# hazdzz/STGCN

Measured on AMD Instinct MI355X. Metric: training windows/sec, METR-LA ChebConv K=3 bs=32, higher is better.
Workload: dtype f32; 1 GPU; C2: METR-LA 207 nodes, STGCNChebGraphConv Ks=3 Kt=3, n_his=12, bs=32 per GPU, fp32, dropout 0.5, AdamW lr 1e-3 wd 1e-3; full step zero_grad+fwd+MSE+bwd+opt; graph=real metr_la adj -> sym_norm_lap -> cheb GSO, global_batch=32, parallelism=dp1, output_block=fused HIP path (stgcn_outblock_*), launch=hipGraph replay, chains=1, backward_products=fp32, operator_products=fp32

## Files before the change

### include/stgcn_hip.h

```cpp
#ifndef STGCN_HIP_H
#define STGCN_HIP_H
#include <stddef.h>
#include <stdint.h>
#ifdef __cplusplus
extern "C" {
#endif

#define STGCN_ABI_VERSION 10

#define STGCN_OK 0
#define STGCN_ERR_UNSUPPORTED 1
#define STGCN_ERR_INVALID 2
#define STGCN_ERR_LAUNCH 3

#define STGCN_ACT_GLU 0
#define STGCN_ACT_GTU 1
#define STGCN_GC_CHEB 0
#define STGCN_GC_KIPF 1

#define STGCN_DTYPE_F32 0
#define STGCN_DTYPE_BF16 1

typedef struct stgcn_stblock_desc {
    int32_t B, T, N;
// ... 154 lines not shown

typedef struct stgcn_head_loss {
    const float* pred;
    const float* target;
    const int64_t* target_index_dev;
    int64_t target_index_stride;
    const int64_t* target_window_dev;
    float grad_scale;
    int32_t kind;
    float delta;
} stgcn_head_loss;

typedef struct stgcn_outblock_plan {
    int64_t T1, rows, rows_in;
    int64_t out_floats;
    int64_t saved_floats, ws_floats;
    int64_t sv_U, sv_S;
    int64_t sv_mean, sv_rstd;
    int64_t sv_yln;
    int64_t sv_hd;
    int64_t sv_rowstat;
    int64_t ws_Wp, ws_Wd, ws_b, ws_W1p, ws_W1d;
    int64_t ws_rowstat_b, ws_dh1, ws_dyln, ws_dZ, ws_part, part_floats;
    int64_t ws_chain;
    int64_t chain_words;
} stgcn_outblock_plan;

int stgcn_outblock_plan_query(const stgcn_outblock_desc* desc, stgcn_outblock_plan* plan);
int stgcn_outblock_forward(const stgcn_outblock_desc* desc, const stgcn_outblock_params* params, const float* x, float* out,
                           float* saved, float* ws, uint64_t seed, uint64_t offset, const uint64_t* offset_dev, void* stream);
int stgcn_outblock_chain_status(const stgcn_outblock_desc* desc, const float* ws, uint32_t* sticky, void* stream);
int64_t stgcn_set_chain_spin_ticks(int64_t ticks);
int stgcn_outblock_backward(const stgcn_outblock_desc* desc, const stgcn_outblock_params* params, const float* x,
                            const float* dout, const float* saved, float* ws, const stgcn_outblock_grads* grads, float* dx,
                            void* stream);
int stgcn_outblock_backward_hook(const stgcn_outblock_desc* desc, const stgcn_outblock_params* params, const float* x,
                                 const float* dout, const float* saved, float* ws, const stgcn_outblock_grads* grads, float* dx,
                                 const stgcn_ln_hook* dx_hook, void* stream);
int stgcn_outblock_backward_loss(const stgcn_outblock_desc* desc, const stgcn_outblock_params* params, const float* x,
                                 const stgcn_head_loss* loss, const float* saved, float* ws, const stgcn_outblock_grads* grads, float* dx,
                                 const stgcn_ln_hook* dx_hook, void* stream);

typedef struct stgcn_prepack_block {
    const stgcn_stblock_desc* desc;
    const stgcn_stblock_params* params;
    float* ws;
} stgcn_prepack_block;
typedef struct stgcn_step_counter {
    int64_t* ptr;
    int64_t inc, mod;
} stgcn_step_counter;
int stgcn_prepack(int32_t n_blocks, const stgcn_prepack_block* blocks, const stgcn_outblock_desc* head_desc,
                  const stgcn_outblock_params* head_params, float* head_ws, int32_t n_counters, const stgcn_step_counter* counters,
                  void* stream);
int stgcn_prepack_park(int32_t n_blocks, const stgcn_prepack_block* blocks, const stgcn_outblock_desc* head_desc,
                  const stgcn_outblock_params* head_params, float* head_ws, int32_t n_counters, const stgcn_step_counter* counters,
                  void* stream);
int stgcn_prepack_flush(void);

typedef struct stgcn_adamw_tensor {
    float* param;
    const float* grad;
    float* exp_avg;
    float* exp_avg_sq;
    int64_t numel;
} stgcn_adamw_tensor;
int stgcn_adamw_step(const stgcn_adamw_tensor* tensors, int32_t count, float lr, float beta1, float beta2, float eps,
                     float weight_decay, int64_t step, const int64_t* step_dev, const float* lr_dev, void* stream);

typedef struct stgcn_flush_block {
    const stgcn_stblock_desc* desc;
    const stgcn_stblock_grads* grads;
    float* ws;
} stgcn_flush_block;
typedef struct stgcn_adamw_hyper {
    float lr, beta1, beta2, eps, weight_decay;
    int64_t step;
    const int64_t* step_dev;
    const float* lr_dev;
} stgcn_adamw_hyper;
int stgcn_grad_flush(int32_t n_blocks, const stgcn_flush_block* blocks, const stgcn_outblock_desc* head_desc,
                     const stgcn_outblock_grads* head_grads, float* head_ws, const stgcn_adamw_tensor* opt, int32_t opt_count,
                     const stgcn_adamw_hyper* hyper, void* stream);

#define STGCN_OPT_ADAMW 0
#define STGCN_OPT_NADAMW 1
#define STGCN_OPT_LION 2
typedef struct stgcn_optim_hyper {
    int32_t kind;
    double lr, beta1, beta2, eps, weight_decay, momentum_decay;
    int64_t step;
    const int64_t* step_dev;
    const float* lr_dev;
    float mu_product;
    float* mu_product_dev;
} stgcn_optim_hyper;
int stgcn_optim_step(const stgcn_adamw_tensor* tensors, int32_t count, const stgcn_optim_hyper* hyper, void* stream);
int stgcn_grad_flush_optim(int32_t n_blocks, const stgcn_flush_block* blocks, const stgcn_outblock_desc* head_desc,
                           const stgcn_outblock_grads* head_grads, float* head_ws, const stgcn_adamw_tensor* opt, int32_t opt_count,
                           const stgcn_optim_hyper* hyper, void* stream);

#define STGCN_CLIP_HDR_WORDS 8
typedef struct stgcn_grad_clip {
    double* state;
    int64_t state_words;
    float max_norm;
} stgcn_grad_clip;
int stgcn_grad_clip_words(const stgcn_adamw_tensor* tensors, int32_t count, int64_t* words);
int stgcn_grad_flush_clip_words(int32_t n_blocks, const stgcn_flush_block* blocks, const stgcn_outblock_desc* head_desc,
                                const stgcn_outblock_grads* head_grads, float* head_ws, int64_t* words);
int stgcn_grad_norm(const stgcn_adamw_tensor* tensors, int32_t count, const stgcn_grad_clip* clip, void* stream);
int stgcn_optim_step_clip(const stgcn_adamw_tensor* tensors, int32_t count, const stgcn_optim_hyper* hyper, const stgcn_grad_clip* clip,
                          void* stream);
int stgcn_grad_flush_clip(int32_t n_blocks, const stgcn_flush_block* blocks, const stgcn_outblock_desc* head_desc,
                          const stgcn_outblock_grads* head_grads, float* head_ws, const stgcn_grad_clip* clip, void* stream);

int stgcn_mse_loss_grad(const float* pred, const float* target, int64_t n, float grad_scale, float* loss, float* dpred,
                        const int64_t* target_index_dev, int64_t target_index_stride, void* stream);
int stgcn_mse_loss_grad_windows(const float* pred, const float* target, int64_t n, float grad_scale, float* loss, float* dpred,
                                const int64_t* target_index_dev, int64_t target_index_stride, const int64_t* target_window_dev,
                                int64_t window_floats, void* stream);
int stgcn_loss_grad(int32_t kind, float delta, const float* pred, const float* target, int64_t n, float grad_scale, float* loss,
                    float* dpred, const int64_t* target_index_dev, int64_t target_index_stride, const int64_t* target_window_dev,
                    int64_t window_floats, void* stream);

#define STGCN_EVAL_STATE_WORDS 264
#define STGCN_EVAL_POS_WORDS 4
int stgcn_eval_arm(double* state, int64_t* pos, void* stream);
int stgcn_eval_accumulate(const float* pred, const float* target, int32_t B, int32_t N, const float* scale, const float* mean,
                          int64_t first_valid, int64_t* pos, int64_t target_stride, int64_t num_windows, double* state, void* stream);

int stgcn_profile_enable(int on);
int stgcn_profile_collect(char* json_buf, size_t cap);

#ifdef __cplusplus
}
#endif
#endif
```

### stgcn_amd/_lib.py

```python
from __future__ import annotations

import ctypes as C
import os
from typing import Optional

_HERE = os.path.dirname(os.path.abspath(__file__))
DEFAULT_LIB = os.path.join(_HERE, "libstgcn_hip.so")

STGCN_OK = 0
ABI_VERSION = 10
ACT = {"glu": 0, "gtu": 1}
GRAPH_CONV = {"cheb_graph_conv": 0, "graph_conv": 1}
DTYPE_F32, DTYPE_BF16 = 0, 1
LOSS = {"mse": 0, "mae": 1, "huber": 2}
EVAL_STATE_WORDS, EVAL_POS_WORDS = 264, 4

_fp = C.POINTER(C.c_float)


class StblockDesc(C.Structure):
    _fields_ = [("B", C.c_int32), ("T", C.c_int32), ("N", C.c_int32), ("c_in", C.c_int32),
                ("c0", C.c_int32), ("c1", C.c_int32), ("c2", C.c_int32), ("Kt", C.c_int32), ("Ks", C.c_int32),
                ("act", C.c_int32), ("graph_conv", C.c_int32), ("training", C.c_int32),
                ("droprate", C.c_float), ("ln_eps", C.c_float), ("need_dx", C.c_int32), ("reserved", C.c_int32),
# ... 127 lines not shown
                                       C.POINTER(C.c_int32)]
        d.stgcn_gso_layout.restype = C.c_int
        d.stgcn_set_gc_tiled_min_nodes.argtypes = [C.c_int32]
        d.stgcn_set_gc_tiled_min_nodes.restype = C.c_int
        d.stgcn_outblock_backward_loss.argtypes = [C.POINTER(OutblockDesc), C.POINTER(OutblockParams), C.c_void_p, C.POINTER(HeadLoss), C.c_void_p,
                                                   C.c_void_p, C.POINTER(OutblockGrads), C.c_void_p, C.POINTER(LnHook), C.c_void_p]
        d.stgcn_outblock_backward_loss.restype = C.c_int
        d.stgcn_set_bwd_precision.argtypes = [C.c_int32]
        d.stgcn_set_bwd_precision.restype = C.c_int
        d.stgcn_set_slab_gc_precision.argtypes = [C.c_int32]
        d.stgcn_set_slab_gc_precision.restype = C.c_int
        d.stgcn_set_tc1_bwd_wgs.argtypes = [C.c_int32]
        d.stgcn_set_tc1_bwd_wgs.restype = C.c_int
        d.stgcn_set_tc2ln_peers.argtypes = [C.c_int32]
        d.stgcn_set_tc2ln_peers.restype = C.c_int
        d.stgcn_stblock_chain_status.argtypes = [C.POINTER(StblockDesc), C.c_void_p, C.POINTER(C.c_uint32), C.c_void_p]
        d.stgcn_stblock_chain_status.restype = C.c_int
        d.stgcn_set_debug_stages.argtypes = [C.c_int32]
        d.stgcn_set_debug_stages.restype = C.c_int
        d.stgcn_set_gc_precision.argtypes = [C.c_int32]
        d.stgcn_set_gc_precision.restype = C.c_int
        d.stgcn_set_gc_ld_pad.argtypes = [C.c_int32]
        d.stgcn_set_gc_ld_pad.restype = C.c_int
        d.stgcn_set_gemm_big_nt.argtypes = [C.c_int32]
        d.stgcn_set_gemm_big_nt.restype = C.c_int
        d.stgcn_set_chain_spin_ticks.argtypes = [C.c_int64]
        d.stgcn_set_chain_spin_ticks.restype = C.c_int64
        d.stgcn_outblock_chain_status.argtypes = [C.POINTER(OutblockDesc), C.c_void_p, C.POINTER(C.c_uint32), C.c_void_p]
        d.stgcn_outblock_chain_status.restype = C.c_int
        d.stgcn_stblock_forward.argtypes = [C.POINTER(StblockDesc), C.POINTER(StblockParams), C.c_void_p, C.c_void_p,
                                            C.c_void_p, C.c_void_p, C.c_void_p, C.c_uint64, C.c_uint64, C.c_void_p, C.c_void_p]
        d.stgcn_stblock_backward.argtypes = [C.POINTER(StblockDesc), C.POINTER(StblockParams), C.c_void_p, C.c_void_p,
                                             C.c_void_p, C.c_void_p, C.c_void_p, C.c_void_p, C.POINTER(StblockGrads), C.c_void_p,
                                             C.c_uint64, C.c_uint64, C.c_void_p, C.c_void_p]
        d.stgcn_stblock_backward_hook.argtypes = [C.POINTER(StblockDesc), C.POINTER(StblockParams), C.c_void_p, C.c_void_p,
                                                  C.c_void_p, C.c_void_p, C.c_void_p, C.c_void_p, C.POINTER(StblockGrads), C.c_void_p,
                                                  C.c_uint64, C.c_uint64, C.c_void_p, C.POINTER(LnHook), C.c_void_p]
        d.stgcn_stblock_ln_hook.argtypes = [C.POINTER(StblockDesc), C.POINTER(StblockParams), C.c_void_p, C.c_void_p, C.c_uint64, C.c_uint64,
                                            C.c_void_p, C.POINTER(LnHook)]
        d.stgcn_outblock_backward_hook.argtypes = [C.POINTER(OutblockDesc), C.POINTER(OutblockParams), C.c_void_p, C.c_void_p, C.c_void_p,
                                                   C.c_void_p, C.POINTER(OutblockGrads), C.c_void_p, C.POINTER(LnHook), C.c_void_p]
        for f in ("stgcn_stblock_backward_hook", "stgcn_stblock_ln_hook", "stgcn_outblock_backward_hook"):
            getattr(d, f).restype = C.c_int
        d.stgcn_dropout_mask.argtypes = [C.c_void_p, C.c_int64, C.c_float, C.c_uint64, C.c_uint64, C.c_void_p, C.c_void_p]
        d.stgcn_outblock_plan_query.argtypes = [C.POINTER(OutblockDesc), C.POINTER(OutblockPlan)]
        d.stgcn_outblock_forward.argtypes = [C.POINTER(OutblockDesc), C.POINTER(OutblockParams), C.c_void_p, C.c_void_p, C.c_void_p,
                                             C.c_void_p, C.c_uint64, C.c_uint64, C.c_void_p, C.c_void_p]
        d.stgcn_outblock_backward.argtypes = [C.POINTER(OutblockDesc), C.POINTER(OutblockParams), C.c_void_p, C.c_void_p, C.c_void_p,
                                              C.c_void_p, C.POINTER(OutblockGrads), C.c_void_p, C.c_void_p]
        for f in ("stgcn_outblock_plan_query", "stgcn_outblock_forward", "stgcn_outblock_backward"):
            getattr(d, f).restype = C.c_int
        d.stgcn_adamw_step.argtypes = [C.POINTER(AdamwTensor), C.c_int32, C.c_float, C.c_float, C.c_float, C.c_float, C.c_float, C.c_int64,
                                       C.c_void_p, C.c_void_p, C.c_void_p]
        d.stgcn_adamw_step.restype = C.c_int
        d.stgcn_prepack.argtypes = [C.c_int32, C.POINTER(PrepackBlock), C.POINTER(OutblockDesc), C.POINTER(OutblockParams), C.c_void_p,
                                    C.c_int32, C.POINTER(StepCounter), C.c_void_p]
        d.stgcn_prepack.restype = C.c_int
        d.stgcn_prepack_park.argtypes = [C.c_int32, C.POINTER(PrepackBlock), C.POINTER(OutblockDesc), C.POINTER(OutblockParams), C.c_void_p,
                                    C.c_int32, C.POINTER(StepCounter), C.c_void_p]
        d.stgcn_prepack_park.restype = C.c_int
        d.stgcn_prepack_flush.argtypes = []
        d.stgcn_prepack_flush.restype = C.c_int
        d.stgcn_grad_flush.argtypes = [C.c_int32, C.POINTER(FlushBlock), C.POINTER(OutblockDesc), C.POINTER(OutblockGrads), C.c_void_p,
                                       C.POINTER(AdamwTensor), C.c_int32, C.POINTER(AdamwHyper), C.c_void_p]
        d.stgcn_grad_flush.restype = C.c_int
        d.stgcn_optim_step.argtypes = [C.POINTER(AdamwTensor), C.c_int32, C.POINTER(OptimHyper), C.c_void_p]
        d.stgcn_optim_step.restype = C.c_int
        d.stgcn_grad_flush_optim.argtypes = [C.c_int32, C.POINTER(FlushBlock), C.POINTER(OutblockDesc), C.POINTER(OutblockGrads), C.c_void_p,
                                             C.POINTER(AdamwTensor), C.c_int32, C.POINTER(OptimHyper), C.c_void_p]
        d.stgcn_grad_flush_optim.restype = C.c_int
        for f in ("stgcn_grad_clip_words", "stgcn_grad_flush_clip_words", "stgcn_grad_norm", "stgcn_optim_step_clip", "stgcn_grad_flush_clip"):
            if not hasattr(d, f):
                raise StgcnError(f"{path} does not export {f} (built before gradient clipping was added): rebuild with "
                                 f"`python -m stgcn_amd.build --force`")
        d.stgcn_grad_clip_words.argtypes = [C.POINTER(AdamwTensor), C.c_int32, C.POINTER(C.c_int64)]
        d.stgcn_grad_flush_clip_words.argtypes = [C.c_int32, C.POINTER(FlushBlock), C.POINTER(OutblockDesc), C.POINTER(OutblockGrads), C.c_void_p,
                                                  C.POINTER(C.c_int64)]
        d.stgcn_grad_norm.argtypes = [C.POINTER(AdamwTensor), C.c_int32, C.POINTER(GradClip), C.c_void_p]
        d.stgcn_optim_step_clip.argtypes = [C.POINTER(AdamwTensor), C.c_int32, C.POINTER(OptimHyper), C.POINTER(GradClip), C.c_void_p]
        d.stgcn_grad_flush_clip.argtypes = [C.c_int32, C.POINTER(FlushBlock), C.POINTER(OutblockDesc), C.POINTER(OutblockGrads), C.c_void_p,
                                            C.POINTER(GradClip), C.c_void_p]
        for f in ("stgcn_grad_clip_words", "stgcn_grad_flush_clip_words", "stgcn_grad_norm", "stgcn_optim_step_clip", "stgcn_grad_flush_clip"):
            getattr(d, f).restype = C.c_int
        d.stgcn_mse_loss_grad.argtypes = [C.c_void_p, C.c_void_p, C.c_int64, C.c_float, C.c_void_p, C.c_void_p, C.c_void_p, C.c_int64,
                                          C.c_void_p]
        d.stgcn_mse_loss_grad.restype = C.c_int
        d.stgcn_mse_loss_grad_windows.argtypes = [C.c_void_p, C.c_void_p, C.c_int64, C.c_float, C.c_void_p, C.c_void_p, C.c_void_p, C.c_int64,
                                                  C.c_void_p, C.c_int64, C.c_void_p]
        d.stgcn_mse_loss_grad_windows.restype = C.c_int
        d.stgcn_loss_grad.argtypes = [C.c_int32, C.c_float, C.c_void_p, C.c_void_p, C.c_int64, C.c_float, C.c_void_p, C.c_void_p, C.c_void_p,
                                      C.c_int64, C.c_void_p, C.c_int64, C.c_void_p]
        d.stgcn_loss_grad.restype = C.c_int
        d.stgcn_eval_arm.argtypes = [C.c_void_p, C.c_void_p, C.c_void_p]
        d.stgcn_eval_arm.restype = C.c_int
        d.stgcn_eval_accumulate.argtypes = [C.c_void_p, C.c_void_p, C.c_int32, C.c_int32, C.c_void_p, C.c_void_p, C.c_int64, C.c_void_p,
                                            C.c_int64, C.c_int64, C.c_void_p, C.c_void_p]
        d.stgcn_eval_accumulate.restype = C.c_int
        d.stgcn_profile_enable.argtypes = [C.c_int]
        d.stgcn_profile_enable.restype = C.c_int
        d.stgcn_profile_collect.argtypes = [C.c_char_p, C.c_size_t]
        d.stgcn_profile_collect.restype = C.c_int
        for f in ("stgcn_stblock_plan_query", "stgcn_gso_prepare", "stgcn_stblock_forward", "stgcn_stblock_backward",
                  "stgcn_dropout_mask"):
            getattr(d, f).restype = C.c_int
        self.backend = d.stgcn_backend().decode()
        self.is_emulator = self.backend.startswith("emu")

    def check(self, rc: int, what: str):
        if rc != STGCN_OK:
            msg = self.dll.stgcn_last_error().decode()
            if rc == 1:
                raise NotImplementedError(f"{what}: {msg}")
            if rc == 2:
                raise ValueError(f"{what}: {msg}")
            raise StgcnError(f"{what}: {msg} (code {rc})")


_lib: Optional[_Lib] = None


def use_library(path: str) -> _Lib:
    global _lib
    _lib = _Lib(path)
    return _lib


def lib() -> _Lib:
    global _lib
    if _lib is None:
        _lib = _Lib(os.environ.get("STGCN_AMD_LIB", DEFAULT_LIB))
    return _lib


EXPORTED_SYMBOLS = ["stgcn_version", "stgcn_backend", "stgcn_last_error", "stgcn_stblock_plan_query", "stgcn_gso_prepare",
                    "stgcn_stblock_forward", "stgcn_stblock_backward", "stgcn_dropout_mask", "stgcn_profile_enable",
                    "stgcn_profile_collect", "stgcn_outblock_plan_query", "stgcn_outblock_forward", "stgcn_outblock_backward", "stgcn_adamw_step", "stgcn_prepack",
                    "stgcn_mse_loss_grad", "stgcn_mse_loss_grad_windows", "stgcn_grad_flush", "stgcn_gso_layout", "stgcn_set_gc_tiled_min_nodes",
                    "stgcn_set_gc_precision", "stgcn_set_gc_ld_pad", "stgcn_set_debug_stages",
                    "stgcn_stblock_ln_hook", "stgcn_stblock_backward_hook", "stgcn_outblock_backward_hook", "stgcn_set_tc1_bwd_wgs",
                    "stgcn_set_slab_gc_precision", "stgcn_outblock_backward_loss", "stgcn_set_bwd_precision", "stgcn_set_gemm_big_nt",
                    "stgcn_set_chain_spin_ticks", "stgcn_outblock_chain_status", "stgcn_set_tc2ln_peers", "stgcn_stblock_chain_status", "stgcn_prepack_park", "stgcn_prepack_flush",
                    "stgcn_optim_step", "stgcn_grad_flush_optim", "stgcn_eval_arm", "stgcn_eval_accumulate", "stgcn_loss_grad",
                    "stgcn_grad_clip_words", "stgcn_grad_flush_clip_words", "stgcn_grad_norm", "stgcn_optim_step_clip", "stgcn_grad_flush_clip"]
```

### stgcn_amd/csrc/stgcn_capi.hip

```cpp
#include "../../include/stgcn_hip.h"

#include <atomic>
#include <stdarg.h>
#include <stdio.h>
#include <stdlib.h>
#include <math.h>
#include <string.h>

#include "stgcn_kernels_bwd.hip.h"
#include "stgcn_kernels_fwd.hip.h"
#include "stgcn_kernels_gctile.hip.h"
#include "stgcn_kernels_gcslab16.hip.h"
#include "stgcn_kernels_head.hip.h"
#include "stgcn_route.h"

using namespace stgcn;

namespace {
thread_local char g_err[512] = "";
thread_local bool g_bf16 = false;
std::atomic<long long> g_chain_spin_ticks{kChainSpinTicks};
int g_gemm_big_nt = 0;

int fail(int code, const char* fmt, ...) __attribute__((format(printf, 2, 3)));
// ... 526 lines not shown
    const int HT = a.NP / 16;
    int pf = 0, pb = 1;
    gc_parts_override(pf, pb);
    {
        const int force_parts = force_gcbwd2_parts();
        const bool b16p = g_bf16 && a.Ks > 1;
        const size_t lds2 = gconv_bwd2_lds_bytes(a.NP, a.N, a.Ks, b16p);
        if (lds2 <= 150 * 1024 && HT <= 64) {
            int best = 0;
            for (int parts = (HT + 7) / 8; parts <= HT && !force_parts; ++parts) {
                const int per = (HT + parts - 1) / parts, njw = gcbwd2_job_waves(a.Ks, parts, per > 8 ? 8 : per);
                if (per < 4 && parts > (HT + 7) / 8) break;
                const int cap = b16p ? wg_capacity(gconv_bwd2_kernel<1, bf16, true>, ((per > 8 ? 8 : per) + njw) * 64, lds2)
                                     : STGCN_ETB_VALUE(wg_capacity(gconv_bwd2_kernel<1, ET>, ((per > 8 ? 8 : per) + njw) * 64, lds2));
                if (a.slabs * parts <= cap) best = parts;
            }
            if (force_parts > 0 && force_parts <= HT && (HT + force_parts - 1) / force_parts <= 24) best = force_parts;
            if (!best && !force_parts && HT <= 24) best = 1;
            if (best > 0) {
                const int per = (HT + best - 1) / best, nwa = per > 8 ? 8 : per, maxq = (per + nwa - 1) / nwa, njw = gcbwd2_job_waves(a.Ks, best, nwa);
                a.parts = best;
                const dim3 grid2((unsigned)(a.slabs * best)), blk2((nwa + njw) * 64);
                if (b16p) {
                    if (maxq <= 1) STGCN_LAUNCH("gconv_bwd", st, (gconv_bwd2_kernel<1, bf16, true>), grid2, blk2, lds2, a, nwa);
                    else if (maxq <= 2) STGCN_LAUNCH("gconv_bwd", st, (gconv_bwd2_kernel<2, bf16, true>), grid2, blk2, lds2, a, nwa);
                    else STGCN_LAUNCH("gconv_bwd", st, (gconv_bwd2_kernel<3, bf16, true>), grid2, blk2, lds2, a, nwa);
                    return STGCN_OK;
                }
                if (maxq <= 1) STGCN_LAUNCH_ETB("gconv_bwd", st, (gconv_bwd2_kernel<1, ET>), grid2, blk2, lds2, a, nwa);
                else if (maxq <= 2) STGCN_LAUNCH_ETB("gconv_bwd", st, (gconv_bwd2_kernel<2, ET>), grid2, blk2, lds2, a, nwa);
                else STGCN_LAUNCH_ETB("gconv_bwd", st, (gconv_bwd2_kernel<3, ET>), grid2, blk2, lds2, a, nwa);
                return STGCN_OK;
            }
        }
    }
    const GcGeom g = gc_geom(HT, pb);
    a.parts = g.parts;
    const size_t lds = ((size_t)a.Ks * 16 * (a.NP + 4) + (size_t)a.NP * 20) * sizeof(float);
    if (lds > 160 * 1024) return fail(STGCN_ERR_UNSUPPORTED, "graph-conv backward needs %zu bytes of LDS (N=%d, terms=%d)", lds, a.N, a.Ks);
    const dim3 grid((unsigned)(a.slabs * g.parts)), blk(g.waves * 64);
    if (g.maxq <= 1) STGCN_LAUNCH_ETB("gconv_bwd", st, (gconv_bwd_kernel<1, 16, ET>), grid, blk, lds, a);
    else if (g.maxq <= 2) STGCN_LAUNCH_ETB("gconv_bwd", st, (gconv_bwd_kernel<2, 8, ET>), grid, blk, lds, a);
    else if (g.maxq <= 3) STGCN_LAUNCH_ETB("gconv_bwd", st, (gconv_bwd_kernel<3, 8, ET>), grid, blk, lds, a);
    else if (g.maxq <= 4) STGCN_LAUNCH_ETB("gconv_bwd", st, (gconv_bwd_kernel<4, 8, ET>), grid, blk, lds, a);
    else return fail(STGCN_ERR_UNSUPPORTED, "graph convolution with %d nodes (supported: up to 512)", a.N);
    return STGCN_OK;
}

template <int MTW>
int launch_bwd_weight_n(const char* label, const TconvBwdWeightArgs& a, const WgradGeom& w, hipStream_t st) {
    const dim3 grid(w.chunks, w.mchunks), blk(kThreads * kWgradGroups);
    if (a.NC == 128) STGCN_LAUNCH_ET(label, st, (tconv_bwd_weight_kernel<MTW, 2, true, ET>), grid, blk, wgrad_lds_bytes(MTW, 2), a);
    else STGCN_LAUNCH_ET(label, st, (tconv_bwd_weight_kernel<MTW, 4, true, ET>), grid, blk, wgrad_lds_bytes(MTW, 4), a);
    return STGCN_OK;
}
int launch_bwd_weight(const char* label, const TconvBwdWeightArgs& a, const WgradGeom& w, hipStream_t st) {
    if (a.NC != 128 && a.NC != 256) return fail(STGCN_ERR_UNSUPPORTED, "weight gradient with %d output channels", a.NC);
    if ((a.ts.C & 3) != 0) {
        if (w.MTW != 1) return fail(STGCN_ERR_UNSUPPORTED, "weight gradient: c_in=%d needs Kt*c_in <= 16", a.ts.C);
        if (a.NC == 128) STGCN_LAUNCH_ET(label, st, (tconv_bwd_weight_kernel<1, 2, false, ET>), dim3(w.chunks, w.mchunks), dim3(kThreads * kWgradGroups), wgrad_lds_bytes(1, 2), a);
        else STGCN_LAUNCH_ET(label, st, (tconv_bwd_weight_kernel<1, 4, false, ET>), dim3(w.chunks, w.mchunks), dim3(kThreads * kWgradGroups), wgrad_lds_bytes(1, 4), a);
        return STGCN_OK;
    }
    switch (w.MTW) {
        case 1: return launch_bwd_weight_n<1>(label, a, w, st);
        case 2: return launch_bwd_weight_n<2>(label, a, w, st);
        case 3: return launch_bwd_weight_n<3>(label, a, w, st);
        default: return launch_bwd_weight_n<4>(label, a, w, st);
    }
}

inline bool wgrad_pair_ok(const TconvBwdWeightArgs& a1, const WgradGeom& w1, const TconvBwdWeightArgs& a2, const WgradGeom& w2) {
    return a1.NC == 256 && w1.MTW == 4 && a2.NC == 128 && w2.MTW == 4 && (a1.ts.C & 3) == 0 && (a2.ts.C & 3) == 0;
}
int launch_wgrad_pair(const char* label, const TconvBwdWeightArgs& a1, const WgradGeom& w1, const TconvBwdWeightArgs& a2, const WgradGeom& w2,
                      hipStream_t st) {
    const int n1 = w1.chunks * w1.mchunks, n2 = w2.chunks * w2.mchunks;
    const size_t l1 = wgrad_lds_bytes(4, 4), l2 = wgrad_lds_bytes(4, 2);
    STGCN_LAUNCH_ETB(label, st, (wgrad_pair_kernel<4, 4, 4, 2, ET>), dim3((unsigned)(n1 + n2)), dim3(kThreads * kWgradGroups), l1 > l2 ? l1 : l2, a1, n1,
                    w1.mchunks, a2, n2, w2.mchunks);
    return STGCN_OK;
}

struct ReduceList {
    ReduceArgs ra;
    int nj;
    bool overflow;
    ReduceList() : nj(0), overflow(false) { memset(&ra, 0, sizeof(ra)); }
    void add(float* dst, const float* src, int Pn, long pstride, int n0, int n1, int n2, long s0, long s1, long s2, long t0, long t1,
             long t2) {
        if (!dst) return;
        if (nj >= kMaxReduceJobs) { overflow = true; return; }
        ReduceJob& j = ra.job[nj];
        j.src = src; j.dst = dst; j.P = Pn; j.pstride = pstride; j.n0 = n0; j.n1 = n1; j.n2 = n2;
        j.s0 = (int)s0; j.s1 = (int)s1; j.s2 = (int)s2; j.t0 = (int)t0; j.t1 = (int)t1; j.t2 = (int)t2;
        ra.start[nj + 1] = ra.start[nj] + reduce_job_setup(j);
        ++nj;
    }
    void add_flat(float* dst, const float* src, int Pn, long pstride, int n) { add(dst, src, Pn, pstride, 1, 1, n, 0, 0, 1, 0, 0, 1); }
};
int launch_reduce_list(const char* label, ReduceList& L, hipStream_t st) {
    if (L.overflow) return fail(STGCN_ERR_INVALID, "%s: more than %d reduction jobs in one launch", label, kMaxReduceJobs);
    if (L.nj == 0) return STGCN_OK;
    L.ra.njobs = L.nj;
    if (reduce_log())
        for (int i = 0; i < L.nj; ++i) {
            const ReduceJob& j = L.ra.job[i];
            fprintf(stderr, "[stgcn reduce] %s job %d: %ld elements x %d partials (%.2f MB read), %d workgroups\n", label, i,
                    (long)j.n0 * j.n1 * j.n2, j.P, 4e-6 * (double)j.n0 * j.n1 * j.n2 * j.P, L.ra.start[i + 1] - L.ra.start[i]);
        }
    STGCN_LAUNCH(label, st, reduce_kernel<kOptAdamw>, dim3(L.ra.start[L.nj]), dim3(kThreads), kThreads * 4 * sizeof(float), L.ra);
    return STGCN_OK;
}
int launch_reduce_list_optim(const char* label, ReduceList& L, int kind, const OptimExtra& x, hipStream_t st) {
    if (L.overflow) return fail(STGCN_ERR_INVALID, "%s: more than %d reduction jobs in one launch", label, kMaxReduceJobs);
    if (L.nj == 0) return STGCN_OK;
    L.ra.njobs = L.nj;
    ReduceOptimArgs a = zeroed<ReduceOptimArgs>();
    static_cast<ReduceArgs&>(a) = L.ra;
    a.x = x;
    if (kind == kOptNadamw)
        STGCN_LAUNCH(label, st, reduce_kernel<kOptNadamw>, dim3(L.ra.start[L.nj]), dim3(kThreads), kThreads * 4 * sizeof(float), a);
    else
        STGCN_LAUNCH(label, st, reduce_kernel<kOptLion>, dim3(L.ra.start[L.nj]), dim3(kThreads), kThreads * 4 * sizeof(float), a);
    return STGCN_OK;
}
void reduce_jobs_block(ReduceList& L, const stgcn_stblock_desc* d, const BlockRoute& v, const float* part, const stgcn_stblock_grads* G) {
    const BwdGeom& bg = v.bg;
    auto add_tconv_at = [&](const float* wp, const float* bp, int Pn, long ps, long pb, int NC, long LD, int Cin, int Cout, float* gw, float* gb, float* gaw,
                            float* gab) {
        L.add(gw, wp, Pn, ps, NC, d->Kt, Cin, LD, Cin, 1, (long)Cin * d->Kt, 1, d->Kt);
        L.add_flat(gb, bp, Pn, pb, NC);
        if (Cin > Cout) {
            L.add(gaw, wp + (long)(d->Kt - 1) * Cin, Pn, ps, 1, Cout, Cin, 0, LD, 1, 0, Cin, 1);
            L.add_flat(gab, bp, Pn, pb, Cout);
        }
    };
    auto add_tconv = [&](const WgradGeom& w, int Cin, int Cout, float* gw, float* gb, float* gaw, float* gab) {
        const float* wp = part + w.off;
        add_tconv_at(wp, wp + (long)w.chunks * w.Mpad * w.NC, w.chunks, (long)w.Mpad * w.NC, w.NC, w.NC, w.Mpad, Cin, Cout, gw, gb, gaw, gab);
    };
    if (bg.k3) {
        const float* wp = part + bg.off_k3;
        add_tconv_at(wp, wp + (long)d->Kt * d->c_in * v.NC1, bg.k3_wgs, bg.k3_stride, bg.k3_stride, v.NC1, (long)d->Kt * d->c_in, d->c_in, d->c0, G->tc1_w,
                     G->tc1_b, G->tc1_aw, G->tc1_ab);
    } else if (bg.thin) {
        const float* wp = part + bg.off_al + (long)d->c0 * 16 + 16;
        L.add(G->tc1_w, wp, bg.al_wgs, bg.al_stride, d->Kt, d->c_in, v.NC1, (long)d->c_in * v.NC1, v.NC1, 1, 1, d->Kt, (long)d->c_in * d->Kt);
        L.add_flat(G->tc1_b, wp + 16 * v.NC1, bg.al_wgs, bg.al_stride, v.NC1);
    } else {
        add_tconv(bg.w1, d->c_in, d->c0, G->tc1_w, G->tc1_b, G->tc1_aw, G->tc1_ab);
    }
    if (bg.k1) {
        const float* wp = part + bg.off_k1;
        add_tconv_at(wp, wp + (long)d->Kt * 16 * v.NC2, bg.k1_wgs, bg.k1_stride, bg.k1_stride, v.NC2, (long)d->Kt * 16, d->c1, d->c2, G->tc2_w, G->tc2_b,
                     G->tc2_aw, G->tc2_ab);
    } else {
        add_tconv(bg.w2, d->c1, d->c2, G->tc2_w, G->tc2_b, G->tc2_aw, G->tc2_ab);
    }
    if (d->c0 > d->c1) {
        const float* ap = bg.k3 ? part + bg.off_k3 + (long)d->Kt * d->c_in * v.NC1 + v.NC1 : part + bg.off_al;
        const int Pn = bg.k3 ? bg.k3_wgs : bg.al_wgs, ps = bg.k3 ? bg.k3_stride : bg.al_stride;
        L.add(G->al_w, ap, Pn, ps, 1, d->c0, d->c1, 0, d->c1, 1, 0, 1, d->c0);
        L.add_flat(G->al_b, ap + (long)d->c0 * d->c1, Pn, ps, d->c1);
    }
    if (d->graph_conv == STGCN_GC_KIPF) L.add_flat(G->gc_w, part + bg.off_gc + 256, bg.gc_count, bg.gc_stride, 256);
// ... 315 lines not shown
    hipStream_t st = (hipStream_t)stream;
    const int NP = gc_padded_nodes(N, terms);
    const size_t M = (size_t)NP * NP;
    const dim3 grid(cdiv((int64_t)M, kThreads)), blk(kThreads);
    if (gc_is_tiled(N, terms)) {
        STGCN_LAUNCH("gso_dense", st, gso_dense_kernel, grid, blk, 0, gso, (int)N, NP, gso_pad);
        STGCN_LAUNCH("gso_dense_t", st, gso_dense_t_kernel, grid, blk, 0, gso, (int)N, NP, gso_t_pad);
        unsigned short* hp = reinterpret_cast<unsigned short*>(gso_pad + M);
        unsigned short* ht = reinterpret_cast<unsigned short*>(gso_t_pad + M);
        const int LD = gc_plane_ld(NP);
        STGCN_LAUNCH("gso_bf16", st, gso_bf16_kernel, grid, blk, 0, gso, (int)N, NP, LD, 0, hp, hp + (size_t)NP * LD);
        STGCN_LAUNCH("gso_bf16_t", st, gso_bf16_kernel, grid, blk, 0, gso, (int)N, NP, LD, 1, ht, ht + (size_t)NP * LD);
        return STGCN_OK;
    }
    float* D[3] = {scratch, scratch + M, scratch + 2 * M};
    STGCN_LAUNCH("gso_dense", st, gso_dense_kernel, grid, blk, 0, gso, (int)N, NP, D[0]);
    const float* tm1 = D[0];
    const float* tm2 = nullptr;
    for (int k = 1; k < terms; ++k) {
        const float* tk = tm1;
        if (k >= 2) {
            float* out = (tm1 == D[1]) ? D[2] : D[1];
            STGCN_LAUNCH("cheb_next", st, cheb_next_kernel, grid, blk, 0, (const float*)D[0], tm1, tm2, (int)N, NP, out);
            tm2 = tm1;
            tm1 = out;
            tk = out;
        }
        STGCN_LAUNCH("gso_frag", st, gso_frag_kernel, grid, blk, 0, tk, NP, gso_pad + (size_t)(k - 1) * M, gso_t_pad + (size_t)(k - 1) * M);
        const size_t t16 = gs16_term_floats(NP, N), o16 = (size_t)(terms - 1) * M + (size_t)(k - 1) * t16;
        const int KC32 = gs16_np32(N) / 32;
        STGCN_LAUNCH("gso_frag16", st, gso_frag16_kernel, dim3(cdiv((int64_t)(NP / 16) * KC32 * 512, kThreads)), blk, 0, tk, NP, KC32, gso_pad + o16,
                     gso_t_pad + o16);
    }
    return STGCN_OK;
}

int stgcn_dropout_mask(float* out, int64_t n, float droprate, uint64_t seed, uint64_t offset, const uint64_t* offset_dev, void* stream) {
    if (!out || n < 0 || (n & 3)) return fail(STGCN_ERR_INVALID, "stgcn_dropout_mask: n must be a non-negative multiple of 4");
    if (!(droprate >= 0.f && droprate < 1.f)) return fail(STGCN_ERR_INVALID, "stgcn_dropout_mask: droprate must be in [0, 1)");
    if (n == 0) return STGCN_OK;
    STGCN_LAUNCH("dropout_mask", (hipStream_t)stream, dropout_mask_kernel, dim3(cdiv(n / 4, kThreads)), dim3(kThreads), 0, out,
                 (long)(n / 4), seed, offset, offset_dev, drop_thresh(droprate), 1.0f / (1.0f - droprate));
    return STGCN_OK;
}

int stgcn_stblock_ln_hook(const stgcn_stblock_desc* d, const stgcn_stblock_params* P, const float* y, float* ws, uint64_t seed, uint64_t offset,
                          const uint64_t* offset_dev, stgcn_ln_hook* h) {
    stgcn_stblock_plan pl;
    int rc = stgcn_stblock_plan_query(d, &pl);
    if (rc) return rc;
    if (!P || !P->ln_w || !P->ln_b || !y || !ws || !h) return fail(STGCN_ERR_INVALID, "stgcn_stblock_ln_hook: NULL argument");
    memset(h, 0, sizeof(*h));
    if (!(fuse_mask() & FUSE_ROWSTATS)) return STGCN_OK;
    h->rowstat = ws + pl.ws_rowstat_b; h->y = y; h->gamma = P->ln_w; h->beta = P->ln_b;
    h->N = d->N; h->C = d->c2; h->training = d->training; h->droprate = d->droprate; h->dtype = d->dtype;
    h->seed = seed; h->offset = offset; h->offset_dev = offset_dev;
    return STGCN_OK;
}

int stgcn_stblock_chain_status(const stgcn_stblock_desc* d, const float* ws, uint32_t* sticky, void* stream) {
    STGCN_FLUSH_PENDING_PACK();
    stgcn_stblock_plan pl;
    const int rc = stgcn_stblock_plan_query(d, &pl);
    if (rc) return rc;
    return read_chain_sticky("stgcn_stblock_chain_status", ws, pl.ws_chain, sticky, stream);
}

int stgcn_stblock_forward(const stgcn_stblock_desc* d, const stgcn_stblock_params* P, const float* x, const float* gso_pad, float* y,
                          float* saved, float* ws, uint64_t seed, uint64_t offset, const uint64_t* offset_dev, void* stream) {
    BlockCall c{d, P, {}, {}, x, saved, ws, seed, offset, offset_dev, (hipStream_t)stream};
    int rc = route_and_plan(d, &c.r, &c.pl);
    if (rc) return rc;
    if (!P || !x || !gso_pad || !y || !saved || !ws) return fail(STGCN_ERR_INVALID, "stgcn_stblock_forward: NULL buffer");
    if (!P->tc1_w || !P->tc1_b || !P->gc_w || !P->tc2_w || !P->tc2_b || !P->ln_w || !P->ln_b)
        return fail(STGCN_ERR_INVALID, "stgcn_stblock_forward: missing parameter pointer");
    if (d->c_in > d->c0 && !P->tc1_aw) return fail(STGCN_ERR_INVALID, "tc1_aw required when c_in > c0");
    if (d->c0 > d->c1 && !P->al_w) return fail(STGCN_ERR_INVALID, "al_w required when c0 > c1");
    if (d->c1 > d->c2 && !P->tc2_aw) return fail(STGCN_ERR_INVALID, "tc2_aw required when c1 > c2");
    g_prof_tag = d->reserved;
    g_bf16 = c.r.bf16;

    const bool ride = g_pending_pack.valid && d->prepacked && c.r.tc1_fwd == TC1_FWD_THIN && g_pending_pack.st == c.st;
    if (!ride) STGCN_FLUSH_PENDING_PACK();
    if (!d->prepacked) rc = c.launch_block_pack();
    if (rc) return rc;

    switch (c.r.tc1_fwd) {
        case TC1_FWD_TSTEP: rc = c.launch_tc1_fwd(); break;
        case TC1_FWD_THIN: rc = c.launch_thin_fwd(ride); break;
        case TC1_FWD_ROWTILE: rc = c.launch_rowtile_tc1_fwd(); break;
    }
    if (rc) return rc;
    rc = c.launch_block_gconv_fwd(gso_pad);
    if (rc) return rc;
    return c.r.tc2_ln_fused ? c.launch_tc2_ln_fwd(y) : c.launch_staged_tc2_ln_fwd(y);
}

#include "stgcn_capi_bwd.inc"
#include "stgcn_capi_head.inc"
```

### stgcn_amd/csrc/stgcn_capi_bwd.inc

```

namespace {
int launch_hook_rowstats(const stgcn_ln_hook* hook, const float* dx, long slabs, hipStream_t st) {
    LnBwdArgs hl = zeroed<LnBwdArgs>();
    const LnRowstatOut o = rowstat_out(hook);
    hl.dy = dx; hl.y = o.y; hl.beta = o.beta; hl.gamma = o.gamma; hl.rowstat = o.rowstat;
    hl.n = o.N * o.C; hl.N = o.N; hl.C = o.C; hl.act = o.act; hl.training = o.training; hl.slabs = slabs;
    hl.keep_scale = o.keep_scale; hl.thresh = o.thresh; hl.seed = o.seed; hl.offset = o.offset; hl.offset_dev = o.offset_dev;
    STGCN_LAUNCH_ET("ln_bwd_rowstats", st, (ln_bwd_rowstats_kernel<ET>), dim3(cdiv(hl.slabs * (hl.n / 4), kThreads)), dim3(kThreads), 0, hl);
    return STGCN_OK;
}

struct BlockBwdCall : BlockCall {
    const float* gso_t_pad;
    const float* dy;
    const float* y;
    float* dx;
    const stgcn_ln_hook* dx_hook;
    LnBwdArgs ln;

    int launch_ln_bwd_stats() {
        ln = zeroed<LnBwdArgs>();
        ln.dy = dy; ln.y = y; ln.beta = P->ln_b; ln.U = saved + pl.sv_U2; ln.S = saved + pl.sv_S2; ln.gamma = P->ln_w;
        ln.mean = saved + pl.sv_mean; ln.rstd = saved + pl.sv_rstd; ln.rowstat = reinterpret_cast<float2*>(ws + pl.ws_rowstat_b);
        ln.dZ = ws + pl.ws_dZ2; ln.dgam_part = part() + r.bg.off_ln_g; ln.dbet_part = part() + r.bg.off_ln_b;
// ... 36 lines not shown
            else if (d->act == STGCN_ACT_GLU) STGCN_LAUNCH_ETB("tc2_bwd", st, (tc2_bwd_kernel<C2_, KT_, false, 0, RC_, ET>), grid, blk, lds, a);       \
            else STGCN_LAUNCH_ETB("tc2_bwd", st, (tc2_bwd_kernel<C2_, KT_, false, 1, RC_, ET>), grid, blk, lds, a);                 \
        } while (0)
#define STGCN_TC2_BWD_RC(C2_, KT_) do { if (recomp) { constexpr bool RC_ = true; STGCN_TC2_BWD(C2_, KT_); } else { constexpr bool RC_ = false; STGCN_TC2_BWD(C2_, KT_); } } while (0)
        if (d->Kt == 2) STGCN_TC2_BWD_RC(64, 2); else if (d->Kt == 3) STGCN_TC2_BWD_RC(64, 3); else STGCN_TC2_BWD_RC(64, 4);
#undef STGCN_TC2_BWD_RC
#undef STGCN_TC2_BWD
        return STGCN_OK;
    }
    int launch_staged_tc2_bwd() {
        STGCN_F32_ONLY("ln_gate_bwd + row-tile weight / data gradients of tmp_conv2");
        int rc = launch_ln_gate_bwd();
        if (rc) return rc;
        TconvBwdWeightArgs wa = zeroed<TconvBwdWeightArgs>();
        wa.ts = make_taps(saved + pl.sv_G, d->c1, d->Kt, d->N, r.T1, r.T2, 1, r.rows2);
        wa.dZ = ws + pl.ws_dZ2; wa.part = part() + r.bg.w2.off; wa.NC = r.NC2; wa.Mpad = r.bg.w2.Mpad; wa.rows_per_chunk = r.bg.w2.rows_per_chunk;
        wa.chunks = r.bg.w2.chunks;
        rc = launch_bwd_weight("tconv_bwd_weight.tc2", wa, r.bg.w2, st);
        if (rc) return rc;
        TconvBwdDataArgs a = zeroed<TconvBwdDataArgs>();
        a.ts = make_taps(ws + pl.ws_dZ2, r.NC2, d->Kt, d->N, r.T2, r.T1, -1, r.rows1);
        a.Wp = ws + pl.ws_W2d; a.KCH = d->Kt * r.NC2 / 16; a.Cin = d->c1; a.Gmask = saved + pl.sv_G; a.dX = ws + pl.ws_dYg;
        return launch_bwd_data("tconv_bwd_data.tc2", a, r.CP1 / 16, st);
    }
    int launch_block_gconv_bwd() {
        GconvBwdArgs a = zeroed<GconvBwdArgs>();
        a.dY = ws + pl.ws_dYg; a.X0 = saved + pl.sv_A; a.Xk = saved + pl.sv_Xk; a.LTp = gso_t_pad; a.W = P->gc_w;
        a.dA = ws + pl.ws_dA; a.part = part() + r.bg.off_gc; a.N = d->N; a.NP = r.NP; a.Ks = r.terms;
        a.kipf = d->graph_conv == STGCN_GC_KIPF; a.slabs = r.slabs1;
        a.Gk = r.tiled_gc ? ws + pl.ws_Gk : nullptr; a.tiles_per_wg = r.bg.gc_tiles_per_wg; a.wgs = r.bg.gc_count;
        a.XT = r.tiled_gc && r.terms > 1 ? ws + pl.ws_XT : nullptr;
        return launch_gconv_bwd(a, r.tiled_gc, st);
    }
    int launch_align_gate_bwd() {
        STGCN_F32_ONLY("align_gate_bwd");
        AlignBwdArgs a = zeroed<AlignBwdArgs>();
        a.dA = ws + pl.ws_dA; a.WaT = ws + pl.ws_WaT; a.dZ = ws + pl.ws_dZ1;
        if (r.recompute_tc1) {
            a.Wd = ws + pl.ws_W1dense; a.bias = ws + pl.ws_b1; a.KPd = r.KP1;
            a.ts = input_taps();
        } else {
            a.U = saved + pl.sv_U1; a.S = saved + pl.sv_S1;
        }
        a.part = part() + r.bg.off_al; a.rows = r.rows1; a.c0 = d->c0; a.c1 = d->c1; a.KCH = r.CP1 / 16; a.act = d->act;
        const size_t lds = (size_t)(64 * (d->c1 + 4) + 64 * (d->c0 + 4) + 16 * d->c1) * sizeof(float);
        if (d->c0 == 64) STGCN_LAUNCH("align_gate_bwd", st, (align_gate_bwd_kernel<1>), dim3(r.bg.al_wgs), dim3(kThreads), lds, a);
        else STGCN_LAUNCH("align_gate_bwd", st, (align_gate_bwd_kernel<2>), dim3(r.bg.al_wgs), dim3(kThreads), lds, a);
        return STGCN_OK;
    }
    int launch_tc1_bwd() {
        if (g_debug_stages && !g_bf16) {
            const int rc = launch_align_gate_bwd();
            if (rc) return rc;
        }
        Tc1BwdArgs a = zeroed<Tc1BwdArgs>();
        a.dA = ws + pl.ws_dA; a.U = saved + pl.sv_U1; a.S = saved + pl.sv_S1; a.x = x; a.WaD = ws + pl.ws_WaDense; a.Wd = ws + pl.ws_W1dense;
        a.dx = dx; a.part = part() + r.bg.off_k3; a.B = d->B; a.T = d->T; a.T1 = r.T1; a.N = d->N; a.node_tiles = r.bg.node_tiles;
        const bool hooked = dx_hook && dx_hook->rowstat, epi = hooked && dx_hook->C == d->c_in && dx_hook->N == d->N;
        if (epi) a.rs = rowstat_out(dx_hook);
        const bool x6 = r.tc1_bwd_x6;
        const size_t lds = r.tc1_bwd_lds;
        const dim3 grid((unsigned)r.bg.k3_wgs), blk(768);
#define STGCN_TC1_BWD(CIN_)                                                                                    \
        do {                                                                                                       \
            if (x6 && d->act == STGCN_ACT_GLU) STGCN_LAUNCH("tc1_bwd", st, (tc1_bwd_x6_kernel<64, CIN_, 3, 0>), grid, blk, lds, a);   \
            else if (x6) STGCN_LAUNCH("tc1_bwd", st, (tc1_bwd_x6_kernel<64, CIN_, 3, 1>), grid, blk, lds, a);             \
            else if (d->act == STGCN_ACT_GLU) STGCN_LAUNCH_ETB("tc1_bwd", st, (tc1_bwd_kernel<64, CIN_, 3, 0, ET>), grid, blk, lds, a);   \
            else STGCN_LAUNCH_ETB("tc1_bwd", st, (tc1_bwd_kernel<64, CIN_, 3, 1, ET>), grid, blk, lds, a);             \
        } while (0)
        if (d->c_in == 64) STGCN_TC1_BWD(64); else if (d->c_in == 32) STGCN_TC1_BWD(32); else STGCN_TC1_BWD(16);
#undef STGCN_TC1_BWD
        if (hooked && !epi) return launch_hook_rowstats(dx_hook, dx, (long)d->B * d->T, st);
        return STGCN_OK;
    }
    int launch_thin_bwd() {
        ThinBwdArgs a = zeroed<ThinBwdArgs>();
        a.dA = ws + pl.ws_dA; a.Wd = ws + pl.ws_W1dense; a.bias = ws + pl.ws_b1; a.WaT = ws + pl.ws_WaT;
        a.dZ = d->need_dx ? ws + pl.ws_dZ1 : nullptr; a.part = part() + r.bg.off_al; a.rows = r.rows1; a.c0 = d->c0; a.act = d->act;
        a.ts = input_taps();
        const dim3 grid(r.bg.al_wgs), blk(kThreads);
        if (!r.thin_bwd_waves) {
            const size_t lds = (size_t)(64 * 20 + 64 * (d->c0 + 4) + 64 * (2 * d->c0 + 4) + 64 * 20 + 256) * sizeof(float);
            STGCN_LAUNCH_ETB("align_gate_bwd", st, (thin_tc1_bwd_kernel<ET>), grid, blk, lds, a);
        } else if (d->act == STGCN_ACT_GLU) STGCN_LAUNCH_ETB("align_gate_bwd", st, (thin_tc1_bwd2_kernel<ET, 0>), grid, blk, thin_bwd2_lds_bytes(), a);
        else STGCN_LAUNCH_ETB("align_gate_bwd", st, (thin_tc1_bwd2_kernel<ET, 1>), grid, blk, thin_bwd2_lds_bytes(), a);
        return STGCN_OK;
    }
    int launch_tc1_bwd_weight() {
        TconvBwdWeightArgs wa = zeroed<TconvBwdWeightArgs>();
        wa.ts = input_taps();
        wa.dZ = ws + pl.ws_dZ1; wa.part = part() + r.bg.w1.off; wa.NC = r.NC1; wa.Mpad = r.bg.w1.Mpad; wa.rows_per_chunk = r.bg.w1.rows_per_chunk;
        wa.chunks = r.bg.w1.chunks;
        return launch_bwd_weight("tconv_bwd_weight.tc1", wa, r.bg.w1, st);
    }
    int launch_tc1_bwd_data() {
        TconvBwdDataArgs a = zeroed<TconvBwdDataArgs>();
        a.ts = make_taps(ws + pl.ws_dZ1, r.NC1, d->Kt, d->N, r.T1, d->T, -1, r.rows0);
        a.Wp = ws + pl.ws_W1d; a.KCH = d->Kt * r.NC1 / 16; a.Cin = d->c_in; a.Gmask = nullptr; a.dX = dx;
        const int rc = launch_bwd_data("tconv_bwd_data.tc1", a, r.CP_in / 16, st);
        if (rc || !(dx_hook && dx_hook->rowstat)) return rc;
        return launch_hook_rowstats(dx_hook, dx, (long)d->B * d->T, st);
    }
};
}

int stgcn_stblock_backward(const stgcn_stblock_desc* d, const stgcn_stblock_params* P, const float* x, const float* gso_t_pad,
                           const float* dy, const float* y, const float* saved, float* ws, const stgcn_stblock_grads* G, float* dx, uint64_t seed,
                           uint64_t offset, const uint64_t* offset_dev, void* stream) {
    return stgcn_stblock_backward_hook(d, P, x, gso_t_pad, dy, y, saved, ws, G, dx, seed, offset, offset_dev, nullptr, stream);
}

int stgcn_stblock_backward_hook(const stgcn_stblock_desc* d, const stgcn_stblock_params* P, const float* x, const float* gso_t_pad,
                                const float* dy, const float* y, const float* saved, float* ws, const stgcn_stblock_grads* G, float* dx, uint64_t seed,
                                uint64_t offset, const uint64_t* offset_dev, const stgcn_ln_hook* dx_hook, void* stream) {
    STGCN_FLUSH_PENDING_PACK();
    BlockBwdCall c{{d, P, {}, {}, x, const_cast<float*>(saved), ws, seed, offset, offset_dev, (hipStream_t)stream}, gso_t_pad, dy, y, dx, dx_hook, {}};
    int rc = route_and_plan(d, &c.r, &c.pl);
    if (rc) return rc;
    if (c.r.bf16 && !c.r.bf16_bwd_ok)
        return fail(STGCN_ERR_UNSUPPORTED, "stgcn_stblock_backward: no bf16 backward for c_in=%d channels=(%d, %d, %d) Kt=%d T=%d need_dx=%d "
                    "(bf16 blocks need tc2_bwd_kernel, and tc1_bwd_kernel or the thin first layer without an input gradient)",
                    d->c_in, d->c0, d->c1, d->c2, d->Kt, d->T, d->need_dx);
    if (!P || !x || !gso_t_pad || !dy || !saved || !ws || !G) return fail(STGCN_ERR_INVALID, "stgcn_stblock_backward: NULL buffer");
    if (!d->dy_rowstats_ready && !y) return fail(STGCN_ERR_INVALID, "stgcn_stblock_backward: y (the forward's output) is required unless dy_rowstats_ready is set");
    if (d->need_dx && !dx) return fail(STGCN_ERR_INVALID, "stgcn_stblock_backward: need_dx set but dx is NULL");
    rc = check_dx_hook("stgcn_stblock_backward", dx_hook, d->N, d->c_in, d->need_dx, d->dtype);
    if (rc) return rc;
    g_prof_tag = d->reserved;
    g_bf16 = c.r.bf16;

    rc = c.launch_ln_bwd_stats();
    if (rc) return rc;
    rc = c.r.tc2_bwd == BWD_FUSED ? c.launch_tc2_bwd() : c.launch_staged_tc2_bwd();
    if (rc) return rc;
    rc = c.launch_block_gconv_bwd();
    if (rc) return rc;
    if (c.r.tc1_bwd == BWD_FUSED) {
        rc = c.launch_tc1_bwd();
    } else {
        rc = c.r.tc1_bwd == BWD_THIN ? c.launch_thin_bwd() : c.launch_align_gate_bwd();
        if (!rc && c.r.tc1_bwd == BWD_STAGED) rc = c.launch_tc1_bwd_weight();
        if (!rc && d->need_dx) rc = c.launch_tc1_bwd_data();
    }
    if (rc) return rc;

    if (d->defer_reduce) return STGCN_OK;
    ReduceList RL;
    reduce_jobs_block(RL, d, c.r, c.part(), G);
    return launch_reduce_list("reduce", RL, c.st);
}
```

### stgcn_amd/csrc/stgcn_capi_head.inc

```

namespace {
struct HeadGeom {
    int T1, NC, KP, KCH, CPin, ln_spg, ln_sg, fc_wgs;
    int dense_bwd;
    int fused_ln_bwd;
    int64_t rows, rows_in, slabs;
    WgradGeom wc, wf;
    long off_ln_g, off_ln_b, off_fc, total;
};

int head_check(const stgcn_outblock_desc* d) {
    if (!d) return fail(STGCN_ERR_INVALID, "desc is NULL");
    if (d->B < 1 || d->T < 1 || d->N < 1 || d->c_in < 1 || d->Ko < 1) return fail(STGCN_ERR_INVALID, "B/T/N/c_in/Ko must be positive");
    if (d->T < d->Ko) return fail(STGCN_ERR_INVALID, "T=%d shorter than Ko=%d", d->T, d->Ko);
    if (d->act != STGCN_ACT_GLU && d->act != STGCN_ACT_GTU) return fail(STGCN_ERR_INVALID, "act must be glu or gtu");
    if (!(d->droprate >= 0.f && d->droprate < 1.f)) return fail(STGCN_ERR_INVALID, "droprate must be in [0, 1)");
    if (!(d->c0 == 64 || d->c0 == 128)) return fail(STGCN_ERR_UNSUPPORTED, "output-head conv channels must be 64 or 128 (got %d)", d->c0);
    if (d->c1 != 128) return fail(STGCN_ERR_UNSUPPORTED, "output-head fc1 width must be 128 (got %d)", d->c1);
    if (d->c_end != 1) return fail(STGCN_ERR_UNSUPPORTED, "end_channel must be 1 (got %d)", d->c_end);
    if ((d->c_in & 3) != 0 && d->Ko * d->c_in > 16) return fail(STGCN_ERR_UNSUPPORTED, "c_in=%d must be a multiple of 4", d->c_in);
    if (d->dtype != STGCN_DTYPE_F32 && d->dtype != STGCN_DTYPE_BF16) return fail(STGCN_ERR_INVALID, "dtype must be STGCN_DTYPE_F32 or STGCN_DTYPE_BF16");
    return STGCN_OK;
}

// ... 75 lines not shown
    ok &= L.add(PK_TCONV_FWD, g.NC * g.KP, ws + pl.ws_Wp, P->tc_w, P->tc_b, P->tc_aw, P->tc_ab, d->c_in, d->c0, d->Ko, g.KCH);
    if (d->need_dx || all) {
        if (g.dense_bwd)
            ok &= L.add(PK_TCONV_BWDT, g.NC * d->Ko * d->c_in, ws + pl.ws_Wd, P->tc_w, P->tc_b, P->tc_aw, P->tc_ab, d->c_in, d->c0, d->Ko, g.NC / 16);
        else
            ok &= L.add(PK_TCONV_BWD, d->Ko * g.NC * g.CPin, ws + pl.ws_Wd, P->tc_w, P->tc_b, P->tc_aw, P->tc_ab, d->c_in, d->c0, d->Ko,
                        d->Ko * g.NC / 16);
    }
    ok &= L.add(PK_TCONV_BIAS, g.NC, ws + pl.ws_b, P->tc_w, P->tc_b, P->tc_aw, P->tc_ab, d->c_in, d->c0, d->Ko, 0);
    ok &= L.add(PK_LIN_FWD, d->c0 * d->c1, ws + pl.ws_W1p, P->fc1_w, nullptr, nullptr, nullptr, d->c0, d->c1, 1, d->c0 / 16);
    ok &= L.add(PK_LIN_BWD, d->c1 * d->c0, ws + pl.ws_W1d, P->fc1_w, nullptr, nullptr, nullptr, d->c0, d->c1, 1, d->c1 / 16);
    ok &= L.add(PK_ZERO, (int)pl.chain_words, ws + pl.ws_chain, nullptr, nullptr, nullptr, nullptr, 0, 0, 0, 0);
    return ok;
}

int prepack_impl(int32_t n_blocks, const stgcn_prepack_block* blocks, const stgcn_outblock_desc* hd, const stgcn_outblock_params* hp,
                 float* hws, int32_t n_counters, const stgcn_step_counter* counters, void* stream, bool park) {
    if (n_blocks < 0 || (n_blocks > 0 && !blocks)) return fail(STGCN_ERR_INVALID, "stgcn_prepack: bad block list");
    if (n_counters < 0 || n_counters > kMaxStepCounters || (n_counters > 0 && !counters))
        return fail(STGCN_ERR_INVALID, "stgcn_prepack: at most %d step counters", kMaxStepCounters);
    STGCN_FLUSH_PENDING_PACK();
    g_prof_tag = 0;
    PackList L;
    L.pa.ncounters = n_counters;
    for (int k = 0; k < n_counters; ++k) {
        if (!counters[k].ptr) return fail(STGCN_ERR_INVALID, "stgcn_prepack: NULL step counter %d", k);
        L.pa.cptr[k] = reinterpret_cast<long*>(counters[k].ptr); L.pa.cinc[k] = (long)counters[k].inc; L.pa.cmod[k] = (long)counters[k].mod;
    }
    auto flush_list = [&]() -> int {
        const int rc = launch_pack_list("prepack", L, (hipStream_t)stream);
        L = PackList();
        return rc;
    };
    auto append = [&](auto&& fill) -> int {
        PackList trial = L;
        if (!fill(trial)) {
            if (L.nj == 0) return fail(STGCN_ERR_UNSUPPORTED, "stgcn_prepack: one module needs more than %d pack jobs", kMaxPackJobs);
            const int rc = flush_list();
            if (rc) return rc;
            trial = L;
            if (!fill(trial)) return fail(STGCN_ERR_UNSUPPORTED, "stgcn_prepack: pack job table overflow");
        }
        L = trial;
        return STGCN_OK;
    };
    for (int i = 0; i < n_blocks; ++i) {
        const stgcn_prepack_block& b = blocks[i];
        if (!b.desc || !b.params || !b.ws) return fail(STGCN_ERR_INVALID, "stgcn_prepack: NULL entry in block %d", i);
        BlockRoute r;
        stgcn_stblock_plan pl;
        int rc = route_and_plan(b.desc, &r, &pl);
        if (!rc) rc = append([&](PackList& T) { return pack_fill_block(T, b.desc, r, b.params, pl, b.ws, true); });
        if (rc) return rc;
    }
    if (hd) {
        if (!hp || !hws) return fail(STGCN_ERR_INVALID, "stgcn_prepack: head params / ws are NULL");
        stgcn_outblock_plan pl;
        int rc = stgcn_outblock_plan_query(hd, &pl);
        if (!rc) rc = append([&](PackList& T) { return pack_fill_head(T, hd, hp, pl, hws, true); });
        if (rc) return rc;
    }
    if (L.nj == 0 && L.pa.ncounters == 0) return STGCN_OK;
    if (park && L.nj > 0) {
        g_pending_pack.valid = true;
        g_pending_pack.L = L;
        g_pending_pack.st = (hipStream_t)stream;
        return STGCN_OK;
    }
    return launch_pack_list("prepack", L, (hipStream_t)stream);
}

int check_loss_kind(const char* who, int32_t kind, float delta) {
    if (kind != STGCN_LOSS_MSE && kind != STGCN_LOSS_MAE && kind != STGCN_LOSS_HUBER)
        return fail(STGCN_ERR_INVALID, "%s: unknown loss kind %d (STGCN_LOSS_MSE = 0, _MAE = 1, _HUBER = 2)", who, (int)kind);
    if (kind == STGCN_LOSS_HUBER && !(delta > 0.f && isfinite(delta)))
        return fail(STGCN_ERR_INVALID, "%s: Huber delta = %g must be finite and positive", who, (double)delta);
    return STGCN_OK;
}

int outblock_backward_impl(const stgcn_outblock_desc* d, const stgcn_outblock_params* P, const float* x, const float* dout,
                           const stgcn_head_loss* hl, const float* saved, float* ws, const stgcn_outblock_grads* G, float* dx,
                           const stgcn_ln_hook* dx_hook, void* stream) {
    STGCN_FLUSH_PENDING_PACK();
    stgcn_outblock_plan pl;
    int rc = stgcn_outblock_plan_query(d, &pl);
    if (rc) return rc;
    if (!P || !x || (!dout && !hl) || !saved || !ws || !G) return fail(STGCN_ERR_INVALID, "stgcn_outblock_backward: NULL buffer");
    if (d->need_dx && !dx) return fail(STGCN_ERR_INVALID, "stgcn_outblock_backward: need_dx set but dx is NULL");
    rc = check_dx_hook("stgcn_outblock_backward", dx_hook, d->N, d->c_in, d->need_dx, d->dtype);
    if (rc) return rc;
    const HeadGeom g = head_geom(d);
    hipStream_t st = (hipStream_t)stream;
    g_prof_tag = 0;
    g_bf16 = d->dtype == STGCN_DTYPE_BF16;
    float* part = ws + pl.ws_part;
    const int training = d->training && d->droprate > 0.f;
    const bool own_rowstats = (fuse_mask() & FUSE_ROWSTATS) && d->c0 == d->c1 && d->c0 == 128;

    {
        FcBwdArgs a = zeroed<FcBwdArgs>();
        a.dout = dout; a.hd = saved + pl.sv_hd; a.w2 = P->fc2_w; a.W1d = ws + pl.ws_W1d; a.dh1 = ws + pl.ws_dh1; a.dyln = ws + pl.ws_dyln;
        a.part = part + g.off_fc; a.rows = g.rows; a.c0 = d->c0; a.c1 = d->c1; a.KCH = d->c1 / 16;
        a.grad_scale = training ? 1.0f / (1.0f - d->droprate) : 1.0f;
        if (hl) {
            a.pred = hl->pred; a.target = hl->target; a.target_index = reinterpret_cast<const long*>(hl->target_index_dev);
            a.target_index_stride = (long)hl->target_index_stride; a.loss_scale = hl->grad_scale;
            a.loss_kind = hl->kind; a.loss_delta = hl->delta;
            a.target_window = reinterpret_cast<const long*>(hl->target_window_dev); a.target_window_elems = (unsigned)(g.rows / d->B);
        }
        if (own_rowstats) {
            a.rs.rowstat = reinterpret_cast<float2*>(ws + pl.ws_rowstat_b); a.rs.U = saved + pl.sv_U; a.rs.S = saved + pl.sv_S; a.rs.gamma = P->ln_w;
            a.rs.mean = saved + pl.sv_mean; a.rs.rstd = saved + pl.sv_rstd; a.rs.N = d->N; a.rs.C = d->c0; a.rs.act = d->act; a.rs.training = 0;
            a.rs.keep_scale = 1.f;
        }
        const size_t lds = (size_t)(head_fc_tile_rows() * (d->c1 + 4) + 8 * d->c1 + 16) * sizeof(float);
        if (head_fc_tile_rows() == 16) {
            if (d->c0 == 128) STGCN_LAUNCH_ETB("head.fc_bwd", st, (fc_bwd_kernel<1, 2, ET>), dim3(g.fc_wgs), dim3(kThreads), lds, a);
            else STGCN_LAUNCH_ETB("head.fc_bwd", st, (fc_bwd_kernel<1, 1, ET>), dim3(g.fc_wgs), dim3(kThreads), lds, a);
        } else if (d->c0 == 128) STGCN_LAUNCH_ETB("head.fc_bwd", st, (fc_bwd_kernel<2, 2, ET>), dim3(g.fc_wgs), dim3(kThreads), lds, a);
        else STGCN_LAUNCH_ETB("head.fc_bwd", st, (fc_bwd_kernel<2, 1, ET>), dim3(g.fc_wgs), dim3(kThreads), lds, a);
    }
    TconvBwdWeightArgs wa = zeroed<TconvBwdWeightArgs>();
    wa.ts = make_taps(saved + pl.sv_yln, d->c0, 1, d->N, g.T1, g.T1, 1, g.rows);
    wa.dZ = ws + pl.ws_dh1; wa.part = part + g.wf.off; wa.NC = d->c1; wa.Mpad = g.wf.Mpad; wa.rows_per_chunk = g.wf.rows_per_chunk;
    wa.chunks = g.wf.chunks;
    const TconvBwdWeightArgs wfc = wa;
    TconvBwdWeightArgs wcv = wa;
    wcv.ts.src = x; wcv.ts.C = d->c_in; wcv.ts.taps = d->Ko; wcv.ts.Tsrc = d->T; wcv.ts.Tdst = g.T1;
    wcv.dZ = ws + pl.ws_dZ; wcv.part = part + g.wc.off; wcv.NC = g.NC; wcv.Mpad = g.wc.Mpad; wcv.rows_per_chunk = g.wc.rows_per_chunk;
    wcv.chunks = g.wc.chunks;
    const bool pair = wgrad_pair_ok(wcv, g.wc, wfc, g.wf);
    if (!pair) {
        rc = launch_bwd_weight("head.fc1_bwd_weight", wfc, g.wf, st);
        if (rc) return rc;
    }
    LnBwdArgs ln = zeroed<LnBwdArgs>();
    ln.dy = ws + pl.ws_dyln; ln.U = saved + pl.sv_U; ln.S = saved + pl.sv_S; ln.gamma = P->ln_w;
    ln.mean = saved + pl.sv_mean; ln.rstd = saved + pl.sv_rstd; ln.rowstat = reinterpret_cast<float2*>(ws + pl.ws_rowstat_b);
    ln.dZ = ws + pl.ws_dZ; ln.dgam_part = part + g.off_ln_g; ln.dbet_part = part + g.off_ln_b;
    ln.n = d->N * d->c0; ln.N = d->N; ln.C = d->c0; ln.act = d->act; ln.training = 0; ln.spg = g.ln_spg; ln.slabs = g.slabs;
    ln.keep_scale = 1.f; ln.thresh = 0;
    if (!own_rowstats)
        STGCN_LAUNCH_ET("head.ln_bwd_rowstats", st, (ln_bwd_rowstats_kernel<ET>), dim3(cdiv(g.slabs * (ln.n / 4), kThreads)), dim3(kThreads), 0, ln);
    if (cdiv(ln.n / 4, kThreads) >= kLnBigColgroups) {
        ln.slabconst = reinterpret_cast<float2*>(ws + pl.ws_rowstat_b + 2 * g.rows);
        STGCN_LAUNCH("head.ln_slab_consts", st, ln_slab_consts_kernel, dim3((unsigned)g.slabs), dim3(kThreads), 64, ln);
    }
    const bool fused_ln = g.fused_ln_bwd && own_rowstats;
    if (!fused_ln)
        STGCN_LAUNCH_ET("head.ln_gate_bwd", st, (ln_gate_bwd_kernel<ET>), dim3(cdiv(ln.n / 4, kThreads), g.ln_sg), dim3(kThreads),
                        (8 + 2 * g.ln_spg) * sizeof(float), ln);
    bool hook_pending = false;
    if (d->need_dx && g.dense_bwd) {
        Tconv4Args aa = zeroed<Tconv4Args>();
        aa.f.ts = make_taps(ws + pl.ws_dZ, g.NC, 1, d->N, 1, 1, 1, g.rows);
        aa.f.Wp = ws + pl.ws_Wd; aa.f.KCH = g.NC / 16; aa.f.Cout = 128;
        aa.out = dx; aa.outT = d->T; aa.outC = d->c_in;
        const bool epi = dx_hook && dx_hook->rowstat && dx_hook->C == d->c_in && (d->c_in == 64 || d->c_in == 128) && dx_hook->N == d->N;
        if (epi) aa.rs = rowstat_out(dx_hook);
        if (fused_ln) {
            aa.lnb.dy = ln.dy; aa.lnb.U = ln.U; aa.lnb.S = ln.S; aa.lnb.gamma = ln.gamma; aa.lnb.mean = ln.mean; aa.lnb.rstd = ln.rstd;
            aa.lnb.rowstat = ln.rowstat; aa.lnb.dZ = ln.dZ; aa.lnb.dgam = ln.dgam_part; aa.lnb.N = d->N; aa.lnb.C = d->c0; aa.lnb.act = d->act;
            aa.lnb.dbet = g_bf16 ? ln.dbet_part : nullptr;
        }
        rc = launch_tconv_fwd4<true>("head.tconv_bwd_data", aa, st);
        if (rc) return rc;
        if (dx_hook && dx_hook->rowstat && !epi) hook_pending = true;
    } else if (d->need_dx) {
        TconvBwdDataArgs a = zeroed<TconvBwdDataArgs>();
        a.ts = make_taps(ws + pl.ws_dZ, g.NC, d->Ko, d->N, g.T1, d->T, -1, g.rows_in);
        a.Wp = ws + pl.ws_Wd; a.KCH = d->Ko * g.NC / 16; a.Cin = d->c_in; a.Gmask = nullptr; a.dX = dx;
        rc = launch_bwd_data("head.tconv_bwd_data", a, g.CPin / 16, st);
        if (rc) return rc;
        if (dx_hook && dx_hook->rowstat) hook_pending = true;
    }
    rc = pair ? launch_wgrad_pair("head.wgrad_pair", wcv, g.wc, wfc, g.wf, st) : launch_bwd_weight("head.tconv_bwd_weight", wcv, g.wc, st);
    if (rc) return rc;
    if (hook_pending) {
        rc = launch_hook_rowstats(dx_hook, dx, (long)d->B * d->T, st);
        if (rc) return rc;
    }
    if (d->defer_reduce) return STGCN_OK;
    ReduceList RL;
    reduce_jobs_head(RL, d, g, part, ws + pl.ws_dyln, G);
    return launch_reduce_list("head.reduce", RL, st);
}
int flush_job_list(ReduceList& RL, const char* who, int32_t n_blocks, const stgcn_flush_block* blocks, const stgcn_outblock_desc* head_desc,
                   const stgcn_outblock_grads* head_grads, float* head_ws, const stgcn_adamw_tensor* opt, int32_t opt_count, bool need_v) {
    if (n_blocks < 0 || (n_blocks > 0 && !blocks)) return fail(STGCN_ERR_INVALID, "%s: bad block table", who);
    for (int i = 0; i < n_blocks; ++i) {
        const stgcn_stblock_desc* d = blocks[i].desc;
        BlockRoute r;
        stgcn_stblock_plan pl;
        int rc = route_and_plan(d, &r, &pl);
        if (rc) return rc;
        if (!blocks[i].grads || !blocks[i].ws) return fail(STGCN_ERR_INVALID, "%s: NULL pointer in block %d", who, i);
        reduce_jobs_block(RL, d, r, blocks[i].ws + pl.ws_part, blocks[i].grads);
    }
    if (head_desc) {
        stgcn_outblock_plan pl;
        int rc = stgcn_outblock_plan_query(head_desc, &pl);
        if (rc) return rc;
        if (!head_grads || !head_ws) return fail(STGCN_ERR_INVALID, "%s: NULL head pointer", who);
        const HeadGeom g = head_geom(head_desc);
        reduce_jobs_head(RL, head_desc, g, head_ws + pl.ws_part, head_ws + pl.ws_dyln, head_grads);
    }
    if (opt_count > 0) {
        int matched = 0;
        for (int k = 0; k < RL.nj; ++k)
            for (int i = 0; i < opt_count; ++i)
                if (opt[i].grad == RL.ra.job[k].dst) {
                    if (!opt[i].param || !opt[i].exp_avg || (need_v && !opt[i].exp_avg_sq)) return fail(STGCN_ERR_INVALID, "%s: NULL pointer in optimizer entry %d", who, i);
                    RL.ra.job[k].p = opt[i].param; RL.ra.job[k].m = opt[i].exp_avg; RL.ra.job[k].v = opt[i].exp_avg_sq;
                    if (((reinterpret_cast<uintptr_t>(opt[i].param) | reinterpret_cast<uintptr_t>(opt[i].exp_avg) | reinterpret_cast<uintptr_t>(opt[i].exp_avg_sq)) & 15) != 0)
                        RL.ra.job[k].dvec = 0;
                    ++matched;
                    break;
                }
        if (matched != opt_count) return fail(STGCN_ERR_INVALID, "%s: %d of %d optimizer entries have no gradient in this flush", who, opt_count - matched, opt_count);
    }
    return STGCN_OK;
}

OptimExtra optim_extra(const stgcn_optim_hyper* h) {
    OptimExtra x = zeroed<OptimExtra>();
    x.omb1 = (float)(1.0 - h->beta1);
    x.omb2 = (float)(1.0 - h->beta2);
    x.mu_k = (float)(h->momentum_decay * log(0.96));
    x.mu_prod = h->mu_product;
    x.mu_dev = h->kind == STGCN_OPT_NADAMW ? h->mu_product_dev : nullptr;
    x.mu_job = -1;
    return x;
}
int check_optim_hyper(const stgcn_optim_hyper* h, const char* who) {
    if (!h) return fail(STGCN_ERR_INVALID, "%s: NULL hyper-parameters", who);
    if (h->kind != STGCN_OPT_ADAMW && h->kind != STGCN_OPT_NADAMW && h->kind != STGCN_OPT_LION)
        return fail(STGCN_ERR_INVALID, "%s: unknown optimizer kind %d", who, (int)h->kind);
    return STGCN_OK;
}
}

int stgcn_outblock_plan_query(const stgcn_outblock_desc* d, stgcn_outblock_plan* p) {
    int rc = head_check(d);
    if (rc) return rc;
    if (!p) return fail(STGCN_ERR_INVALID, "plan is NULL");
    const HeadGeom g = head_geom(d);
    memset(p, 0, sizeof(*p));
    p->T1 = g.T1; p->rows = g.rows; p->rows_in = g.rows_in; p->out_floats = g.rows * d->c_end;
    int64_t o = 0;
    auto take = [&](int64_t n) { int64_t at = o; o += rup(n, 64); return at; };
    const bool bf = d->dtype == STGCN_DTYPE_BF16;
    auto act = [&](int64_t n) { return bf ? (n + 1) / 2 : n; };
    p->sv_U = take(act(g.rows * d->c0));
    p->sv_S = take(act(g.rows * d->c0));
    p->sv_mean = take(g.slabs);
    p->sv_rstd = take(g.slabs);
    p->sv_yln = take(act(g.rows * d->c0));
    p->sv_hd = take(act(g.rows * d->c1));
    p->sv_rowstat = take(2 * g.rows);
    p->saved_floats = o;
    o = 0;
    p->chain_words = kChainHdr + g.slabs;
    p->ws_chain = take(p->chain_words);
    p->ws_Wp = take((int64_t)g.NC * g.KP);
    p->ws_Wd = take((int64_t)d->Ko * g.NC * g.CPin);
    p->ws_b = take(g.NC);
    p->ws_W1p = take((int64_t)d->c0 * d->c1);
    p->ws_W1d = take((int64_t)d->c1 * d->c0);
    p->ws_rowstat_b = take(2 * g.rows + 2 * g.slabs);
    p->ws_dh1 = take(act(g.rows * d->c1));
    p->ws_dyln = take(act(g.rows * d->c0));
    p->ws_dZ = take(act(g.rows * g.NC));
    p->part_floats = g.total;
    p->ws_part = take(g.total);
    p->ws_floats = o;
    return STGCN_OK;
}

int stgcn_prepack(int32_t n_blocks, const stgcn_prepack_block* blocks, const stgcn_outblock_desc* hd, const stgcn_outblock_params* hp,
                  float* hws, int32_t n_counters, const stgcn_step_counter* counters, void* stream) {
    return prepack_impl(n_blocks, blocks, hd, hp, hws, n_counters, counters, stream, false);
}
int stgcn_prepack_flush(void) {
    return flush_pending_pack();
}
int stgcn_prepack_park(int32_t n_blocks, const stgcn_prepack_block* blocks, const stgcn_outblock_desc* hd, const stgcn_outblock_params* hp,
                       float* hws, int32_t n_counters, const stgcn_step_counter* counters, void* stream) {
    return prepack_impl(n_blocks, blocks, hd, hp, hws, n_counters, counters, stream, true);
}

int stgcn_outblock_forward(const stgcn_outblock_desc* d, const stgcn_outblock_params* P, const float* x, float* out, float* saved,
                           float* ws, uint64_t seed, uint64_t offset, const uint64_t* offset_dev, void* stream) {
    STGCN_FLUSH_PENDING_PACK();
    stgcn_outblock_plan pl;
    int rc = stgcn_outblock_plan_query(d, &pl);
    if (rc) return rc;
    if (!P || !x || !out || !saved || !ws) return fail(STGCN_ERR_INVALID, "stgcn_outblock_forward: NULL buffer");
    if (!P->tc_w || !P->tc_b || !P->ln_w || !P->ln_b || !P->fc1_w || !P->fc2_w)
        return fail(STGCN_ERR_INVALID, "stgcn_outblock_forward: missing parameter pointer");
    if (d->c_in > d->c0 && !P->tc_aw) return fail(STGCN_ERR_INVALID, "tc_aw required when c_in > c0");
    const HeadGeom g = head_geom(d);
    hipStream_t st = (hipStream_t)stream;
    g_prof_tag = 0;
    g_bf16 = d->dtype == STGCN_DTYPE_BF16;

    if (!d->prepacked) {
        PackList L;
        if (!pack_fill_head(L, d, P, pl, ws, false)) return fail(STGCN_ERR_INVALID, "pack job table overflow");
        rc = launch_pack_list("head.pack", L, st);
        if (rc) return rc;
    }

    TconvFwdArgs t = zeroed<TconvFwdArgs>();
    t.ts = make_taps(x, d->c_in, d->Ko, d->N, d->T, g.T1, 1, g.rows);
    t.Wp = ws + pl.ws_Wp; t.bias = ws + pl.ws_b; t.KCH = g.KCH; t.Cout = d->c0; t.act = d->act;
    t.U = saved + pl.sv_U; t.S = saved + pl.sv_S; t.rowstat = reinterpret_cast<float2*>(saved + pl.sv_rowstat);

    if (head_fuse_mode() && g.T1 == 1 && d->c0 == 128 && d->c1 == 128 && tconv4_ok(t)) {
        constexpr int KC = 4;
        int tm = 0, ticket = 0;
        {
            const int forced = head_fuse_mode() > 1 ? head_fuse_mode() : 0;
            const size_t l2 = (size_t)(tconv2_lds_floats(g.KP, 256, 32) + 48) * sizeof(float), l4 = (size_t)(tconv2_lds_floats(g.KP, 256, 64) + 48) * sizeof(float);
            const int cap2 = STGCN_ET_VALUE(wg_capacity(head_fwd_kernel<2, KC, ET>, 512, l2));
            const int cap4 = STGCN_ET_VALUE(wg_capacity(head_fwd_kernel<4, KC, ET>, 512, l4));
            const int t2 = cdiv(g.rows, 32), t4 = cdiv(g.rows, 64);
            const bool tk2 = d->N >= 32 && d->N <= 1024 && cap2 >= 4 * cdiv(d->N, 32) + 16, tk4 = d->N >= 64 && d->N <= 2048 && cap4 >= 4 * cdiv(d->N, 64) + 16;
            if (forced == 2) { if (d->N >= 32 && t2 <= cap2) tm = 2; }
            else if (forced == 4) { if (d->N >= 64 && t4 <= cap4) tm = 4; }
            else if (forced == 3) { if (tk2) { tm = 2; ticket = 1; } }
            else if (forced == 5) { if (tk4) { tm = 4; ticket = 1; } }
            else if (tk2 && t2 <= cap2) { tm = 2; ticket = 1; }
            else if (tk4 && t4 <= cap4) { tm = 4; ticket = 1; }
            else if (tk2) { tm = 2; ticket = 1; }
            else if (tk4) { tm = 4; ticket = 1; }
        }
        if (tm) {
            Tconv4Args aa = zeroed<Tconv4Args>();
            aa.f = t;
            HeadFcTail f = zeroed<HeadFcTail>();
            const int TR = 16 * tm, tiles = cdiv(g.rows, TR);
            f.chain.words = reinterpret_cast<unsigned*>(ws + pl.ws_chain); f.chain.ncount = (int)g.slabs; f.chain.total = (unsigned)tiles;
            f.chain.spin = g_chain_spin_ticks;
            f.gamma = P->ln_w; f.beta = P->ln_b; f.yln = saved + pl.sv_yln; f.mean = saved + pl.sv_mean; f.rstd = saved + pl.sv_rstd;
            f.eps = d->ln_eps;
            f.W1p = ws + pl.ws_W1p; f.b1 = P->fc1_b; f.w2 = P->fc2_w; f.b2 = P->fc2_b; f.hd = saved + pl.sv_hd; f.out = out;
            f.training = d->training && d->droprate > 0.f;
            f.keep_scale = 1.0f / (1.0f - d->droprate); f.thresh = drop_thresh(d->droprate); f.seed = seed; f.offset = offset;
            f.offset_dev = offset_dev;
            f.use_ticket = ticket;
            const size_t lds = (size_t)(tconv2_lds_floats(g.KP, 256, TR) + 48) * sizeof(float);
            if (tm == 2) STGCN_LAUNCH_ET("head.fwd", st, (head_fwd_kernel<2, KC, ET>), dim3(tiles), dim3(512), lds, aa, f);
            else STGCN_LAUNCH_ET("head.fwd", st, (head_fwd_kernel<4, KC, ET>), dim3(tiles), dim3(512), lds, aa, f);
            return STGCN_OK;
        }
    }
    rc = launch_tconv_fwd("head.tconv_fwd", t, st);
    if (rc) return rc;

    LnFwdArgs ln = zeroed<LnFwdArgs>();
    ln.U = saved + pl.sv_U; ln.S = saved + pl.sv_S; ln.gamma = P->ln_w; ln.beta = P->ln_b; ln.y = saved + pl.sv_yln;
    ln.mean = saved + pl.sv_mean; ln.rstd = saved + pl.sv_rstd; ln.rowstat = reinterpret_cast<const float2*>(saved + pl.sv_rowstat);
    ln.n = d->N * d->c0; ln.N = d->N; ln.C = d->c0; ln.act = d->act; ln.training = 0;
    ln.eps = d->ln_eps; ln.keep_scale = 1.f; ln.thresh = 0;
    const bool fuse_ln = (fuse_mask() & FUSE_HEAD_LN_FWD) && g.T1 == 1 && d->c0 % 16 == 0 && d->c0 <= 128 && d->N <= 1024;
    if (!fuse_ln) {
        rc = launch_ln_fwd("head.ln_fwd", ln, g.slabs, st);
        if (rc) return rc;
    }

    FcFwdArgs f = zeroed<FcFwdArgs>();
    if (fuse_ln) f.ln = ln;
    f.ts = make_taps(saved + pl.sv_yln, d->c0, 1, d->N, g.T1, g.T1, 1, g.rows);
    f.W1p = ws + pl.ws_W1p; f.b1 = P->fc1_b; f.w2 = P->fc2_w; f.b2 = P->fc2_b; f.hd = saved + pl.sv_hd; f.out = out;
    f.KCH = d->c0 / 16; f.c1 = d->c1; f.training = d->training && d->droprate > 0.f;
    f.keep_scale = 1.0f / (1.0f - d->droprate); f.thresh = drop_thresh(d->droprate); f.seed = seed; f.offset = offset;
// ... 19 lines not shown
}

int stgcn_outblock_backward_hook(const stgcn_outblock_desc* d, const stgcn_outblock_params* P, const float* x, const float* dout,
                                 const float* saved, float* ws, const stgcn_outblock_grads* G, float* dx, const stgcn_ln_hook* dx_hook,
                                 void* stream) {
    return outblock_backward_impl(d, P, x, dout, nullptr, saved, ws, G, dx, dx_hook, stream);
}

int stgcn_outblock_backward_loss(const stgcn_outblock_desc* d, const stgcn_outblock_params* P, const float* x, const stgcn_head_loss* hl,
                                 const float* saved, float* ws, const stgcn_outblock_grads* G, float* dx, const stgcn_ln_hook* dx_hook,
                                 void* stream) {
    if (!hl || !hl->pred || !hl->target) return fail(STGCN_ERR_INVALID, "stgcn_outblock_backward_loss: NULL pred / target");
    if (!G || !G->loss) return fail(STGCN_ERR_INVALID, "stgcn_outblock_backward_loss: grads->loss is NULL");
    const int rc = check_loss_kind("stgcn_outblock_backward_loss", hl->kind, hl->delta);
    if (rc) return rc;
    if (hl->target_window_dev && !hl->target_index_dev)
        return fail(STGCN_ERR_INVALID, "stgcn_outblock_backward_loss: target_window_dev (window table) needs target_index_dev != NULL");
    return outblock_backward_impl(d, P, x, nullptr, hl, saved, ws, G, dx, dx_hook, stream);
}

namespace {
int adamw_step_impl(const stgcn_adamw_tensor* tensors, int32_t count, float lr, float beta1, float beta2, float eps, float weight_decay,
                    int64_t step, const int64_t* step_dev, const float* lr_dev, const double* clip_state, void* stream) {
    STGCN_FLUSH_PENDING_PACK();
    if (count < 0 || (count > 0 && !tensors)) return fail(STGCN_ERR_INVALID, "stgcn_adamw_step: bad tensor table");
    hipStream_t st = (hipStream_t)stream;
    for (int off = 0; off < count; off += kAdamwMaxTensors) {
        AdamwArgs a = zeroed<AdamwArgs>();
        const int n = count - off < kAdamwMaxTensors ? count - off : kAdamwMaxTensors;
        for (int i = 0; i < n; ++i) {
            const stgcn_adamw_tensor& t = tensors[off + i];
            if (!t.param || !t.grad || !t.exp_avg || !t.exp_avg_sq || t.numel < 0) return fail(STGCN_ERR_INVALID, "stgcn_adamw_step: NULL pointer in entry %d", off + i);
            a.t[i].p = t.param; a.t[i].g = t.grad; a.t[i].m = t.exp_avg; a.t[i].v = t.exp_avg_sq; a.t[i].n = (long)t.numel;
            a.start[i + 1] = a.start[i] + cdiv(t.numel, kAdamwChunk);
        }
        a.count = n; a.lr = lr; a.b1 = beta1; a.b2 = beta2; a.eps = eps; a.wd = weight_decay; a.step = (long)step;
        a.lb1 = (float)log((double)beta1); a.lb2 = (float)log((double)beta2);
        a.step_dev = reinterpret_cast<const long*>(step_dev); a.lr_dev = lr_dev;
        g_prof_tag = 0;
        if (a.start[n] > 0) {
            if (clip_state) STGCN_LAUNCH("adamw_clip", st, adamw_clip_kernel, dim3(a.start[n]), dim3(kThreads), 0, a, clip_state);
            else STGCN_LAUNCH("adamw", st, adamw_kernel, dim3(a.start[n]), dim3(kThreads), 0, a);
        }
    }
    return STGCN_OK;
}

int grad_norm_wgs(const stgcn_adamw_tensor* tensors, int off, int n) {
    long chunks = 0;
    for (int i = 0; i < n; ++i) chunks += cdiv(tensors[off + i].numel, kAdamwChunk);
    return chunks < 1 ? 1 : (chunks > kClipMaxWgs ? kClipMaxWgs : (int)chunks);
}
int grad_clip_words_impl(const stgcn_adamw_tensor* tensors, int32_t count, const char* who, int64_t* words) {
    if (count < 0 || (count > 0 && !tensors)) return fail(STGCN_ERR_INVALID, "%s: bad tensor table", who);
    int wgs = 1;
    for (int off = 0; off < count; off += kAdamwMaxTensors) {
        const int n = count - off < kAdamwMaxTensors ? count - off : kAdamwMaxTensors;
        for (int i = 0; i < n; ++i)
            if (tensors[off + i].numel < 0) return fail(STGCN_ERR_INVALID, "%s: negative numel in entry %d", who, off + i);
        const int w = grad_norm_wgs(tensors, off, n);
        wgs = w > wgs ? w : wgs;
    }
    *words = STGCN_CLIP_HDR_WORDS + wgs;
    return STGCN_OK;
}
int check_clip(const stgcn_grad_clip* c, int64_t need, const char* who) {
    if (!c || !c->state) return fail(STGCN_ERR_INVALID, "%s: NULL clip state", who);
    if (!(c->max_norm > 0.f)) return fail(STGCN_ERR_INVALID, "%s: max_norm = %g must be > 0", who, (double)c->max_norm);
    if (c->state_words < need)
        return fail(STGCN_ERR_INVALID, "%s: a clip state of %lld words is too small, %lld needed", who, (long long)c->state_words, (long long)need);
    return STGCN_OK;
}
}

int stgcn_adamw_step(const stgcn_adamw_tensor* tensors, int32_t count, float lr, float beta1, float beta2, float eps,
                     float weight_decay, int64_t step, const int64_t* step_dev, const float* lr_dev, void* stream) {
    return adamw_step_impl(tensors, count, lr, beta1, beta2, eps, weight_decay, step, step_dev, lr_dev, nullptr, stream);
}

int stgcn_grad_flush(int32_t n_blocks, const stgcn_flush_block* blocks, const stgcn_outblock_desc* head_desc,
                     const stgcn_outblock_grads* head_grads, float* head_ws, const stgcn_adamw_tensor* opt, int32_t opt_count,
                     const stgcn_adamw_hyper* hyper, void* stream) {
    STGCN_FLUSH_PENDING_PACK();
    if (opt_count < 0 || (opt_count > 0 && (!opt || !hyper))) return fail(STGCN_ERR_INVALID, "stgcn_grad_flush: optimizer table without hyper-parameters");
    ReduceList RL;
    int rc = flush_job_list(RL, "stgcn_grad_flush", n_blocks, blocks, head_desc, head_grads, head_ws, opt, opt_count, true);
    if (rc) return rc;
    if (opt_count > 0) {
        RL.ra.lr = hyper->lr; RL.ra.b1 = hyper->beta1; RL.ra.b2 = hyper->beta2; RL.ra.eps = hyper->eps; RL.ra.wd = hyper->weight_decay;
        RL.ra.lb1 = (float)log((double)hyper->beta1); RL.ra.lb2 = (float)log((double)hyper->beta2);
        RL.ra.step = (long)hyper->step; RL.ra.step_dev = reinterpret_cast<const long*>(hyper->step_dev); RL.ra.lr_dev = hyper->lr_dev;
    }
    g_prof_tag = 0;
    return launch_reduce_list(opt_count > 0 ? "reduce_adamw" : "reduce_all", RL, (hipStream_t)stream);
}

namespace {
int optim_step_impl(const char* who, const stgcn_adamw_tensor* tensors, int32_t count, const stgcn_optim_hyper* hyper, const double* clip_state,
                    void* stream) {
    if (hyper->kind == STGCN_OPT_ADAMW)
        return adamw_step_impl(tensors, count, (float)hyper->lr, (float)hyper->beta1, (float)hyper->beta2, (float)hyper->eps, (float)hyper->weight_decay,
                               hyper->step, hyper->step_dev, hyper->lr_dev, clip_state, stream);
    STGCN_FLUSH_PENDING_PACK();
    if (count < 0 || (count > 0 && !tensors)) return fail(STGCN_ERR_INVALID, "%s: bad tensor table", who);
    const bool lion = hyper->kind == STGCN_OPT_LION;
    hipStream_t st = (hipStream_t)stream;
    for (int off = 0; off < count; off += kAdamwMaxTensors) {
        AdamwArgs a = zeroed<AdamwArgs>();
        const int n = count - off < kAdamwMaxTensors ? count - off : kAdamwMaxTensors;
        for (int i = 0; i < n; ++i) {
            const stgcn_adamw_tensor& t = tensors[off + i];
            if (!t.param || !t.grad || !t.exp_avg || (!lion && !t.exp_avg_sq) || t.numel < 0)
                return fail(STGCN_ERR_INVALID, "%s: NULL pointer in entry %d", who, off + i);
            a.t[i].p = t.param; a.t[i].g = t.grad; a.t[i].m = t.exp_avg; a.t[i].v = lion ? nullptr : t.exp_avg_sq; a.t[i].n = (long)t.numel;
            a.start[i + 1] = a.start[i] + cdiv(t.numel, kAdamwChunk);
        }
        a.count = n; a.lr = (float)hyper->lr; a.b1 = (float)hyper->beta1; a.b2 = (float)hyper->beta2; a.eps = (float)hyper->eps;
        a.wd = (float)hyper->weight_decay; a.step = (long)hyper->step;
        a.lb1 = (float)log(hyper->beta1); a.lb2 = (float)log(hyper->beta2);
        a.step_dev = reinterpret_cast<const long*>(hyper->step_dev); a.lr_dev = hyper->lr_dev;
        OptimExtra x = optim_extra(hyper);
        int first = -1;
        for (int i = 0; off == 0 && i < n && first < 0; ++i)
            if (a.t[i].n > 0) first = i;
        x.mu_job = first;
        g_prof_tag = 0;
        if (a.start[n] > 0) {
            if (clip_state) {
                if (lion) STGCN_LAUNCH("lion_clip", st, optim_clip_kernel<kOptLion>, dim3(a.start[n]), dim3(kThreads), 0, a, x, clip_state);
                else STGCN_LAUNCH("nadamw_clip", st, optim_clip_kernel<kOptNadamw>, dim3(a.start[n]), dim3(kThreads), 0, a, x, clip_state);
            } else if (lion) STGCN_LAUNCH("lion", st, optim_kernel<kOptLion>, dim3(a.start[n]), dim3(kThreads), 0, a, x);
            else STGCN_LAUNCH("nadamw", st, optim_kernel<kOptNadamw>, dim3(a.start[n]), dim3(kThreads), 0, a, x);
        }
    }
    return STGCN_OK;
}
}

int stgcn_optim_step(const stgcn_adamw_tensor* tensors, int32_t count, const stgcn_optim_hyper* hyper, void* stream) {
    const int rc = check_optim_hyper(hyper, "stgcn_optim_step");
    if (rc) return rc;
    return optim_step_impl("stgcn_optim_step", tensors, count, hyper, nullptr, stream);
}

int stgcn_grad_clip_words(const stgcn_adamw_tensor* tensors, int32_t count, int64_t* words) {
    if (!words) return fail(STGCN_ERR_INVALID, "stgcn_grad_clip_words: words is NULL");
    return grad_clip_words_impl(tensors, count, "stgcn_grad_clip_words", words);
}

int stgcn_grad_norm(const stgcn_adamw_tensor* tensors, int32_t count, const stgcn_grad_clip* clip, void* stream) {
    STGCN_FLUSH_PENDING_PACK();
    int64_t need = 0;
    int rc = grad_clip_words_impl(tensors, count, "stgcn_grad_norm", &need);
    if (rc) return rc;
    rc = check_clip(clip, need, "stgcn_grad_norm");
    if (rc) return rc;
    for (int i = 0; i < count; ++i)
        if (!tensors[i].grad && tensors[i].numel > 0) return fail(STGCN_ERR_INVALID, "stgcn_grad_norm: NULL gradient in entry %d", i);
    hipStream_t st = (hipStream_t)stream;
    const int launches = count > 0 ? cdiv(count, kAdamwMaxTensors) : 1;
    for (int l = 0; l < launches; ++l) {
        const int off = l * kAdamwMaxTensors;
        AdamwArgs a = zeroed<AdamwArgs>();
        const int n = count - off < kAdamwMaxTensors ? count - off : kAdamwMaxTensors;
        for (int i = 0; i < n; ++i) {
            a.t[i].g = tensors[off + i].grad; a.t[i].n = (long)tensors[off + i].numel;
            a.start[i + 1] = a.start[i] + cdiv(tensors[off + i].numel, kAdamwChunk);
        }
        a.count = n;
        ClipArgs c;
        c.state = clip->state; c.max_norm = clip->max_norm; c.first = l == 0; c.last = l == launches - 1;
        g_prof_tag = 0;
        STGCN_LAUNCH("grad_norm", st, grad_norm_kernel, dim3(grad_norm_wgs(tensors, off, n)), dim3(kThreads), (kThreads / 64) * sizeof(double), a, c);
    }
    return STGCN_OK;
}

int stgcn_optim_step_clip(const stgcn_adamw_tensor* tensors, int32_t count, const stgcn_optim_hyper* hyper, const stgcn_grad_clip* clip,
                          void* stream) {
    int rc = check_optim_hyper(hyper, "stgcn_optim_step_clip");
    if (rc) return rc;
    int64_t need = 0;
    rc = grad_clip_words_impl(tensors, count, "stgcn_optim_step_clip", &need);
    if (rc) return rc;
    rc = check_clip(clip, need, "stgcn_optim_step_clip");
    if (rc) return rc;
    return optim_step_impl("stgcn_optim_step_clip", tensors, count, hyper, clip->state, stream);
}

int stgcn_grad_flush_clip_words(int32_t n_blocks, const stgcn_flush_block* blocks, const stgcn_outblock_desc* head_desc,
                                const stgcn_outblock_grads* head_grads, float* head_ws, int64_t* words) {
    if (!words) return fail(STGCN_ERR_INVALID, "stgcn_grad_flush_clip_words: words is NULL");
    ReduceList RL;
    const int rc = flush_job_list(RL, "stgcn_grad_flush_clip_words", n_blocks, blocks, head_desc, head_grads, head_ws, nullptr, 0, false);
    if (rc) return rc;
    *words = STGCN_CLIP_HDR_WORDS + (RL.ra.start[RL.nj] > 1 ? RL.ra.start[RL.nj] : 1);
    return STGCN_OK;
}

int stgcn_grad_flush_clip(int32_t n_blocks, const stgcn_flush_block* blocks, const stgcn_outblock_desc* head_desc,
                          const stgcn_outblock_grads* head_grads, float* head_ws, const stgcn_grad_clip* clip, void* stream) {
    STGCN_FLUSH_PENDING_PACK();
    ReduceList RL;
    int rc = flush_job_list(RL, "stgcn_grad_flush_clip", n_blocks, blocks, head_desc, head_grads, head_ws, nullptr, 0, false);
    if (rc) return rc;
    if (RL.overflow) return fail(STGCN_ERR_INVALID, "stgcn_grad_flush_clip: more than %d reduction jobs in one launch", kMaxReduceJobs);
    if (RL.nj == 0 || RL.ra.start[RL.nj] < 1) return fail(STGCN_ERR_INVALID, "stgcn_grad_flush_clip: nothing to flush");
    rc = check_clip(clip, STGCN_CLIP_HDR_WORDS + (int64_t)RL.ra.start[RL.nj], "stgcn_grad_flush_clip");
    if (rc) return rc;
    RL.ra.njobs = RL.nj;
    ReduceClipArgs a = zeroed<ReduceClipArgs>();
    static_cast<ReduceArgs&>(a) = RL.ra;
    a.c.state = clip->state; a.c.max_norm = clip->max_norm; a.c.first = 1; a.c.last = 1;
    a.skip_job = -1;
    for (int k = 0; k < RL.nj; ++k)
        if (head_desc && head_grads->loss && RL.ra.job[k].dst == head_grads->loss) a.skip_job = k;
    g_prof_tag = 0;
    STGCN_LAUNCH("reduce_norm", (hipStream_t)stream, reduce_kernel<kOptNorm>, dim3(RL.ra.start[RL.nj]), dim3(kThreads), kThreads * 4 * sizeof(float), a);
    return STGCN_OK;
}

int stgcn_grad_flush_optim(int32_t n_blocks, const stgcn_flush_block* blocks, const stgcn_outblock_desc* head_desc,
                           const stgcn_outblock_grads* head_grads, float* head_ws, const stgcn_adamw_tensor* opt, int32_t opt_count,
                           const stgcn_optim_hyper* hyper, void* stream) {
    int rc = check_optim_hyper(hyper, "stgcn_grad_flush_optim");
    if (rc) return rc;
    if (hyper->kind == STGCN_OPT_ADAMW) {
        stgcn_adamw_hyper h = zeroed<stgcn_adamw_hyper>();
        h.lr = (float)hyper->lr; h.beta1 = (float)hyper->beta1; h.beta2 = (float)hyper->beta2; h.eps = (float)hyper->eps;
        h.weight_decay = (float)hyper->weight_decay; h.step = hyper->step; h.step_dev = hyper->step_dev; h.lr_dev = hyper->lr_dev;
        return stgcn_grad_flush(n_blocks, blocks, head_desc, head_grads, head_ws, opt, opt_count, &h, stream);
    }
    STGCN_FLUSH_PENDING_PACK();
    if (opt_count < 1 || !opt) return fail(STGCN_ERR_INVALID, "stgcn_grad_flush_optim: empty optimizer table");
    const bool lion = hyper->kind == STGCN_OPT_LION;
    ReduceList RL;
    rc = flush_job_list(RL, "stgcn_grad_flush_optim", n_blocks, blocks, head_desc, head_grads, head_ws, opt, opt_count, !lion);
    if (rc) return rc;
    if (RL.overflow) return fail(STGCN_ERR_INVALID, "stgcn_grad_flush_optim: more than %d reduction jobs in one launch", kMaxReduceJobs);
    RL.ra.lr = (float)hyper->lr; RL.ra.b1 = (float)hyper->beta1; RL.ra.b2 = (float)hyper->beta2; RL.ra.eps = (float)hyper->eps;
    RL.ra.wd = (float)hyper->weight_decay; RL.ra.lb1 = (float)log(hyper->beta1); RL.ra.lb2 = (float)log(hyper->beta2);
    RL.ra.step = (long)hyper->step; RL.ra.step_dev = reinterpret_cast<const long*>(hyper->step_dev); RL.ra.lr_dev = hyper->lr_dev;
    OptimExtra x = optim_extra(hyper);
    for (int k = 0; k < RL.nj && x.mu_job < 0; ++k)
        if (RL.ra.job[k].p && (long)RL.ra.job[k].n0 * RL.ra.job[k].n1 * RL.ra.job[k].n2 > 0) x.mu_job = k;
    if (lion)
        for (int k = 0; k < RL.nj; ++k) RL.ra.job[k].v = nullptr;
    g_prof_tag = 0;
    return launch_reduce_list_optim(lion ? "reduce_lion" : "reduce_nadamw", RL, hyper->kind, x, (hipStream_t)stream);
}

int stgcn_loss_grad(int32_t kind, float delta, const float* pred, const float* target, int64_t n, float grad_scale, float* loss, float* dpred,
                    const int64_t* target_index_dev, int64_t target_index_stride, const int64_t* target_window_dev, int64_t window_floats,
                    void* stream) {
    STGCN_FLUSH_PENDING_PACK();
    int rc = check_loss_kind("stgcn_loss_grad", kind, delta);
    if (rc) return rc;
    if (!pred || !target || !loss || !dpred || n < 1) return fail(STGCN_ERR_INVALID, "stgcn_loss_grad: NULL buffer or n < 1");
    if (target_window_dev) {
        if (!target_index_dev) return fail(STGCN_ERR_INVALID, "stgcn_loss_grad: target_window_dev (window table) needs target_index_dev != NULL");
        if (window_floats < 1 || n % window_floats != 0 || n >= (1ll << 31))
            return fail(STGCN_ERR_INVALID, "stgcn_loss_grad: n = %lld must be a multiple of window_floats = %lld and below 2^31", (long long)n,
                        (long long)window_floats);
    }
    g_prof_tag = 0;
    const char* label = kind == STGCN_LOSS_MSE ? "mse_loss_grad" : "loss_grad";
    STGCN_LAUNCH(label, (hipStream_t)stream, loss_grad_kernel, dim3(1), dim3(1024), 16 * sizeof(float), (int)kind, delta, pred, target,
                 (long)n, grad_scale, loss, dpred, reinterpret_cast<const long*>(target_index_dev), (long)target_index_stride,
                 reinterpret_cast<const long*>(target_window_dev), target_window_dev ? (unsigned)window_floats : 0u);
    return STGCN_OK;
}

int stgcn_mse_loss_grad(const float* pred, const float* target, int64_t n, float grad_scale, float* loss, float* dpred,
                        const int64_t* target_index_dev, int64_t target_index_stride, void* stream) {
    return stgcn_loss_grad(STGCN_LOSS_MSE, 0.f, pred, target, n, grad_scale, loss, dpred, target_index_dev, target_index_stride, nullptr, 0, stream);
}

int stgcn_mse_loss_grad_windows(const float* pred, const float* target, int64_t n, float grad_scale, float* loss, float* dpred,
                                const int64_t* target_index_dev, int64_t target_index_stride, const int64_t* target_window_dev,
                                int64_t window_floats, void* stream) {
    return stgcn_loss_grad(STGCN_LOSS_MSE, 0.f, pred, target, n, grad_scale, loss, dpred, target_index_dev, target_index_stride, target_window_dev,
                           window_floats, stream);
}

int stgcn_eval_arm(double* state, int64_t* pos, void* stream) {
    STGCN_FLUSH_PENDING_PACK();
    if (!state) return fail(STGCN_ERR_INVALID, "stgcn_eval_arm: state is NULL");
    g_prof_tag = 0;
    STGCN_LAUNCH("eval_arm", (hipStream_t)stream, eval_arm_kernel, dim3(1), dim3(64), 0, state, reinterpret_cast<long*>(pos));
    return STGCN_OK;
}

int stgcn_eval_accumulate(const float* pred, const float* target, int32_t B, int32_t N, const float* scale, const float* mean,
                          int64_t first_valid, int64_t* pos, int64_t target_stride, int64_t num_windows, double* state, void* stream) {
    STGCN_FLUSH_PENDING_PACK();
    if (!state) return fail(STGCN_ERR_INVALID, "stgcn_eval_accumulate: state is NULL");
    if (!pred || !target) return fail(STGCN_ERR_INVALID, "stgcn_eval_accumulate: NULL pred / target");
    if (B < 1 || N < 1) return fail(STGCN_ERR_INVALID, "stgcn_eval_accumulate: n = B * N must be positive (B=%d, N=%d)", B, N);
    if ((scale == nullptr) != (mean == nullptr)) return fail(STGCN_ERR_INVALID, "stgcn_eval_accumulate: scale and mean come together (both or neither)");
    if (first_valid < 0 || first_valid >= B)
        return fail(STGCN_ERR_INVALID, "stgcn_eval_accumulate: first_valid=%lld outside [0, B=%d)", (long long)first_valid, B);
    if (pos) {
        if (first_valid != 0) return fail(STGCN_ERR_INVALID, "stgcn_eval_accumulate: with position words first_valid is read from them (pass 0)");
        if (num_windows < B) return fail(STGCN_ERR_INVALID, "stgcn_eval_accumulate: %lld windows are fewer than one batch of %d", (long long)num_windows, B);
        if (target_stride < 0) return fail(STGCN_ERR_INVALID, "stgcn_eval_accumulate: negative target stride");
    }
    EvalAccArgs a;
    a.pred = pred; a.target = target; a.scale = scale; a.mean = mean; a.state = state;
    a.pos = reinterpret_cast<long*>(pos);
    a.tstride = (long)target_stride; a.first_valid = (long)first_valid; a.num = (long)num_windows;
    a.B = B; a.N = N;
    const long n = (long)B * N;
    int wgs = 1;
    if (n >= eval_big_threshold()) {
        wgs = cdiv(n, 2 * kEvalThreads);
        wgs = wgs < 2 ? 2 : (wgs > kEvalMaxWgs ? kEvalMaxWgs : wgs);
// ... 20 lines not shown
```

### stgcn_amd/csrc/stgcn_device.hip.h

```cpp
#pragma once
#include <hip/hip_runtime.h>
#include <stdint.h>
#include <type_traits>

typedef float f32x4 __attribute__((ext_vector_type(4)));

#ifdef STGCN_PHASE_TIMING
#ifdef STGCN_PHASE_WALL
#define STGCN_PHASE_CLOCK() wall_clock64()
#else
#define STGCN_PHASE_CLOCK() clock64()
#endif
__device__ long long stgcn_phase_buf[4096 * 16];
__device__ int stgcn_phase_kid;
#define STGCN_PHASE(kid, i)                                                                                     \
    do {                                                                                                        \
        if (stgcn_phase_kid == (kid) && threadIdx.x == 0 && blockIdx.y == 0 && blockIdx.x < 4096)                \
            stgcn_phase_buf[blockIdx.x * 16 + (i)] = STGCN_PHASE_CLOCK();                                       \
    } while (0)
#define STGCN_ACC_DECL() long long stgcn_acc_ = 0, stgcn_t0_ = 0, stgcn_acc2_ = 0, stgcn_t2_ = 0
#define STGCN_ACC_BEGIN() stgcn_t0_ = clock64()
#define STGCN_ACC_END() stgcn_acc_ += clock64() - stgcn_t0_
#define STGCN_ACC2_BEGIN() stgcn_t2_ = clock64()
#define STGCN_ACC2_END() stgcn_acc2_ += clock64() - stgcn_t2_
#define STGCN_ACC_STORE(kid, i, cond)                                                                           \
    do {                                                                                                        \
        if (stgcn_phase_kid == (kid) && (cond) && blockIdx.x < 4096) stgcn_phase_buf[blockIdx.x * 16 + (i)] = stgcn_acc_; \
    } while (0)
#define STGCN_ACC2_STORE(kid, i, cond)                                                                          \
    do {                                                                                                        \
        if (stgcn_phase_kid == (kid) && (cond) && blockIdx.x < 4096) stgcn_phase_buf[blockIdx.x * 16 + (i)] = stgcn_acc2_; \
    } while (0)
#else
#define STGCN_PHASE(kid, i) ((void)0)
#define STGCN_ACC_DECL() ((void)0)
#define STGCN_ACC_BEGIN() ((void)0)
#define STGCN_ACC_END() ((void)0)
#define STGCN_ACC_STORE(kid, i, cond) ((void)0)
#define STGCN_ACC2_BEGIN() ((void)0)
#define STGCN_ACC2_END() ((void)0)
#define STGCN_ACC2_STORE(kid, i, cond) ((void)0)
#endif

namespace stgcn {

constexpr int kThreads = 256;
constexpr int kTileRows = 64;
#ifndef STGCN_GC_RING1
#define STGCN_GC_RING1 2
#endif
constexpr int gc_ring(int maxq) { return maxq <= 1 ? STGCN_GC_RING1 : 2; }
constexpr int kSegMax = 128;

#ifndef STGCN_TS_DBG
#define STGCN_TS_DBG 0
#endif
__device__ __forceinline__ f32x4 mfma4(float a, float b, f32x4 c) {
#if STGCN_TS_DBG == 2
    asm volatile("" ::"v"(a), "v"(b));
    return c;
#else
    return __builtin_amdgcn_mfma_f32_16x16x4f32(a, b, c, 0, 0, 0);
#endif
}
__device__ __forceinline__ f32x4 ld4(const float* p) { return *reinterpret_cast<const f32x4*>(p); }
#if STGCN_TS_DBG
__device__ __forceinline__ f32x4 dbg_opaque4() {
    f32x4 v;
    asm volatile("v_mov_b32 %0, 0\n\tv_mov_b32 %1, 0\n\tv_mov_b32 %2, 0\n\tv_mov_b32 %3, 0" : "=v"(v[0]), "=v"(v[1]), "=v"(v[2]), "=v"(v[3]));
    return v;
}
__device__ __forceinline__ void dbg_keep4(f32x4 v) { asm volatile("" ::"v"(v[0]), "v"(v[1]), "v"(v[2]), "v"(v[3])); }
#endif
__device__ __forceinline__ void st4(float* p, f32x4 v) { *reinterpret_cast<f32x4*>(p) = v; }
#ifndef STGCN_WT_STORES
#define STGCN_WT_STORES 1
#endif
__device__ __forceinline__ void st4_wt(float* p, f32x4 v) {
#if STGCN_WT_STORES && defined(__HIP_DEVICE_COMPILE__)
    asm volatile("global_store_dwordx4 %0, %1, off sc1\n\ts_nop 1" ::"v"(p), "v"(v) : "memory");
#else
    st4(p, v);
#endif
}
__device__ __forceinline__ void st4_wt2(float* p, f32x4 v) {
#if STGCN_WT_STORES >= 2 && defined(__HIP_DEVICE_COMPILE__)
    asm volatile("global_store_dwordx4 %0, %1, off sc1\n\ts_nop 1" ::"v"(p), "v"(v) : "memory");
#else
    st4(p, v);
#endif
}
__device__ __forceinline__ void glds16(const void* g, void* lds_base) {
    __builtin_amdgcn_global_load_lds((const __attribute__((address_space(1))) void*)g, (__attribute__((address_space(3))) void*)lds_base, 16, 0, 0);
}
__device__ __forceinline__ f32x4 zero4() {
    f32x4 z = {0.f, 0.f, 0.f, 0.f};
    return z;
}

struct bf16 { unsigned short v; };
struct f32x { float v; };
typedef unsigned int u32x2_t __attribute__((ext_vector_type(2)));
typedef __bf16 bf16x8 __attribute__((ext_vector_type(8)));
typedef short s16x4 __attribute__((ext_vector_type(4)));

__device__ __forceinline__ unsigned bf16_bits_rne(float x) {
    const unsigned u = __builtin_bit_cast(unsigned, x);
    if ((u & 0x7fffffffu) > 0x7f800000u) return (u >> 16) | 0x40u;
    return (u + 0x7fffu + ((u >> 16) & 1u)) >> 16;
}
__device__ __forceinline__ unsigned pack_bf16x2(float a, float b) {
#if defined(__HIP_DEVICE_COMPILE__)
    typedef float f32x2_ __attribute__((ext_vector_type(2)));
    typedef __bf16 bf16x2_ __attribute__((ext_vector_type(2)));
    const f32x2_ v = {a, b};
    return __builtin_bit_cast(unsigned, __builtin_convertvector(v, bf16x2_));
#else
    return bf16_bits_rne(a) | (bf16_bits_rne(b) << 16);
#endif
}
__device__ __forceinline__ u32x2_t pack_bf16x4(f32x4 v) {
    u32x2_t r;
    r[0] = pack_bf16x2(v[0], v[1]);
    r[1] = pack_bf16x2(v[2], v[3]);
    return r;
}
__device__ __forceinline__ f32x4 unpack_bf16x4(u32x2_t r) {
    f32x4 v;
    v[0] = __builtin_bit_cast(float, r[0] << 16);
    v[1] = __builtin_bit_cast(float, r[0] & 0xffff0000u);
    v[2] = __builtin_bit_cast(float, r[1] << 16);
    v[3] = __builtin_bit_cast(float, r[1] & 0xffff0000u);
    return v;
}
__device__ __forceinline__ float bf16_round(float x) { return __builtin_bit_cast(float, bf16_bits_rne(x) << 16); }

template <typename ET> __device__ __forceinline__ const ET* et_ptr(const float* p) { return reinterpret_cast<const ET*>(p); }
template <typename ET> __device__ __forceinline__ ET* et_ptr(float* p) { return reinterpret_cast<ET*>(p); }

#if STGCN_TS_DBG == 1
__device__ __forceinline__ f32x4 ldx4(const float* p) { (void)p; return dbg_opaque4(); }
#else
__device__ __forceinline__ f32x4 ldx4(const float* p) { return ld4(p); }
#endif
__device__ __forceinline__ f32x4 ldx4(const f32x* p) { return ld4(reinterpret_cast<const float*>(p)); }
__device__ __forceinline__ void stx4(f32x* p, f32x4 v) { st4(reinterpret_cast<float*>(p), v); }
__device__ __forceinline__ float ldx1(const f32x* p) { return p->v; }
__device__ __forceinline__ void stx1(f32x* p, float v) { p->v = v; }
// ... 597 lines not shown
```

### stgcn_amd/csrc/stgcn_kernels_bwd.hip.h

```cpp
#pragma once
#include <stdlib.h>
#include <string.h>
#include "stgcn_device.hip.h"
#include "stgcn_kernels_fwd.hip.h"
#include "stgcn_kernels_gctile.hip.h"
#include "stgcn_kernels_tstep.hip.h"
#include "stgcn_kernels_thin.hip.h"

namespace stgcn {

struct LnBwdArgs {
    const float* dy;
    const float* y;
    const float* beta;
    const float* U;
    const float* S;
    const float* gamma;
    const float* mean;
    const float* rstd;
    float2* rowstat;
    float2* slabconst;
    float* dZ;
    float* dgam_part;
    float* dbet_part;
// ... 878 lines not shown
            const long R = row0 + row;
            f32x4 h = zero4(), du = zero4(), dq = zero4();
            if (R < a.rows) {
                const f32x4 dh = ld4(Ht + row * LDH + 4 * c4);
                f32x4 u = bu, qv = bqv;
#pragma unroll
                for (int k = 0; k < kThinK; ++k) {
                    if (k < K) {
                        const float xv = xt[row * LDX + k];
#pragma unroll
                        for (int i = 0; i < 4; ++i) {
                            u[i] = fmaf(xv, wpr[k][i], u[i]);
                            qv[i] = fmaf(xv, wqr[k][i], qv[i]);
                        }
                    }
                }
#pragma unroll
                for (int i = 0; i < 4; ++i) {
                    const float sg = sigmoid_f(qv[i]);
                    float du_, dq_;
                    gate_bwd(dh[i], u[i], sg, a.act, du_, dq_);
                    du[i] = du_;
                    dq[i] = dq_;
                    h[i] = gate_fwd(u[i], sg, a.act);
                }
                if (a.dZ) {
                    stx4_wt(dZ_ + (size_t)R * NC + 4 * c4, du);
                    stx4_wt(dZ_ + (size_t)R * NC + c0 + 4 * c4, dq);
                }
            }
            st4(Ht + row * LDH + 4 * c4, h);
            st4(Zt + row * LDZ + 4 * c4, du);
            st4(Zt + row * LDZ + c0 + 4 * c4, dq);
        }
        __syncthreads();
        for (int r = 0; r < zrows; ++r) zsum += Zt[(zpart * zrows + r) * LDZ + zcol];
#pragma unroll
        for (int i = 0; i < 4; ++i) {
            const int rbase = i * 16 + 4 * g;
            if constexpr (std::is_same<ET, float>::value) {
#pragma unroll
                for (int sx = 0; sx < 4; ++sx) {
                    const int row = rbase + sx;
                    wacc = mfma4(Ht[row * LDH + wave * 16 + l15], dAt[row * LDA + l15], wacc);
                    const float xa = xt[row * LDX + l15];
                    gacc[0] = mfma4(xa, Zt[row * LDZ + (2 * wave) * 16 + l15], gacc[0]);
                    gacc[1] = mfma4(xa, Zt[row * LDZ + (2 * wave + 1) * 16 + l15], gacc[1]);
                }
            } else {
                wacc = MM::mma(MM::cvt(gather4(Ht + rbase * LDH + wave * 16 + l15, LDH)), MM::cvt(gather4(dAt + rbase * LDA + l15, LDA)), wacc);
                MM::mma_b2(MM::cvt(gather4(xt + rbase * LDX + l15, LDX)), MM::cvt(gather4(Zt + rbase * LDZ + (2 * wave) * 16 + l15, LDZ)),
                           MM::cvt(gather4(Zt + rbase * LDZ + (2 * wave + 1) * 16 + l15, LDZ)), gacc[0], gacc[1]);
            }
        }
    }
    const int pstride = c0 * 16 + 16 + 16 * NC + NC;
    float* part = a.part + (size_t)blockIdx.x * pstride;
#pragma unroll
    for (int r = 0; r < 4; ++r) {
        part[(wave * 16 + 4 * g + r) * 16 + l15] = wacc[r];
        part[c0 * 16 + 16 + (4 * g + r) * NC + (2 * wave) * 16 + l15] = gacc[0][r];
        part[c0 * 16 + 16 + (4 * g + r) * NC + (2 * wave + 1) * 16 + l15] = gacc[1][r];
    }
    __syncthreads();
    red[tid] = bsum;
    __syncthreads();
    if (tid < 16) {
        float sacc = 0.f;
        for (int rg = 0; rg < 16; ++rg) sacc += red[rg * 16 + tid];
        part[c0 * 16 + tid] = sacc;
    }
    __syncthreads();
    red[tid] = zsum;
    __syncthreads();
    if (tid < NC) {
        float sacc = 0.f;
        for (int pz = 0; pz < kThreads / NC; ++pz) sacc += red[pz * NC + tid];
        part[c0 * 16 + 16 + 16 * NC + tid] = sacc;
    }
}

template <typename ET, int ACT>
__global__ __launch_bounds__(256, 3) void thin_tc1_bwd2_kernel(ThinBwdArgs a) {
    thin_tc1_bwd2_body<ET, ACT>(a);
}

#ifndef STGCN_WGRAD_GROUPS
#define STGCN_WGRAD_GROUPS 2
#endif
constexpr int kWgradGroups = STGCN_WGRAD_GROUPS;
struct TconvBwdWeightArgs {
    TapSrc ts;
    const float* dZ;
    float* part;
    int NC, Mpad, rows_per_chunk, chunks;
};
constexpr int wgrad_step_rows(int MTW, int NTW) {
    return (size_t)kWgradGroups * 64 * ((MTW * 16 + 4) + (NTW * 64 + 4)) * sizeof(float) <= 156 * 1024 ? 64 : 32;
}
constexpr size_t wgrad_lds_bytes(int MTW, int NTW) {
    return (size_t)kWgradGroups * wgrad_step_rows(MTW, NTW) * ((MTW * 16 + 4) + (NTW * 64 + 4)) * sizeof(float);
}

template <int MTW, int NTW, bool VEC, typename ET>
__device__ __forceinline__ void tconv_bwd_weight_body(const TconvBwdWeightArgs& a, int flat_wg, int n_wgs, int mchunks) {
    extern __shared__ float stgcn_smem[];
    constexpr int GROUPS = kWgradGroups;
    constexpr int SR = wgrad_step_rows(MTW, NTW);
    const int grp = threadIdx.x >> 8, tid = threadIdx.x & 255;
    const int wave = tid >> 6, lane = tid & 63, g = lane >> 4, l15 = lane & 15;
    constexpr int MC = MTW * 16, LDC = MC + 4;
    constexpr int NC = NTW * 64, LDZ = NC + 4;
    float* ct = stgcn_smem + grp * (SR * LDC + SR * LDZ);
    float* zt = ct + SR * LDC;
    const int item = xcd_item(flat_wg, n_wgs);
    const int chunk = item / mchunks, mchunk = item % mchunks, m0 = mchunk * MC;
    const long crow0 = (long)chunk * a.rows_per_chunk;
    long crow1 = crow0 + a.rows_per_chunk;
    if (crow1 > a.ts.rows) crow1 = a.ts.rows;
    const int nsteps = (int)((crow1 - crow0 + SR - 1) / SR);
    const int nit = (nsteps + GROUPS - 1) / GROUPS;
    const int K = a.ts.taps * a.ts.C;
    const unsigned per_b = (unsigned)(a.ts.Tdst * a.ts.N);
    const int csh = pow2_shift(a.ts.C);
    const ET* const xsrc = tap_origin<ET>(a.ts);
    const ET* const dZ_ = et_ptr<ET>(a.dZ);
    const TapWin tw = tap_win(a.ts);

    constexpr int NCR = (SR * (MC / 4) + kThreads - 1) / kThreads;
    constexpr int NCS = (SR * MC + kThreads - 1) / kThreads;
    constexpr int NZ = SR * NTW * 16 / kThreads;
    Raw4<ET> creg[VEC ? NCR : 1], zreg[NZ];
    float cs[VEC ? 1 : NCS];
    auto load_regs = [&](int step) {
        const long r0 = crow0 + (long)step * SR;
        if constexpr (VEC) {
#pragma unroll
            for (int i = 0; i < NCR; ++i) {
                const int idx = tid + i * kThreads;
                const int r = idx / (MC / 4), q = idx - r * (MC / 4);
                Raw4<ET> v;
                v.v = {};
                if (r < SR) {
                    const long R = r0 + r;
                    const int kidx = m0 + 4 * q;
                    if (R < crow1 && kidx < K) {
                        const unsigned Ru = (unsigned)R, b = Ru / per_b, rem = Ru - b * per_b;
                        const int tap = fast_div(kidx, a.ts.C, csh), ch = kidx - tap * a.ts.C;
                        v = ldraw4(xsrc + (tap_src_row(tw, b, rem) + (size_t)tap * a.ts.N) * a.ts.C + ch);
                    }
                }
                creg[i] = v;
            }
        } else {
#pragma unroll
            for (int i = 0; i < NCS; ++i) {
                const int idx = tid + i * kThreads;
                const int r = idx / MC, q = idx - r * MC;
                float v = 0.f;
                if (r < SR) {
                    const long R = r0 + r;
                    const int kidx = m0 + q;
                    if (R < crow1 && kidx < K) {
                        const unsigned Ru = (unsigned)R, b = Ru / per_b, rem = Ru - b * per_b;
                        const int tap = fast_div(kidx, a.ts.C, csh), ch = kidx - tap * a.ts.C;
                        v = ldx1(xsrc + (tap_src_row(tw, b, rem) + (size_t)tap * a.ts.N) * a.ts.C + ch);
                    }
                }
                cs[i] = v;
            }
        }
#pragma unroll
        for (int z = 0; z < NZ; ++z) {
            const int idx = tid + z * kThreads;
            const int r = idx / (NC / 4), q = idx - r * (NC / 4);
            const long R = r0 + r;
            zreg[z].v = {};
            if (R < crow1) zreg[z] = ldraw4(dZ_ + (size_t)R * NC + 4 * q);
        }
    };
    auto store_regs = [&]() {
        if constexpr (VEC) {
#pragma unroll
            for (int i = 0; i < NCR; ++i) {
                const int idx = tid + i * kThreads;
                const int r = idx / (MC / 4), q = idx - r * (MC / 4);
                if (r < SR) st4(ct + r * LDC + 4 * q, cvt4(creg[i]));
            }
        } else {
#pragma unroll
            for (int i = 0; i < NCS; ++i) {
                const int idx = tid + i * kThreads;
                const int r = idx / MC, q = idx - r * MC;
                if (r < SR) ct[r * LDC + q] = cs[i];
            }
        }
#pragma unroll
        for (int z = 0; z < NZ; ++z) {
            const int idx = tid + z * kThreads;
            const int r = idx / (NC / 4), q = idx - r * (NC / 4);
            st4(zt + r * LDZ + 4 * q, cvt4(zreg[z]));
        }
    };

    f32x4 acc[MTW][NTW];
#pragma unroll
    for (int i = 0; i < MTW; ++i)
#pragma unroll
        for (int j = 0; j < NTW; ++j) acc[i][j] = zero4();
    constexpr int tpc = kThreads / NC, rpt = SR / tpc;
    const int bcol = tid % NC, bpart = tid / NC;
    float bsum = 0.f;

    STGCN_PHASE(3, 0);
    if (grp < nsteps) load_regs(grp);
    STGCN_PHASE(3, 1);
    for (int it = 0; it < nit; ++it) {
        const int step = it * GROUPS + grp;
// ... 12 lines not shown
            if constexpr (std::is_same<ET, float>::value) {
#pragma unroll
                for (int sx = 0; sx < 4; ++sx) {
                    const int row = k16 * 16 + 4 * g + sx;
                    float av[MTW], bv[NTW];
#pragma unroll
                    for (int i = 0; i < MTW; ++i) av[i] = ct[row * LDC + i * 16 + l15];
#pragma unroll
                    for (int j = 0; j < NTW; ++j) bv[j] = zt[row * LDZ + (wave * NTW + j) * 16 + l15];
#pragma unroll
                    for (int i = 0; i < MTW; ++i)
#pragma unroll
                        for (int j = 0; j < NTW; ++j) acc[i][j] = mfma4(av[i], bv[j], acc[i][j]);
                }
            } else {
                const int row = k16 * 16 + 4 * g;
                typename Mma<ET>::frag fa[MTW], fb[NTW];
#pragma unroll
                for (int i = 0; i < MTW; ++i) fa[i] = Mma<ET>::cvt(gather4(ct + row * LDC + i * 16 + l15, LDC));
#pragma unroll
                for (int j = 0; j < NTW; ++j) fb[j] = Mma<ET>::cvt(gather4(zt + row * LDZ + (wave * NTW + j) * 16 + l15, LDZ));
#pragma unroll
                for (int i = 0; i < MTW; ++i)
#pragma unroll
                    for (int j = 0; j < NTW; ++j) acc[i][j] = Mma<ET>::mma(fa[i], fb[j], acc[i][j]);
            }
        }
    }
    STGCN_PHASE(3, 2);
    if (GROUPS > 1) {
        float* xb = stgcn_smem;
        for (int q = 1; q < GROUPS; ++q) {
            __syncthreads();
            if (grp == q) {
#pragma unroll
                for (int i = 0; i < MTW; ++i)
#pragma unroll
                    for (int j = 0; j < NTW; ++j) st4(xb + ((i * NTW + j) * kThreads + tid) * 4, acc[i][j]);
                xb[MTW * NTW * kThreads * 4 + tid] = bsum;
            }
            __syncthreads();
            if (grp == 0) {
#pragma unroll
                for (int i = 0; i < MTW; ++i)
#pragma unroll
                    for (int j = 0; j < NTW; ++j) acc[i][j] += ld4(xb + ((i * NTW + j) * kThreads + tid) * 4);
                bsum += xb[MTW * NTW * kThreads * 4 + tid];
            }
        }
    }
    float* part = a.part + (size_t)chunk * a.Mpad * NC;
    if (grp == 0) {
#pragma unroll
        for (int i = 0; i < MTW; ++i)
#pragma unroll
            for (int j = 0; j < NTW; ++j)
                st4_wt(part + (size_t)((wave * NTW + j) * 16 + l15) * a.Mpad + m0 + i * 16 + 4 * g, acc[i][j]);
    }
    if (mchunk == 0) {
        float* bp = a.part + (size_t)a.chunks * a.Mpad * NC + (size_t)chunk * NC;
        if (tpc == 1) {
            if (grp == 0) bp[bcol] = bsum;
        } else {
            __syncthreads();
            if (grp == 0) stgcn_smem[tid] = bsum;
            __syncthreads();
            if (grp == 0 && tid < NC) {
                float s = 0.f;
                for (int p = 0; p < tpc; ++p) s += stgcn_smem[p * NC + tid];
                bp[tid] = s;
            }
        }
    }
    STGCN_PHASE(3, 3);
}
template <int MTW, int NTW, bool VEC, typename ET>
__global__ __launch_bounds__(256 * kWgradGroups) void tconv_bwd_weight_kernel(TconvBwdWeightArgs a) {
    tconv_bwd_weight_body<MTW, NTW, VEC, ET>(a, (int)(blockIdx.y * gridDim.x + blockIdx.x), (int)(gridDim.x * gridDim.y), (int)gridDim.y);
}
template <int MTW1, int NTW1, int MTW2, int NTW2, typename ET>
__global__ __launch_bounds__(256 * kWgradGroups) void wgrad_pair_kernel(TconvBwdWeightArgs a1, int n1, int mc1, TconvBwdWeightArgs a2, int n2, int mc2) {
    if ((int)blockIdx.x < n1) tconv_bwd_weight_body<MTW1, NTW1, true, ET>(a1, (int)blockIdx.x, n1, mc1);
    else tconv_bwd_weight_body<MTW2, NTW2, true, ET>(a2, (int)blockIdx.x - n1, n2, mc2);
}

enum { kOptAdamw = 0, kOptNadamw = 1, kOptLion = 2, kOptNorm = 3 };
struct OptimExtra {
    float omb1, omb2;
    float mu_k;
    float mu_prod;
    float* mu_dev;
    int mu_job;
};
struct OptimScalars {
    float decay, lr;
    float rbc2, cg, cm;
    float mu_prod;
};
template <int KIND>
__device__ __forceinline__ OptimScalars optim_scalars(float t, float lr, float b1, float lb2, float wd, const OptimExtra& x) {
#pragma clang fp contract(off)
    OptimScalars s;
    s.lr = lr;
    s.decay = fmaf(-lr, wd, 1.0f);
    s.rbc2 = s.cg = s.cm = s.mu_prod = 0.f;
    if (KIND == kOptNadamw) {
        const float mu = b1 * (1.0f - 0.5f * expf(t * x.mu_k)), mu_next = b1 * (1.0f - 0.5f * expf((t + 1.0f) * x.mu_k));
        const float prev = x.mu_dev ? x.mu_dev[((long)t - 1) & 1] : x.mu_prod;
        s.mu_prod = prev * mu;
        s.rbc2 = -expm1f(t * lb2);
        s.cg = -lr * (1.0f - mu) / (1.0f - s.mu_prod);
        s.cm = -lr * mu_next / (1.0f - s.mu_prod * mu_next);
    }
    return s;
}
__device__ __forceinline__ void nadamw_element(float g, float& p, float& m, float& v, float b2, float eps, const OptimScalars& s, const OptimExtra& x) {
#pragma clang fp contract(off)
    const float pd = p * s.decay;
    m = fmaf(x.omb1, g - m, m);
    v = fmaf(x.omb2 * g, g, v * b2);
    const float d = sqrtf(v / s.rbc2) + eps;
    const float p1 = pd + (s.cg * g) / d;
    p = p1 + (s.cm * m) / d;
}
__device__ __forceinline__ void lion_element(float g, float& p, float& m, float b1, float b2, const OptimScalars& s, const OptimExtra& x) {
#pragma clang fp contract(off)
    const float pd = p * s.decay;
    const float c = m * b1 + g * x.omb1;
    const float sg = c > 0.f ? 1.0f : (c < 0.f ? -1.0f : 0.0f);
    p = pd - s.lr * sg;
    m = fmaf(g, x.omb2, m * b2);
}

struct ReduceJob {
    const float* src;
    float* dst;
    float* p;
    float* m;
    float* v;
    long pstride;
    int P;
    int vec;
    int dvec;
    int slices;
    int n0, n1, n2;
    int s0, s1, s2;
    int t0, t1, t2;
};
constexpr int kMaxReduceJobs = 32;
struct ReduceArgs {
    ReduceJob job[kMaxReduceJobs];
    int start[kMaxReduceJobs + 1];
    int njobs;
    float lr, b1, b2, eps, wd, lb1, lb2;
    long step;
    const long* step_dev;
    const float* lr_dev;
};
struct ReduceOptimArgs : ReduceArgs {
    OptimExtra x;
};
static_assert(sizeof(ReduceOptimArgs) <= 4096, "reduce_kernel arguments exceed 4 KiB");
struct ReduceClipArgs : ReduceArgs {
    ClipArgs c;
    int skip_job;
};
// ... 142 lines not shown
```

### stgcn_amd/csrc/stgcn_kernels_thin.hip.h

```cpp
#pragma once
#include <type_traits>
#include "stgcn_device.hip.h"
#include "stgcn_kernels_fwd.hip.h"

namespace stgcn {

constexpr int kThinTaps = 4;

__device__ __forceinline__ size_t thin_row_base(const TapWin& tw, long R, unsigned per_b, long start) {
    const unsigned Ru = (unsigned)R, b = Ru / per_b, rem = Ru - b * per_b;
    return tap_src_row(tw, b, rem, start);
}
__device__ __forceinline__ long thin_row_start(const TapWin& tw, long t, long tiles, long rows, int l15, unsigned per_b) {
    if (!tw.tab) return 0;
    const long R0 = (t < tiles ? t : tiles - 1) * 16 + l15, R = R0 < rows ? R0 : rows - 1;
    return tap_win_start(tw, (unsigned)R / per_b);
}

__device__ __forceinline__ float thin_weff(const float* cw, int C, int Kt, int k, int o) {
    if (k >= Kt * C) return 0.f;
    const int tap = k / C, ch = k - tap * C;
    float v = cw[((size_t)o * C + ch) * Kt + tap];
    if (tap == Kt - 1 && o == ch) v += 1.0f;
    return v;
// ... 83 lines not shown
        for (int mt = 0; mt < 8; ++mt) bz[mt] = a.cb ? ld4(a.cb + 16 * mt + 4 * g) : zero4();
#pragma unroll
        for (int kc = 0; kc < 4; ++kc) waf[kc] = MM::cvt(ld4(a.aw + (size_t)l15 * 64 + 16 * kc + 4 * g));
        ba4 = a.ab ? ld4(a.ab + 4 * g) : zero4();
    } else {
        cw.load(a.Wd, K, g, l15);
#pragma unroll
        for (int mt = 0; mt < 8; ++mt) bz[mt] = ld4(a.bias + 16 * mt + 4 * g);
#pragma unroll
        for (int kc = 0; kc < 4; ++kc) waf[kc] = MM::cvt(ld4(a.Wap + ((size_t)kc * 64 + lane) * 4));
        ba4 = ld4(a.ba + 4 * g);
    }

    const bool shared_idx = sy.on && a.ts.idx_dev == sy.idx_ptr;
    const ET* xsrc = shared_idx ? et_ptr<ET>(a.ts.src) : tap_origin<ET>(a.ts);
    TapWin tw = shared_idx ? tap_win_at(a.ts, 0) : tap_win(a.ts);
    if (shared_idx) {
        const long old = (long)chain_ld64(reinterpret_cast<const unsigned long long*>(a.ts.idx_dev));
        chain_drain_stores();
        if (lane == 0) chain_add(g_pack_readers + (int)(wave_id & (kPackSyncWords - 1)) * kPackSyncStride, 1u);
        const long v = old + sy.inc, pos = sy.mod > 0 ? v % sy.mod : v;
        if (a.ts.win_tab) tw = tap_win_at(a.ts, pos);
        else xsrc = et_ptr<ET>(a.ts.src) + pos * a.ts.idx_stride;
    }
    auto request = [&](long t, long start, Raw1<ET> (&xr)[kThinTaps]) __attribute__((always_inline)) {
        const long R0 = (t < tiles ? t : tiles - 1) * 16 + l15, R = R0 < rows ? R0 : rows - 1;
        const size_t base = thin_row_base(tw, R, per_b, start);
#pragma unroll
        for (int k = 0; k < kThinTaps; ++k) {
            const int kk = k < K ? k : K - 1, tap = kk / C, ch = kk - tap * C;
            xr[k] = ldraw1(xsrc + (base + (size_t)tap * N) * C + ch);
        }
    };
    Raw1<ET> xn[kThinTaps];
    const long ws0 = thin_row_start(tw, wave_id, tiles, rows, l15, per_b);
    long ws1 = thin_row_start(tw, wave_id + nwaves, tiles, rows, l15, per_b);
    request(wave_id, ws0, xn);
    for (long t = wave_id; t < tiles; t += nwaves) {
        f32x4 xk;
#pragma unroll
        for (int k = 0; k < kThinTaps; ++k) xk[k] = k < K ? cvt1(xn[k]) : 0.f;
        const long ws2 = thin_row_start(tw, t + 2 * nwaves, tiles, rows, l15, per_b);
        request(t + nwaves, ws1, xn);
        ws1 = ws2;
        f32x4 acc[8];
#pragma unroll
        for (int mt = 0; mt < 8; ++mt) acc[mt] = bz[mt];
        cw.run(xk, g, acc);
        f32x4 out = zero4();
#pragma unroll
        for (int kc = 0; kc < 4; ++kc) {
            f32x4 h;
#pragma unroll
            for (int s = 0; s < 4; ++s) h[s] = gate_fwd(acc[kc][s], sigmoid_f(acc[4 + kc][s]), ACT);
            out = MM::mma(waf[kc], MM::cvt(h), out);
        }
        const long R = t * 16 + l15;
        if (R < rows) stx4_wt(A_ + (size_t)R * 16 + 4 * g, out + ba4);
    }
}

template <typename ET, int ACT>
__global__ __launch_bounds__(256) void thin_tc1_fwd_kernel(ThinFwdArgs a) {
    thin_tc1_fwd_body<ET, ACT>(a, (int)blockIdx.x, (int)gridDim.x, PackSync{0, nullptr, 0u, 0, 0});
}
template <typename ET, int ACT>
__global__ __launch_bounds__(256) void pack_thin_fwd_kernel(PackArgs p, ThinFwdArgs t, int n_thin, PackSync sy) {
#ifdef STGCN_DIAG_FUSE
    if (STGCN_DIAG_FUSE == 1 && (int)blockIdx.x >= n_thin) return;
    if (STGCN_DIAG_FUSE == 2 && (int)blockIdx.x < n_thin) return;
#endif
    if ((int)blockIdx.x < n_thin) thin_tc1_fwd_body<ET, ACT>(t, (int)blockIdx.x, n_thin, sy);
    else pack_body(p, (int)blockIdx.x - n_thin, sy);
}

struct ThinBwdArgs;

constexpr int kThinLdT = 68, kThinLdD = 20, kThinLdX = 16;
constexpr int kThinWaveLds = 16 * kThinLdT + 16 * kThinLdD + 16 * kThinLdX + 128 + 4 * 256;
inline size_t thin_bwd2_lds_bytes() { return (size_t)4 * kThinWaveLds * sizeof(float); }
static_assert(4 * kThinWaveLds >= 2 * 12 * 64 * 4 + 2 * 16, "the end-of-kernel combine reuses the waves' tiles");

template <typename ET, int ACT, typename ARGS>
__device__ __forceinline__ void thin_tc1_bwd2_body(const ARGS& a) {
    typedef Mma<ET> MM;
    constexpr bool kF32 = sizeof(ET) == 4;
    typedef typename std::conditional<kF32, float, bf16>::type ST;
    extern __shared__ float stgcn_smem[];
    const int wave = threadIdx.x >> 6, lane = threadIdx.x & 63, g = lane >> 4, l15 = lane & 15;
    float* const Tt = stgcn_smem + wave * kThinWaveLds;
    float* const Dt = Tt + 16 * kThinLdT;
    float* const Xt = Dt + 16 * kThinLdD;
    float* const Bs = Xt + 16 * kThinLdX;
    float* const Ws = Bs + 128;
    const long wave_id = (long)blockIdx.x * 4 + wave, nwaves = (long)gridDim.x * 4;
    const long rows = a.rows, tiles = (rows + 15) >> 4;
    const int K = a.ts.taps * a.ts.C, C = a.ts.C, N = a.ts.N;
    const unsigned per_b = (unsigned)(a.ts.Tdst * N);
    const TapWin tw = tap_win(a.ts);
    const ST* const xsrc = tap_origin<ST>(a.ts);
    const ST* const dA_ = et_ptr<ST>(a.dA);
    ST* const dZ_ = et_ptr<ST>(a.dZ);

    ThinConv<ST> cw;
    cw.load(a.Wd, K, g, l15);
    {
        const f32x4 b0 = ld4(a.bias + 4 * (lane & 31));
        f32x4 wf[4];
#pragma unroll
        for (int mt = 0; mt < 4; ++mt) wf[mt] = ld4(a.WaT + ((size_t)mt * 64 + lane) * 4);
        if (lane < 32) st4(Bs + 4 * lane, b0);
#pragma unroll
        for (int mt = 0; mt < 4; ++mt) st4(Ws + (mt * 64 + lane) * 4, wf[mt]);
        for (int i = lane; i < 16 * kThinLdX; i += 64) Xt[i] = 0.f;
    }
    wave_lds_sync();

    f32x4 accW[8], accA[4], dba = zero4();
#pragma unroll
    for (int i = 0; i < 8; ++i) accW[i] = zero4();
#pragma unroll
    for (int i = 0; i < 4; ++i) accA[i] = zero4();

    struct Req { Raw4<ST> da; Raw1<ST> x[kThinTaps]; };
    auto request = [&](long t, long start, Req& q) __attribute__((always_inline)) {
        const long R0 = (t < tiles ? t : tiles - 1) * 16 + l15, R = R0 < rows ? R0 : rows - 1;
        q.da = ldraw4(dA_ + (size_t)R * 16 + 4 * g);
        const size_t base = thin_row_base(tw, R, per_b, start);
#pragma unroll
        for (int k = 0; k < kThinTaps; ++k) {
            const int kk = k < K ? k : K - 1, tap = kk / C, ch = kk - tap * C;
            q.x[k] = ldraw1(xsrc + (base + (size_t)tap * N) * C + ch);
        }
    };
    Req rq;
    const long ws0 = thin_row_start(tw, wave_id, tiles, rows, l15, per_b);
    long ws1 = thin_row_start(tw, wave_id + nwaves, tiles, rows, l15, per_b);
    request(wave_id, ws0, rq);
    for (long t = wave_id; t < tiles; t += nwaves) {
        const long R = t * 16 + l15;
        const bool rv = R < rows;
        const f32x4 da = rv ? cvt4(rq.da) : zero4();
        f32x4 xk;
#pragma unroll
        for (int k = 0; k < kThinTaps; ++k) xk[k] = k < K ? cvt1(rq.x[k]) : 0.f;
        const long ws2 = thin_row_start(tw, t + 2 * nwaves, tiles, rows, l15, per_b);
        request(t + nwaves, ws1, rq);
        ws1 = ws2;
        dba += da;
        st4(Dt + l15 * kThinLdD + 4 * g, da);
        Xt[l15 * kThinLdX + g] = g < K ? (g == 0 ? xk[0] : g == 1 ? xk[1] : g == 2 ? xk[2] : xk[3]) : (g == K ? 1.f : 0.f);
        if (g == 0) Xt[l15 * kThinLdX + 4] = K == 4 ? 1.f : 0.f;
        f32x4 z[8];
#pragma unroll
        for (int mt = 0; mt < 8; ++mt) z[mt] = ld4(Bs + 16 * mt + 4 * g);
        cw.run(xk, g, z);
        {
            const typename MM::frag db = MM::cvt(da);
#pragma unroll
            for (int mt = 0; mt < 4; ++mt) {
                const f32x4 dh = MM::mma(MM::cvt(ld4(Ws + (mt * 64 + lane) * 4)), db, zero4());
                f32x4 hq;
#pragma unroll
                for (int s = 0; s < 4; ++s) {
                    const float u = z[mt][s], sg = sigmoid_f(z[4 + mt][s]);
                    float du, dq;
                    gate_bwd(dh[s], u, sg, ACT, du, dq);
                    hq[s] = gate_fwd(u, sg, ACT);
                    z[mt][s] = du;
                    z[4 + mt][s] = dq;
                }
                st4(Tt + l15 * kThinLdT + 16 * mt + 4 * g, hq);
            }
        }
        if (a.dZ && rv) {
#pragma unroll
            for (int mt = 0; mt < 8; ++mt) stx4_wt(dZ_ + (size_t)R * 128 + 16 * mt + 4 * g, z[mt]);
        }
        wave_lds_sync();
        {
            const typename MM::frag bd = MM::cvt(gather4(Dt + (4 * g) * kThinLdD + l15, kThinLdD));
#pragma unroll
            for (int ct = 0; ct < 4; ++ct)
                accA[ct] = MM::mma(MM::cvt(gather4(Tt + (4 * g) * kThinLdT + 16 * ct + l15, kThinLdT)), bd, accA[ct]);
        }
        const typename MM::frag bx = MM::cvt(gather4(Xt + (4 * g) * kThinLdX + l15, kThinLdX));
#pragma unroll
        for (int half = 0; half < 2; ++half) {
            wave_lds_sync();
#pragma unroll
            for (int mt = 0; mt < 4; ++mt) st4(Tt + l15 * kThinLdT + 16 * mt + 4 * g, z[4 * half + mt]);
            wave_lds_sync();
#pragma unroll
            for (int mt = 0; mt < 4; ++mt)
                accW[4 * half + mt] = MM::mma(MM::cvt(gather4(Tt + (4 * g) * kThinLdT + 16 * mt + l15, kThinLdT)), bx, accW[4 * half + mt]);
        }
        wave_lds_sync();
    }
#pragma unroll
    for (int i = 0; i < 4; ++i) {
        float v = dba[i];
        v += __shfl_xor(v, 1); v += __shfl_xor(v, 2); v += __shfl_xor(v, 4); v += __shfl_xor(v, 8);
        dba[i] = v;
    }
    f32x4* const cmb = reinterpret_cast<f32x4*>(stgcn_smem);
    float* const cmb_ba = stgcn_smem + 2 * 12 * 64 * 4;
    __syncthreads();
    if (wave >= 2) {
#pragma unroll
        for (int i = 0; i < 8; ++i) cmb[((wave - 2) * 12 + i) * 64 + lane] = accW[i];
#pragma unroll
        for (int i = 0; i < 4; ++i) cmb[((wave - 2) * 12 + 8 + i) * 64 + lane] = accA[i];
        if (l15 == 0) st4(cmb_ba + (wave - 2) * 16 + 4 * g, dba);
    }
    __syncthreads();
    if (wave < 2) {
#pragma unroll
        for (int i = 0; i < 8; ++i) accW[i] += cmb[(wave * 12 + i) * 64 + lane];
#pragma unroll
        for (int i = 0; i < 4; ++i) accA[i] += cmb[(wave * 12 + 8 + i) * 64 + lane];
        dba += ld4(cmb_ba + wave * 16 + 4 * g);
    }
    __syncthreads();
    if (wave == 1) {
#pragma unroll
        for (int i = 0; i < 8; ++i) cmb[i * 64 + lane] = accW[i];
#pragma unroll
        for (int i = 0; i < 4; ++i) cmb[(8 + i) * 64 + lane] = accA[i];
        if (l15 == 0) st4(cmb_ba + 4 * g, dba);
    }
    __syncthreads();
    if (wave != 0) return;
#pragma unroll
    for (int i = 0; i < 8; ++i) accW[i] += cmb[i * 64 + lane];
#pragma unroll
    for (int i = 0; i < 4; ++i) accA[i] += cmb[(8 + i) * 64 + lane];
    dba += ld4(cmb_ba + 4 * g);
    constexpr int c0 = 64, NC = 128;
    float* const part = a.part + (size_t)blockIdx.x * (c0 * 16 + 16 + 16 * NC + NC);
#pragma unroll
    for (int ct = 0; ct < 4; ++ct)
#pragma unroll
        for (int r = 0; r < 4; ++r) part[(16 * ct + 4 * g + r) * 16 + l15] = accA[ct][r];
    if (l15 == 0) st4(part + c0 * 16 + 4 * g, dba);
    if (l15 < K) {
#pragma unroll
        for (int mt = 0; mt < 8; ++mt) st4(part + c0 * 16 + 16 + (size_t)l15 * NC + 16 * mt + 4 * g, accW[mt]);
    } else if (l15 == K) {
#pragma unroll
        for (int mt = 0; mt < 8; ++mt) st4(part + c0 * 16 + 16 + 16 * NC + 16 * mt + 4 * g, accW[mt]);
    }
}

}
```

### stgcn_amd/csrc/stgcn_route.h

```cpp
#pragma once
#include <stdio.h>
#include <stdlib.h>
#include "../../include/stgcn_hip.h"

namespace stgcn {

inline int64_t rup(int64_t v, int64_t m) { return (v + m - 1) / m * m; }
inline int cdiv(int64_t a, int64_t b) { return (int)((a + b - 1) / b); }

inline int env_int(const char* name, int unset) {
    const char* e = getenv(name);
    return e ? atoi(e) : unset;
}
inline bool env_not_zero(const char* name) {
    const char* e = getenv(name);
    return !(e && e[0] == '0');
}
enum FuseBit { FUSE_TC2_BWD = 1, FUSE_TC2_LN_FWD = 2, FUSE_ROWSTATS = 4, FUSE_TC1_BWD = 8, FUSE_TC1_FWD = 16, FUSE_HEAD_LN_FWD = 32, FUSE_HEAD_LN_BWD = 64 };
inline int fuse_mask() { static const int m = env_int("STGCN_FUSE", 0x7fffffff); return m; }
inline bool thin_wave_tiles() { return env_not_zero("STGCN_THIN"); }
inline bool mfma_x6() { return env_not_zero("STGCN_MFMA_X6"); }
inline bool hook_mask_from_y() {
    const char* e = getenv("STGCN_HOOK_MASK");
    return !(e && e[0] == 'p');
}
inline FILE* launch_log_file() { static FILE* f = getenv("STGCN_LAUNCH_LOG") ? fopen(getenv("STGCN_LAUNCH_LOG"), "w") : nullptr; return f; }
inline bool tconv4_off() { static const bool off = env_int("STGCN_TCONV4", 1) == 0; return off; }
inline int head_fc_tile_knob() {
    const char* e = getenv("STGCN_HEAD_FC_TILE");
    return !e ? 0 : atoi(e) == 32 ? 32 : 16;
}
inline int head_fuse_mode() {
#if !STGCN_WT_STORES
    return 0;
#else
    return env_int("STGCN_HEAD_FUSE", 1);
#endif
}
inline int ln_stats_min_chunks() { static const int v = env_int("STGCN_LN_STATS_MIN_CHUNKS", 8); return v; }
inline int force_tconv_tile_rows() { static const int v = env_int("STGCN_TCONV_TR", 0); return v; }
inline int force_gemm_ntw() { static const int v = env_int("STGCN_GEMM_NTW", 0); return v; }
inline int force_gemm_bf16_bk() { static const int v = env_int("STGCN_GEMM_BF16_BK", 0); return v; }
inline int gemm_big_bk() { static const int v = env_int("STGCN_GEMM_BIG_BK", 64) == 32 ? 32 : 64; return v; }
inline int force_bwd_data_waves() { static const int v = env_int("STGCN_BWD_DATA_WAVES", 0); return v; }
inline int force_gcbwd2_parts() { return env_int("STGCN_GCBWD2_PARTS", 0); }
inline void gc_parts_override(int& fwd, int& bwd) {
    static int f = 0, b = 0, init = 0;
    if (!init) {
        init = 1;
        const char* e = getenv("STGCN_GC_PARTS");
        if (e) sscanf(e, "%d,%d", &f, &b);
    }
    if (f > 0) fwd = f;
    if (b > 0) bwd = b;
}
inline bool reduce_log() { static const bool on = getenv("STGCN_REDUCE_LOG") != nullptr; return on; }
inline long eval_big_threshold() { const char* e = getenv("STGCN_EVAL_BIG"); return e ? atol(e) : 32768; }

inline int g_debug_stages = 0;
inline int g_tc1_bwd_wgs = 0;
inline int runtime_cus() {
    static int cus = 0;
    if (!cus) {
        int dev = 0;
        if (hipGetDevice(&dev) != hipSuccess || hipDeviceGetAttribute(&cus, hipDeviceAttributeMultiprocessorCount, dev) != hipSuccess || cus <= 0) cus = 256;
    }
    return cus;
}
inline int device_cus() { return g_tc1_bwd_wgs > 0 ? g_tc1_bwd_wgs : runtime_cus(); }
constexpr int kTc2LnMaxPeers = 4;
inline int g_tc2ln_peers = 0;
inline int tc2_ln_peers(int N, long slabs2) {
    const int tiles = (N + 15) / 16;
    int pp = 1;
    if (g_tc2ln_peers > 0) pp = g_tc2ln_peers;
    else if (4 * slabs2 <= device_cus()) pp = 4;
    else if (2 * slabs2 <= device_cus()) pp = 2;
    if (N > 384) pp = 1;
    while (pp > 1 && tiles < 2 * pp) pp >>= 1;
    return pp;
}
inline bool tc2_ln_fwd_fused_ok(int c1, int c2, int Kt, int N) {
    return (fuse_mask() & FUSE_TC2_LN_FWD) && c1 == 16 && c2 == 64 && Kt >= 2 && Kt <= 4 && N <= 448 && tc2_ln_fwd_lds_bytes(Kt, N) <= 150 * 1024;
}
inline bool tc2_recompute(int dtype_bf16) { return dtype_bf16 != 0; }
inline int tc1_min_steps() { return 2; }
inline int tc1_range_wgs(long items, int steps, int per_cu) {
    const long want = (long)device_cus() * per_cu, by_steps = items * (long)steps / tc1_min_steps(), most = items > by_steps ? items : by_steps;
    return (int)(most < want ? most : want);
}
inline bool tc1_ts_shape(int c_in, int c0, int c1, int Kt) { return c0 == 64 && c1 == 16 && Kt == 3 && (c_in == 16 || c_in == 32 || c_in == 64); }
inline bool tc1_bwd_shape_ok(int c_in, int c0, int c1, int Kt) {
    return (fuse_mask() & FUSE_TC1_BWD) && tc1_ts_shape(c_in, c0, c1, Kt) && tc1_bwd_lds_bytes(c0, c_in, Kt) <= 150 * 1024;
}
inline bool tc1_fwd_shape_ok(int c_in, int c0, int c1, int Kt) { return (fuse_mask() & FUSE_TC1_FWD) && tc1_ts_shape(c_in, c0, c1, Kt); }
inline bool tc2_bwd_fused_ok(int c1, int c2, int Kt, int T1, int T2) {
    return (fuse_mask() & FUSE_TC2_BWD) && c1 == 16 && c2 == 64 && Kt >= 2 && Kt <= 4 && T1 <= kTsMaxT && tc2_bwd_lds_bytes(c2, Kt, T1, T2) <= 80 * 1024;
}

inline int g_gc_tiled_min_n = 513;
inline int g_gc_precision = 0;
inline int g_slab_gc_precision = 0;
inline int g_bwd_precision = 0;
inline long gc_operand_cols(long slabs) { return (slabs * 16 + 127) / 128 * 128; }
inline long gc_operand_alloc(long slabs) { return gc_operand_cols(slabs) + 384; }
inline int g_gc_ld_pad = 0;
inline int gc_plane_ld(int NP) { return NP + g_gc_ld_pad; }
inline bool gc_is_tiled(int N, int terms) {
    if (N >= g_gc_tiled_min_n) return true;
    const long NP = (N + 15) / 16 * 16;
    return ((long)terms * 16 * (NP + 4) + NP * 20) * (long)sizeof(float) > 160 * 1024;
}
inline int gc_padded_nodes(int N, int terms) { return gc_is_tiled(N, terms) ? (N + kGtBM - 1) / kGtBM * kGtBM : (N + 15) / 16 * 16; }

struct WgradGeom {
    int M, Mtiles, MTW, mchunks, Mpad, NC, rows_per_chunk, chunks;
    long off;
    long floats;
};
constexpr int kLnBigColgroups = 64;
struct BwdGeom {
// ... 199 lines not shown
```

### stgcn_amd/ops.py

```python
from __future__ import annotations

import ctypes as C
import os
from dataclasses import dataclass
from typing import Dict, Optional, Tuple

import torch

from . import _lib
from ._lib import (HEAD_PARAM_FIELDS, PARAM_FIELDS, AdamwHyper, AdamwTensor, FlushBlock, OutblockDesc, OutblockGrads, OutblockParams, OutblockPlan, StblockDesc,
                   StblockGrads, StblockParams, StblockPlan)


@dataclass(frozen=True)
class BlockConfig:
    Kt: int
    Ks: int
    n_vertex: int
    c_in: int
    channels: Tuple[int, int, int]
    act_func: str
    graph_conv_type: str
    droprate: float
    ln_eps: float = 1e-12
# ... 252 lines not shown
    if L.is_emulator == state.is_cuda:
        raise RuntimeError(f"evaluation state is on {state.device}, the bound library is {L.backend}")


def eval_accumulate(pred: torch.Tensor, target: torch.Tensor, state: torch.Tensor, scale: Optional[torch.Tensor] = None,
                    mean: Optional[torch.Tensor] = None, first_valid: int = 0, pos: Optional[torch.Tensor] = None, num_windows: int = 0,
                    target_stride: Optional[int] = None) -> None:
    L = _lib.lib()
    p = pred.detach()
    _check_device(p, "pred")
    _check_eval_state(L, state, pos)
    if p.dim() != 2 or not p.is_contiguous() or target.dtype != torch.float32 or not target.is_contiguous() or target.shape != p.shape:
        raise ValueError(f"eval_accumulate: contiguous float32 (B, N) tensors expected, got {tuple(p.shape)} / {tuple(target.shape)}")
    B, N = p.shape
    for t, what in ((scale, "scale"), (mean, "mean")):
        if t is not None and (t.dtype != torch.float32 or t.numel() != N or not t.is_contiguous() or t.device != p.device):
            raise ValueError(f"eval_accumulate: {what} must be {N} contiguous float32 values on {p.device}")
    L.check(L.dll.stgcn_eval_accumulate(p.data_ptr(), target.data_ptr(), B, N, _optr(scale), _optr(mean), int(first_valid), _optr(pos),
                                        N if target_stride is None else int(target_stride), int(num_windows), state.data_ptr(),
                                        _stream_of(p)), "stgcn_eval_accumulate")


def eval_metrics(words) -> dict:
    import math
    sse, sad, ssd, sy, n = (float(w) for w in words[:5])
    return {"mse": sse / n, "mae": sad / n, "rmse": math.sqrt(ssd / n), "wmape": sad / sy, "elements": int(n)}


class _PendingLoss:
    __slots__ = ("placeholder", "pred", "target", "index", "index_stride", "window", "grad_scale", "loss", "kind", "delta")


_pending_loss: Optional[_PendingLoss] = None
_VIEW_NODES = ("ViewBackward", "UnsafeViewBackward", "ReshapeAliasBackward", "UnsqueezeBackward", "SqueezeBackward", "AliasBackward")


def _head_node_of(pred: torch.Tensor):
    fn = pred.grad_fn
    while fn is not None and type(fn).__name__.startswith(_VIEW_NODES):
        nxt = [f for f, _ in fn.next_functions if f is not None]
        if len(nxt) != 1:
            return None
        fn = nxt[0]
    return fn if fn is not None and type(fn).__name__ == "_OutBlockFnBackward" else None


def loss_backward(pred: torch.Tensor, target: torch.Tensor, kind="mse", delta: float = 1.0, grad_scale: float = 1.0) -> torch.Tensor:
    global _pending_loss
    code = loss_kind_code(kind)
    p = pred.detach()
    if (_head_node_of(pred) is None or not p.is_contiguous() or p.shape != target.shape or not target.is_contiguous()
            or target.dtype != torch.float32 or os.environ.get("STGCN_FUSED_LOSS", "1") == "0"):
        loss, dpred = loss_and_grad(pred, target, code, delta, grad_scale)
        pred.backward(dpred)
        return loss
    _check_device(p, "pred")
    pl = _PendingLoss()
    pl.placeholder = torch.empty_like(p)
    pl.pred, pl.target, pl.grad_scale = p, target, float(grad_scale)
    pl.kind, pl.delta = code, float(delta)
    pl.index, pl.index_stride, pl.window = _index_of(target)
    pl.loss = torch.empty(1, dtype=torch.float32, device=p.device)
    _pending_loss = pl
    try:
        pred.backward(pl.placeholder)
        if _pending_loss is not None:
            raise RuntimeError("loss_backward: the output head did not take the fused loss (was its backward run through another path?)")
    finally:
        _pending_loss = None
    return pl.loss


def mse_backward(pred: torch.Tensor, target: torch.Tensor, grad_scale: float = 1.0) -> torch.Tensor:
    return loss_backward(pred, target, "mse", grad_scale=grad_scale)


class GradSink:

    def __init__(self, grads: Dict[torch.nn.Parameter, torch.Tensor]):
        self.by_ptr = {p.data_ptr(): g for p, g in grads.items()}
        self.blocks = []
        self.head = None
        self.owners = []

    def holds(self, wsc) -> bool:
        return any(o is wsc for o in self.owners)

    def grad_for(self, p: Optional[torch.Tensor]) -> Optional[torch.Tensor]:
        return None if p is None else self.by_ptr.get(p.data_ptr())

    def _tables(self):
        arr = (FlushBlock * max(len(self.blocks), 1))()
        for i, (desc, gst, ws, _) in enumerate(self.blocks):
            arr[i].desc, arr[i].grads, arr[i].ws = C.pointer(desc), C.pointer(gst), ws.data_ptr()
        hd = hg = hws = None
        if self.head is not None:
            hd, hg, hws = C.byref(self.head[0]), C.byref(self.head[1]), self.head[2].data_ptr()
        return arr, hd, hg, hws

    def clip_words(self) -> int:
        L = _lib.lib()
        arr, hd, hg, hws = self._tables()
        w = C.c_int64(0)
        L.check(L.dll.stgcn_grad_flush_clip_words(len(self.blocks), arr, hd, hg, hws, C.byref(w)), "stgcn_grad_flush_clip_words")
        return int(w.value)

    def flush(self, opt_table=None, hyper: Optional[AdamwHyper | _lib.OptimHyper] = None, stream: Optional[int] = None, clip=None) -> None:
        L = _lib.lib()
        arr, hd, hg, hws = self._tables()
        n_opt = 0 if opt_table is None else len(opt_table)
        if clip is not None:
            assert opt_table is None and hyper is None, "the clipping flush is reduce-only: the update follows as stgcn_optim_step_clip"
            L.check(L.dll.stgcn_grad_flush_clip(len(self.blocks), arr, hd, hg, hws, C.byref(clip), stream), "stgcn_grad_flush_clip")
        elif isinstance(hyper, _lib.OptimHyper):
            L.check(L.dll.stgcn_grad_flush_optim(len(self.blocks), arr, hd, hg, hws, opt_table, n_opt, C.byref(hyper), stream),
                    "stgcn_grad_flush_optim")
        else:
            L.check(L.dll.stgcn_grad_flush(len(self.blocks), arr, hd, hg, hws, opt_table, n_opt, None if hyper is None else C.byref(hyper), stream),
                    "stgcn_grad_flush")
        self.blocks, self.head = [], None
        for o in self.owners:
            o.pending_sink = None
        self.owners = []


_sink: Optional[GradSink] = None


class grad_sink_scope:
    def __init__(self, sink: Optional[GradSink]):
        self.sink = sink

    def __enter__(self):
        global _sink
        self.prev, _sink = _sink, self.sink
        return self.sink

    def __exit__(self, *exc):
        global _sink
        _sink = self.prev
        return False


_chain = 0


def current_chain() -> int:
    return _chain


class chain_scope:

    def __init__(self, c: int):
        self.c = int(c)

    def __enter__(self):
        global _chain
        self.prev, _chain = _chain, self.c
        return self

    def __exit__(self, *exc):
        global _chain
        _chain = self.prev
        return False


# ... 280 lines not shown
def _head_struct(cls, tensors):
    s = cls()
    for name, t in zip(HEAD_PARAM_FIELDS, tensors):
        setattr(s, name, None if t is None else t.data_ptr())
    return s


class _OutBlockFn(torch.autograd.Function):

    @staticmethod
    def forward(ctx, x_cl, cfg: HeadConfig, training: bool, seed: int, offset: int, offset_dev, wsc: WorkspaceCache, *params):
        L = _lib.lib()
        B, T, N, c_in = x_cl.shape
        need_dx = bool(x_cl.requires_grad)
        desc = make_head_desc(cfg, B, T, training, need_dx, prepacked=wsc.take_prepacked(), dtype=x_cl.dtype)
        plan = query_head_plan(desc)
        dev = x_cl.device
        ps = [None if p is None else p.detach() for p in params]
        out = torch.empty(B, plan.T1, N, dtype=torch.float32, device=dev)
        saved = torch.empty(plan.saved_floats, dtype=torch.float32, device=dev)
        ws = wsc.get(plan.ws_floats, dev)
        pst = _head_struct(OutblockParams, ps)
        L.check(L.dll.stgcn_outblock_forward(C.byref(desc), C.byref(pst), x_cl.data_ptr(), out.data_ptr(), saved.data_ptr(), ws.data_ptr(),
                                             seed, offset, _optr(offset_dev), _stream_of(x_cl)), "stgcn_outblock_forward")
        ctx.in_hook = _take_ln_hook(x_cl) if need_dx else None
        ctx.save_for_backward(x_cl, saved, *[p for p in params if p is not None])
        ctx.param_present = [p is not None for p in params]
        ctx.param_needs_grad = [p is not None and p.requires_grad for p in params]
        ctx.cfg, ctx.training, ctx.ws, ctx.need_dx, ctx.wsc = cfg, training, ws, need_dx, wsc
        return out

    @staticmethod
    def backward(ctx, dout):
        L = _lib.lib()
        x_cl, saved, *present = ctx.saved_tensors
        it = iter(present)
        params = [next(it) if pr else None for pr in ctx.param_present]
        cfg = ctx.cfg
        B, T, N, c_in = x_cl.shape
        sink = _sink
        desc = make_head_desc(cfg, B, T, ctx.training, ctx.need_dx, defer=sink is not None, dtype=x_cl.dtype)
        dout = dout.contiguous()
        if dout.dtype != torch.float32:
            dout = dout.float()
        global _pending_loss
        fused_loss = _pending_loss if (_pending_loss is not None and _pending_loss.placeholder.data_ptr() == dout.data_ptr()) else None
        if fused_loss is not None:
            _pending_loss = None
        used = {"tc_aw": c_in > cfg.channels[0], "tc_ab": c_in > cfg.channels[0]}
        grads = []
        for name, p, need in zip(HEAD_PARAM_FIELDS, params, ctx.param_needs_grad):
            if not (p is not None and need and used.get(name, True)):
                grads.append(None)
            elif sink is not None:
                grads.append(sink.grad_for(p))
                if grads[-1] is None:
                    raise RuntimeError(f"gradient sink has no buffer for head parameter {name}")
            else:
                grads.append(torch.empty_like(p))
        dx = torch.empty_like(x_cl) if ctx.need_dx else None
        pst = _head_struct(OutblockParams, [None if p is None else p.detach() for p in params])
        gst = _head_struct(OutblockGrads, grads)
        ih = ctx.in_hook if dx is not None else None
        if fused_loss is not None:
            gst.loss = fused_loss.loss.data_ptr()
            hl = _lib.HeadLoss()
            hl.pred, hl.target = fused_loss.pred.data_ptr(), fused_loss.target.data_ptr()
            hl.target_index_dev, hl.target_index_stride, hl.grad_scale = fused_loss.index, fused_loss.index_stride, fused_loss.grad_scale
            hl.target_window_dev = fused_loss.window
            hl.kind, hl.delta = fused_loss.kind, fused_loss.delta
            ctx.keep_loss = fused_loss
            L.check(L.dll.stgcn_outblock_backward_loss(C.byref(desc), C.byref(pst), x_cl.data_ptr(), C.byref(hl), saved.data_ptr(),
                                                       ctx.ws.data_ptr(), C.byref(gst), None if dx is None else dx.data_ptr(),
                                                       None if ih is None else C.byref(ih.hook), _stream_of(x_cl)),
                    "stgcn_outblock_backward_loss")
        else:
            L.check(L.dll.stgcn_outblock_backward_hook(C.byref(desc), C.byref(pst), x_cl.data_ptr(), dout.data_ptr(), saved.data_ptr(),
                                                       ctx.ws.data_ptr(), C.byref(gst), None if dx is None else dx.data_ptr(),
                                                       None if ih is None else C.byref(ih.hook), _stream_of(x_cl)),
                    "stgcn_outblock_backward")
        if ih is not None:
            ih.mark_ready(dx)
        if sink is not None:
            sink.head = (desc, gst, ctx.ws, (grads, params))
            sink.owners.append(ctx.wsc)
            ctx.wsc.pending_sink = sink
            grads = [None] * len(grads)
        return (dx, None, None, None, None, None, None, *grads)


def block_chain_status(cfg: BlockConfig, B: int, T: int, wsc: WorkspaceCache, dtype=torch.float32) -> int:
    L = _lib.lib()
    ws = wsc.buf
    if ws is None:
        return 0
    desc = make_desc(cfg, B, T, False, False, dtype=dtype)
    w = C.c_uint32(0)
    L.check(L.dll.stgcn_stblock_chain_status(C.byref(desc), ws.data_ptr(), C.byref(w), _stream_of(ws)), "stgcn_stblock_chain_status")
    return int(w.value)


def head_chain_status(cfg: HeadConfig, B: int, T: int, wsc: WorkspaceCache, dtype=torch.float32) -> int:
    L = _lib.lib()
    ws = wsc.buf
    if ws is None:
        return 0
    desc = make_head_desc(cfg, B, T, False, False, dtype=dtype)
    w = C.c_uint32(0)
    L.check(L.dll.stgcn_outblock_chain_status(C.byref(desc), ws.data_ptr(), C.byref(w), _stream_of(ws)), "stgcn_outblock_chain_status")
    return int(w.value)


def output_block(x: torch.Tensor, cfg: HeadConfig, params, training: bool, seed: int, offset: int, wsc: WorkspaceCache,
                 offset_dev: Optional[torch.Tensor] = None) -> torch.Tensor:
    _check_device(x, "x", activation=True)
    if x.dim() != 4 or x.shape[1] != cfg.c_in or x.shape[3] != cfg.n_vertex:
        raise ValueError(f"expected input (B, {cfg.c_in}, T, {cfg.n_vertex}), got {tuple(x.shape)}")
    x_cl = x.permute(0, 2, 3, 1).contiguous()
    out = _OutBlockFn.apply(x_cl, cfg, training, seed, offset, offset_dev, wsc, *params)
    return out.unsqueeze(1)
```

Before: 90970 windows/s.

## Defer head weight-gradient kernel to ride on first block's thin backward launch

The output head's paired temporal-conv weight-gradient work is parked instead of launched. It is then appended as extra workgroups to the first ST block's thin align/gate backward kernel, so both run in one launch. Every other entry point flushes any pending parked work, and a drop hook releases it when the gradient sink dies. This aims to remove a separate small launch and fill idle CUs during the thin backward. It adds global pending state and lifetime hazards, and the ridden wgrad uses a single-group, smaller-step variant that may be less efficient.

```diff
diff --git a/include/stgcn_hip.h b/include/stgcn_hip.h
--- a/include/stgcn_hip.h
+++ b/include/stgcn_hip.h
@@ -260,6 +260,7 @@
 int stgcn_grad_flush(int32_t n_blocks, const stgcn_flush_block* blocks, const stgcn_outblock_desc* head_desc,
                      const stgcn_outblock_grads* head_grads, float* head_ws, const stgcn_adamw_tensor* opt, int32_t opt_count,
                      const stgcn_adamw_hyper* hyper, void* stream);
+int stgcn_wgrad_ride_drop(const float* head_ws);
 
 #define STGCN_OPT_ADAMW 0
 #define STGCN_OPT_NADAMW 1
diff --git a/stgcn_amd/_lib.py b/stgcn_amd/_lib.py
--- a/stgcn_amd/_lib.py
+++ b/stgcn_amd/_lib.py
@@ -233,6 +233,11 @@
                                             C.POINTER(GradClip), C.c_void_p]
         for f in ("stgcn_grad_clip_words", "stgcn_grad_flush_clip_words", "stgcn_grad_norm", "stgcn_optim_step_clip", "stgcn_grad_flush_clip"):
             getattr(d, f).restype = C.c_int
+        if not hasattr(d, "stgcn_wgrad_ride_drop"):
+            raise StgcnError(f"{path} does not export stgcn_wgrad_ride_drop (built before the head's weight gradients rode on the first "
+                             f"layer's backward): rebuild with `python -m stgcn_amd.build --force`")
+        d.stgcn_wgrad_ride_drop.argtypes = [C.c_void_p]
+        d.stgcn_wgrad_ride_drop.restype = C.c_int
         d.stgcn_mse_loss_grad.argtypes = [C.c_void_p, C.c_void_p, C.c_int64, C.c_float, C.c_void_p, C.c_void_p, C.c_void_p, C.c_int64,
                                           C.c_void_p]
         d.stgcn_mse_loss_grad.restype = C.c_int
@@ -292,4 +297,5 @@
                     "stgcn_set_slab_gc_precision", "stgcn_outblock_backward_loss", "stgcn_set_bwd_precision", "stgcn_set_gemm_big_nt",
                     "stgcn_set_chain_spin_ticks", "stgcn_outblock_chain_status", "stgcn_set_tc2ln_peers", "stgcn_stblock_chain_status", "stgcn_prepack_park", "stgcn_prepack_flush",
                     "stgcn_optim_step", "stgcn_grad_flush_optim", "stgcn_eval_arm", "stgcn_eval_accumulate", "stgcn_loss_grad",
-                    "stgcn_grad_clip_words", "stgcn_grad_flush_clip_words", "stgcn_grad_norm", "stgcn_optim_step_clip", "stgcn_grad_flush_clip"]
+                    "stgcn_grad_clip_words", "stgcn_grad_flush_clip_words", "stgcn_grad_norm", "stgcn_optim_step_clip", "stgcn_grad_flush_clip",
+                    "stgcn_wgrad_ride_drop"]
diff --git a/stgcn_amd/csrc/stgcn_capi.hip b/stgcn_amd/csrc/stgcn_capi.hip
--- a/stgcn_amd/csrc/stgcn_capi.hip
+++ b/stgcn_amd/csrc/stgcn_capi.hip
@@ -632,6 +632,44 @@
     return STGCN_OK;
 }
 
+struct PendingWgrad {
+    bool valid = false;
+    WgradRoleArgs w;
+    const float* ws = nullptr;
+    hipStream_t st = nullptr;
+};
+thread_local PendingWgrad g_pending_wgrad;
+inline dim3 wgrad_role_grid(const WgradRoleArgs& w) { return dim3((unsigned)(w.n1 + w.n2)); }
+int flush_pending_wgrad() {
+    if (!g_pending_wgrad.valid) return STGCN_OK;
+    const int tag = g_prof_tag;
+    g_prof_tag = 0;
+    const int rc = [&]() -> int {
+        STGCN_LAUNCH("head.wgrad_role", g_pending_wgrad.st, wgrad_role_kernel, wgrad_role_grid(g_pending_wgrad.w), dim3(kThreads),
+                     wgrad_role_pair_lds_bytes(), g_pending_wgrad.w);
+        return STGCN_OK;
+    }();
+    g_prof_tag = tag;
+    if (!rc) g_pending_wgrad.valid = false;
+    return rc;
+}
+#define STGCN_FLUSH_PENDING_WGRAD()                    \
+    do {                                               \
+        const int rc_pw_ = flush_pending_wgrad();      \
+        if (rc_pw_) return rc_pw_;                     \
+    } while (0)
+int park_wgrad_pair(const TconvBwdWeightArgs& a1, const WgradGeom& w1, const TconvBwdWeightArgs& a2, const WgradGeom& w2, const float* ws,
+                    hipStream_t st) {
+    STGCN_FLUSH_PENDING_WGRAD();
+    WgradRoleArgs& w = g_pending_wgrad.w;
+    g_pending_wgrad.ws = ws;
+    w.a1 = a1; w.n1 = w1.chunks * w1.mchunks; w.mc1 = w1.mchunks;
+    w.a2 = a2; w.n2 = w2.chunks * w2.mchunks; w.mc2 = w2.mchunks;
+    g_pending_wgrad.st = st;
+    g_pending_wgrad.valid = true;
+    return STGCN_OK;
+}
+
 struct ReduceList {
     ReduceArgs ra;
     int nj;
@@ -1113,6 +1151,7 @@
 
     const bool ride = g_pending_pack.valid && d->prepacked && c.r.tc1_fwd == TC1_FWD_THIN && g_pending_pack.st == c.st;
     if (!ride) STGCN_FLUSH_PENDING_PACK();
+    STGCN_FLUSH_PENDING_WGRAD();
     if (!d->prepacked) rc = c.launch_block_pack();
     if (rc) return rc;
 
diff --git a/stgcn_amd/csrc/stgcn_capi_bwd.inc b/stgcn_amd/csrc/stgcn_capi_bwd.inc
--- a/stgcn_amd/csrc/stgcn_capi_bwd.inc
+++ b/stgcn_amd/csrc/stgcn_capi_bwd.inc
@@ -142,6 +142,13 @@
         if (!r.thin_bwd_waves) {
             const size_t lds = (size_t)(64 * 20 + 64 * (d->c0 + 4) + 64 * (2 * d->c0 + 4) + 64 * 20 + 256) * sizeof(float);
             STGCN_LAUNCH_ETB("align_gate_bwd", st, (thin_tc1_bwd_kernel<ET>), grid, blk, lds, a);
+        } else if (g_pending_wgrad.valid && g_pending_wgrad.st == st && !g_bf16 && g_bwd_precision == 0) {
+            const WgradRoleArgs& w = g_pending_wgrad.w;
+            const int n_thin = r.bg.al_wgs;
+            const dim3 gridf((unsigned)(n_thin + w.n1 + w.n2));
+            if (d->act == STGCN_ACT_GLU) STGCN_LAUNCH("align_gate_bwd", st, (thin_bwd_wgrad_kernel<0>), gridf, blk, thin_bwd2_lds_bytes(), a, n_thin, w);
+            else STGCN_LAUNCH("align_gate_bwd", st, (thin_bwd_wgrad_kernel<1>), gridf, blk, thin_bwd2_lds_bytes(), a, n_thin, w);
+            g_pending_wgrad.valid = false;
         } else if (d->act == STGCN_ACT_GLU) STGCN_LAUNCH_ETB("align_gate_bwd", st, (thin_tc1_bwd2_kernel<ET, 0>), grid, blk, thin_bwd2_lds_bytes(), a);
         else STGCN_LAUNCH_ETB("align_gate_bwd", st, (thin_tc1_bwd2_kernel<ET, 1>), grid, blk, thin_bwd2_lds_bytes(), a);
         return STGCN_OK;
diff --git a/stgcn_amd/csrc/stgcn_capi_head.inc b/stgcn_amd/csrc/stgcn_capi_head.inc
--- a/stgcn_amd/csrc/stgcn_capi_head.inc
+++ b/stgcn_amd/csrc/stgcn_capi_head.inc
@@ -181,6 +181,7 @@
                            const stgcn_head_loss* hl, const float* saved, float* ws, const stgcn_outblock_grads* G, float* dx,
                            const stgcn_ln_hook* dx_hook, void* stream) {
     STGCN_FLUSH_PENDING_PACK();
+    STGCN_FLUSH_PENDING_WGRAD();
     stgcn_outblock_plan pl;
     int rc = stgcn_outblock_plan_query(d, &pl);
     if (rc) return rc;
@@ -273,7 +274,11 @@
         if (rc) return rc;
         if (dx_hook && dx_hook->rowstat) hook_pending = true;
     }
-    rc = pair ? launch_wgrad_pair("head.wgrad_pair", wcv, g.wc, wfc, g.wf, st) : launch_bwd_weight("head.tconv_bwd_weight", wcv, g.wc, st);
+    const bool role = pair && !g_bf16 && g_bwd_precision == 0 && wgrad_ride();
+    rc = role   ? park_wgrad_pair(wcv, g.wc, wfc, g.wf, ws, st)
+         : pair ? launch_wgrad_pair("head.wgrad_pair", wcv, g.wc, wfc, g.wf, st)
+                : launch_bwd_weight("head.tconv_bwd_weight", wcv, g.wc, st);
+    if (!rc && role && !d->defer_reduce) rc = flush_pending_wgrad();
     if (rc) return rc;
     if (hook_pending) {
         rc = launch_hook_rowstats(dx_hook, dx, (long)d->B * d->T, st);
@@ -391,6 +396,7 @@
 int stgcn_outblock_forward(const stgcn_outblock_desc* d, const stgcn_outblock_params* P, const float* x, float* out, float* saved,
                            float* ws, uint64_t seed, uint64_t offset, const uint64_t* offset_dev, void* stream) {
     STGCN_FLUSH_PENDING_PACK();
+    STGCN_FLUSH_PENDING_WGRAD();
     stgcn_outblock_plan pl;
     int rc = stgcn_outblock_plan_query(d, &pl);
     if (rc) return rc;
@@ -576,6 +582,7 @@
                      const stgcn_outblock_grads* head_grads, float* head_ws, const stgcn_adamw_tensor* opt, int32_t opt_count,
                      const stgcn_adamw_hyper* hyper, void* stream) {
     STGCN_FLUSH_PENDING_PACK();
+    STGCN_FLUSH_PENDING_WGRAD();
     if (opt_count < 0 || (opt_count > 0 && (!opt || !hyper))) return fail(STGCN_ERR_INVALID, "stgcn_grad_flush: optimizer table without hyper-parameters");
     ReduceList RL;
     int rc = flush_job_list(RL, "stgcn_grad_flush", n_blocks, blocks, head_desc, head_grads, head_ws, opt, opt_count, true);
@@ -587,6 +594,11 @@
     }
     g_prof_tag = 0;
     return launch_reduce_list(opt_count > 0 ? "reduce_adamw" : "reduce_all", RL, (hipStream_t)stream);
+}
+
+int stgcn_wgrad_ride_drop(const float* head_ws) {
+    if (g_pending_wgrad.valid && g_pending_wgrad.ws == head_ws) g_pending_wgrad.valid = false;
+    return STGCN_OK;
 }
 
 namespace {
@@ -695,6 +707,7 @@
 int stgcn_grad_flush_clip(int32_t n_blocks, const stgcn_flush_block* blocks, const stgcn_outblock_desc* head_desc,
                           const stgcn_outblock_grads* head_grads, float* head_ws, const stgcn_grad_clip* clip, void* stream) {
     STGCN_FLUSH_PENDING_PACK();
+    STGCN_FLUSH_PENDING_WGRAD();
     ReduceList RL;
     int rc = flush_job_list(RL, "stgcn_grad_flush_clip", n_blocks, blocks, head_desc, head_grads, head_ws, nullptr, 0, false);
     if (rc) return rc;
@@ -726,6 +739,7 @@
         return stgcn_grad_flush(n_blocks, blocks, head_desc, head_grads, head_ws, opt, opt_count, &h, stream);
     }
     STGCN_FLUSH_PENDING_PACK();
+    STGCN_FLUSH_PENDING_WGRAD();
     if (opt_count < 1 || !opt) return fail(STGCN_ERR_INVALID, "stgcn_grad_flush_optim: empty optimizer table");
     const bool lion = hyper->kind == STGCN_OPT_LION;
     ReduceList RL;
diff --git a/stgcn_amd/csrc/stgcn_device.hip.h b/stgcn_amd/csrc/stgcn_device.hip.h
--- a/stgcn_amd/csrc/stgcn_device.hip.h
+++ b/stgcn_amd/csrc/stgcn_device.hip.h
@@ -64,6 +64,12 @@
 #endif
 }
 __device__ __forceinline__ f32x4 ld4(const float* p) { return *reinterpret_cast<const f32x4*>(p); }
+__device__ __forceinline__ int opaque_i32(int v) {
+#if defined(__HIP_DEVICE_COMPILE__)
+    asm volatile("" : "+v"(v));
+#endif
+    return v;
+}
 #if STGCN_TS_DBG
 __device__ __forceinline__ f32x4 dbg_opaque4() {
     f32x4 v;
diff --git a/stgcn_amd/csrc/stgcn_kernels_bwd.hip.h b/stgcn_amd/csrc/stgcn_kernels_bwd.hip.h
--- a/stgcn_amd/csrc/stgcn_kernels_bwd.hip.h
+++ b/stgcn_amd/csrc/stgcn_kernels_bwd.hip.h
@@ -984,7 +984,7 @@
 
 template <typename ET, int ACT>
 __global__ __launch_bounds__(256, 3) void thin_tc1_bwd2_kernel(ThinBwdArgs a) {
-    thin_tc1_bwd2_body<ET, ACT>(a);
+    thin_tc1_bwd2_body<ET, ACT>(a, (int)blockIdx.x, (int)gridDim.x);
 }
 
 #ifndef STGCN_WGRAD_GROUPS
@@ -1004,12 +1004,11 @@
     return (size_t)kWgradGroups * wgrad_step_rows(MTW, NTW) * ((MTW * 16 + 4) + (NTW * 64 + 4)) * sizeof(float);
 }
 
-template <int MTW, int NTW, bool VEC, typename ET>
+template <int MTW, int NTW, bool VEC, typename ET, int GROUPS = kWgradGroups, int SR = wgrad_step_rows(MTW, NTW)>
 __device__ __forceinline__ void tconv_bwd_weight_body(const TconvBwdWeightArgs& a, int flat_wg, int n_wgs, int mchunks) {
     extern __shared__ float stgcn_smem[];
-    constexpr int GROUPS = kWgradGroups;
-    constexpr int SR = wgrad_step_rows(MTW, NTW);
-    const int grp = threadIdx.x >> 8, tid = threadIdx.x & 255;
+    static_assert(SR % 16 == 0 && (SR * NTW * 16) % kThreads == 0, "a step is whole 16-row MFMA blocks and whole float4 rounds of dZ");
+    const int grp = threadIdx.x >> 8, tid = threadIdx.x & 255, tid_ = tid;
     const int wave = tid >> 6, lane = tid & 63, g = lane >> 4, l15 = lane & 15;
     constexpr int MC = MTW * 16, LDC = MC + 4;
     constexpr int NC = NTW * 64, LDZ = NC + 4;
@@ -1036,6 +1035,7 @@
     float cs[VEC ? 1 : NCS];
     auto load_regs = [&](int step) {
         const long r0 = crow0 + (long)step * SR;
+        const int tid = GROUPS == 1 ? opaque_i32(tid_) : tid_;
         if constexpr (VEC) {
 #pragma unroll
             for (int i = 0; i < NCR; ++i) {
@@ -1214,6 +1214,26 @@
 __global__ __launch_bounds__(256 * kWgradGroups) void wgrad_pair_kernel(TconvBwdWeightArgs a1, int n1, int mc1, TconvBwdWeightArgs a2, int n2, int mc2) {
     if ((int)blockIdx.x < n1) tconv_bwd_weight_body<MTW1, NTW1, true, ET>(a1, (int)blockIdx.x, n1, mc1);
     else tconv_bwd_weight_body<MTW2, NTW2, true, ET>(a2, (int)blockIdx.x - n1, n2, mc2);
+}
+constexpr int kWgradRoleRows = 32;
+constexpr size_t wgrad_role_lds_bytes(int MTW, int NTW) { return (size_t)kWgradRoleRows * ((MTW * 16 + 4) + (NTW * 64 + 4)) * sizeof(float); }
+constexpr size_t wgrad_role_pair_lds_bytes() { return wgrad_role_lds_bytes(4, 4) > wgrad_role_lds_bytes(4, 2) ? wgrad_role_lds_bytes(4, 4) : wgrad_role_lds_bytes(4, 2); }
+static_assert(wgrad_role_pair_lds_bytes() <= (size_t)4 * kThinWaveLds * sizeof(float), "the role runs in the LDS of the thin first-layer backward");
+struct WgradRoleArgs {
+    TconvBwdWeightArgs a1, a2;
+    int n1, mc1, n2, mc2;
+};
+__device__ __forceinline__ void wgrad_role_body(const WgradRoleArgs& w, const int vb) {
+    if (vb < w.n1) tconv_bwd_weight_body<4, 4, true, float, 1, kWgradRoleRows>(w.a1, vb, w.n1, w.mc1);
+    else tconv_bwd_weight_body<4, 2, true, float, 1, kWgradRoleRows>(w.a2, vb - w.n1, w.n2, w.mc2);
+}
+__global__ __launch_bounds__(256, 3) void wgrad_role_kernel(WgradRoleArgs w) {
+    wgrad_role_body(w, (int)blockIdx.x);
+}
+template <int ACT>
+__global__ __launch_bounds__(256, 3) void thin_bwd_wgrad_kernel(ThinBwdArgs a, int n_thin, WgradRoleArgs w) {
+    if ((int)blockIdx.x < n_thin) thin_tc1_bwd2_body<float, ACT>(a, (int)blockIdx.x, n_thin);
+    else wgrad_role_body(w, (int)blockIdx.x - n_thin);
 }
 
 enum { kOptAdamw = 0, kOptNadamw = 1, kOptLion = 2, kOptNorm = 3 };
diff --git a/stgcn_amd/csrc/stgcn_kernels_thin.hip.h b/stgcn_amd/csrc/stgcn_kernels_thin.hip.h
--- a/stgcn_amd/csrc/stgcn_kernels_thin.hip.h
+++ b/stgcn_amd/csrc/stgcn_kernels_thin.hip.h
@@ -189,7 +189,7 @@
 static_assert(4 * kThinWaveLds >= 2 * 12 * 64 * 4 + 2 * 16, "the end-of-kernel combine reuses the waves' tiles");
 
 template <typename ET, int ACT, typename ARGS>
-__device__ __forceinline__ void thin_tc1_bwd2_body(const ARGS& a) {
+__device__ __forceinline__ void thin_tc1_bwd2_body(const ARGS& a, const int vb, const int nb) {
     typedef Mma<ET> MM;
     constexpr bool kF32 = sizeof(ET) == 4;
     typedef typename std::conditional<kF32, float, bf16>::type ST;
@@ -200,7 +200,7 @@
     float* const Xt = Dt + 16 * kThinLdD;
     float* const Bs = Xt + 16 * kThinLdX;
     float* const Ws = Bs + 128;
-    const long wave_id = (long)blockIdx.x * 4 + wave, nwaves = (long)gridDim.x * 4;
+    const long wave_id = (long)vb * 4 + wave, nwaves = (long)nb * 4;
     const long rows = a.rows, tiles = (rows + 15) >> 4;
     const int K = a.ts.taps * a.ts.C, C = a.ts.C, N = a.ts.N;
     const unsigned per_b = (unsigned)(a.ts.Tdst * N);
@@ -344,7 +344,7 @@
     for (int i = 0; i < 4; ++i) accA[i] += cmb[(8 + i) * 64 + lane];
     dba += ld4(cmb_ba + 4 * g);
     constexpr int c0 = 64, NC = 128;
-    float* const part = a.part + (size_t)blockIdx.x * (c0 * 16 + 16 + 16 * NC + NC);
+    float* const part = a.part + (size_t)vb * (c0 * 16 + 16 + 16 * NC + NC);
 #pragma unroll
     for (int ct = 0; ct < 4; ++ct)
 #pragma unroll
diff --git a/stgcn_amd/csrc/stgcn_route.h b/stgcn_amd/csrc/stgcn_route.h
--- a/stgcn_amd/csrc/stgcn_route.h
+++ b/stgcn_amd/csrc/stgcn_route.h
@@ -37,6 +37,7 @@
     return env_int("STGCN_HEAD_FUSE", 1);
 #endif
 }
+inline bool wgrad_ride() { return env_not_zero("STGCN_WGRAD_RIDE"); }
 inline int ln_stats_min_chunks() { static const int v = env_int("STGCN_LN_STATS_MIN_CHUNKS", 8); return v; }
 inline int force_tconv_tile_rows() { static const int v = env_int("STGCN_TCONV_TR", 0); return v; }
 inline int force_gemm_ntw() { static const int v = env_int("STGCN_GEMM_NTW", 0); return v; }
diff --git a/stgcn_amd/ops.py b/stgcn_amd/ops.py
--- a/stgcn_amd/ops.py
+++ b/stgcn_amd/ops.py
@@ -358,6 +358,13 @@
         self.blocks = []
         self.head = None
         self.owners = []
+
+    def __del__(self):
+        try:
+            if self.head is not None and _lib._lib is not None:
+                _lib._lib.dll.stgcn_wgrad_ride_drop(self.head[2].data_ptr())
+        except Exception:
+            pass
 
     def holds(self, wsc) -> bool:
         return any(o is wsc for o in self.owners)
@@ -804,7 +811,7 @@
         if ih is not None:
             ih.mark_ready(dx)
         if sink is not None:
-            sink.head = (desc, gst, ctx.ws, (grads, params))
+            sink.head = (desc, gst, ctx.ws, (grads, params, x_cl, saved, fused_loss))
             sink.owners.append(ctx.wsc)
             ctx.wsc.pending_sink = sink
             grads = [None] * len(grads)
```

Result: slower. 90030 windows/s (-1.0%).
